# shiftlab-nanodrone/sparse-gslam

Hardware: AMD Instinct MI355X
Metric: edge-Jacobians/sec per GN iter on SE(2) graph; final chi2 vs g2o (higher is better)
Workload: dtype f64

## Files before the change

### sparse_gslam_amd/csrc/sgo_amg.h

```cpp
#pragma once
#include <hip/hip_runtime.h>

#include <string>
#include <vector>

#include "sgo_internal.h"

namespace sgo {

struct AmgConfig {
  double theta = 0.02;
  double theta_coarse = 0.02;
  double theta_scale = 1.0;
  double omega = 0.8;
  int max_levels = 10;
  int nu_coarse = 1;
  bool nu_from_env = false;
  int kdepth = 1 << 20;
  int fcg2_depth = 1;
  bool smooth = true;
  double omega_p = 0.66;
  double theta_filter = 1e-3;
  bool filtered_smoothing = true;
  bool fold = true;
  int fold0_rows = 60000;
  bool lists_on_device = true;
  int coarsest_nodes = 400;
  const struct AmgKeptAgg* keep_agg = nullptr;
};
struct AmgKeptAgg {
  std::vector<std::vector<int>> agg, visit_c;
  std::vector<int> nc;
};

struct AmgProf {
  void* user = nullptr;
  void (*begin)(void* user, int kid, double bytes) = nullptr;
  void (*end)(void* user) = nullptr;
};

struct AmgHalo {
  HaloDev* dev = nullptr;
  int G = 1, bmax = 0;
  const int* bnd_host = nullptr;
  bool (*reserve)(void* user, size_t packet_doubles) = nullptr;
  void* user = nullptr;
  const std::vector<double>* w0 = nullptr;
};

struct ChunkArena;
struct DevArena;
struct Amg;

struct HostLevel {
  int n = 0, nslot = 0;
  std::vector<int> rowptr, row, col;
  std::vector<int> visit;
};

enum class AmgPatterns { host, device, device_aggregation };
Amg* amg_create(hipStream_t s, const BsrDev& A0, const Sym0Dev& S0, const Tile0Dev& T0, const HostLevel& H0, const double* d_poses,
                const int* d_free_id, const AmgConfig& cfg, const AmgProf& prof, std::string* err, ChunkArena* scratch, DevArena* arena,
                DevArena* tmp_arena, AmgPatterns patterns, struct AmgHostL0* pre0 = nullptr, const AmgHalo* halo = nullptr);
struct AmgHostL0;
AmgHostL0* amg_host_l0_new();
void amg_host_l0_run(AmgHostL0* p, const HostLevel& H0, const std::vector<double>& w, const AmgConfig& cfg, ChunkArena* scratch, bool agg_only = false);
bool amg_host_l0_agg_only(const AmgHostL0* p);
void amg_host_l0_free(AmgHostL0* p);
bool amg_host_l0_ready(const AmgHostL0* p);
AmgConfig amg_effective_config(const AmgConfig& cfg_in, int n, int nslot);
void amg_destroy(Amg* m);
int amg_update(Amg* m, hipStream_t s, std::string* err);
enum class AmgXs0 {
  compute = 0,
  ready = 1,
  ready_with_halo = 2
};
int amg_apply(Amg* m, hipStream_t s, const double* r, double* z, const double* dotvec, double* partials,
              const PcgScalars* S, const double* dotvec2 = nullptr, AmgXs0 xs0 = AmgXs0::compute);
struct Comm;
void amg_set_shard(Amg* m, Comm* comm, int u0, int u1, int row0, int row1, const HaloDev* slices = nullptr);
bool amg_comm_failed(const Amg* m);
int amg_debug_coarse_rhs(Amg* m, hipStream_t s, const double* r, double* out_dev, int cap3);
long long amg_debug_array(Amg* m, hipStream_t s, int level, int what, void* out, long long cap_bytes);
double* amg_xs0(Amg* m);
double amg_omega(const Amg* m);
bool amg_coarsest_not_spd(Amg* m, hipStream_t s);
int amg_num_levels(const Amg* m);
bool amg_has_filtered(const Amg* m);
long long amg_level0_bytes(const Amg* m);
void amg_describe(const Amg* m, std::string* out);
void amg_kept_aggregates(const Amg* m, AmgKeptAgg* out);

}
```

### sparse_gslam_amd/csrc/sgo_amg.hip

```cpp
#include <algorithm>
#include <chrono>
#include <cmath>
#include <cstdio>
#include <cstdlib>
#include <cstring>
#include <numeric>
#include <vector>

#include "sgo_amg.h"
#include "sgo_amg_host.h"
#include "sgo_sort.h"
#include "sgo_comm.h"
#include "sgo_device.h"

namespace sgo {

namespace {

__global__ __launch_bounds__(kBlock) void k_block_norms(BsrDev A, double* __restrict__ w) {
  for (int k = blockIdx.x * kBlock + threadIdx.x; k < A.nslot; k += gridDim.x * kBlock) {
    double b[9];
    load_block(A, (size_t)k, b);
    double s = 0.0;
#pragma unroll
// ... 318 lines not shown
    }
    seg_scan<9>(key, acc);
    if (segment_end(key, lane)) {
#pragma unroll
      for (int c = 0; c < 9; ++c) {
        if (OUT_BSR) out[blk_at(c, (size_t)key, nout)] = acc[c];
        else out[9 * (size_t)key + c] = acc[c];
      }
      if (OUT_BSR && mirror) {
        const int mk = mirror[key];
        if (mk >= 0) {
#pragma unroll
          for (int r = 0; r < 3; ++r)
#pragma unroll
            for (int c = 0; c < 3; ++c) out[blk_at(3 * c + r, (size_t)mk, nout)] = acc[3 * r + c];
        }
      }
    }
  }
}

__device__ __forceinline__ void restrict_groups(const PDev& P, const double* __restrict__ r, double* __restrict__ rc,
                                                const PcgScalars* S, int row0, int row1, int nb_main, int block) {
  const int lane = threadIdx.x & 63;
  const size_t np = (size_t)P.t_n;
  if (block >= nb_main) {
    if (S && S->stop) return;
    __shared__ double sm[kWavesPerBlock][3];
    const int lc = block - nb_main;
    const int gb = P.t_long[2 * lc], ge = P.t_long[2 * lc + 1];
    double acc[3] = {0.0, 0.0, 0.0};
    for (int t = gb + (int)threadIdx.x; t < ge; t += kBlock) {
      const size_t i = (size_t)P.t_row[t];
      if (row1 > 0 && ((int)i < row0 || (int)i >= row1)) continue;
      const double ri[3] = {r[3 * i], r[3 * i + 1], r[3 * i + 2]};
      double b[9];
      load9_pairs(P.t_blk, P.t_blk8, (size_t)t, np, b, P.stream_nt != 0);
      block_tmul_acc(b, ri, acc);
    }
#pragma unroll
    for (int q = 0; q < 3; ++q) {
      const double v = wave_sum(acc[q]);
      if (lane == 0) sm[threadIdx.x >> 6][q] = v;
    }
    __syncthreads();
    if (threadIdx.x < 3) {
      double v = sm[0][threadIdx.x];
      for (int w = 1; w < kWavesPerBlock; ++w) v += sm[w][threadIdx.x];
      rc[3 * (size_t)P.t_col[gb] + threadIdx.x] = v;
    }
    return;
  }
  GroupCursor gc = group_cursor(P.t_grp, P.t_ngrp, nb_main, block);
  if (S && S->stop) return;
  for (bool first = true; gc.g < gc.gend; gc.g += gc.gstride, first = false) {
    int gb, ge;
    group_bounds(gc, P.t_grp, first, gb, ge);
    if (P.t_nlong > 0 && ge - gb > kLongColumn) continue;
    double acc[3] = {0.0, 0.0, 0.0};
    int key = -1 - lane;
    for (int t = gb + lane; t < ge; t += 64) {
      key = P.t_col[t];
      const size_t i = (size_t)P.t_row[t];
      if (row1 > 0 && ((int)i < row0 || (int)i >= row1)) continue;
      const double ri[3] = {r[3 * i], r[3 * i + 1], r[3 * i + 2]};
      double b[9];
      load9_pairs(P.t_blk, P.t_blk8, (size_t)t, np, b, P.stream_nt != 0);
      block_tmul_acc(b, ri, acc);
    }
    seg_scan<3>(key, acc);
    if (segment_end(key, lane)) {
      rc[3 * (size_t)key] = acc[0];
      rc[3 * (size_t)key + 1] = acc[1];
      rc[3 * (size_t)key + 2] = acc[2];
    }
  }
}
__global__ __launch_bounds__(kBlock) void k_restrict_p(PDev P, const double* __restrict__ r, double* __restrict__ rc,
                                                       const PcgScalars* S, int row0, int row1, int nb_main) {
  restrict_groups(P, r, rc, S, row0, row1, nb_main, (int)blockIdx.x);
}
__global__ __launch_bounds__(kBlock, 4) void k_jacobi0_restrict(Sym0Dev A, Spmv0Args a, int nb_spmv, PDev P, double* __restrict__ rc,
                                                                 int nb_main) {
  if ((int)blockIdx.x < nb_spmv) spmv0_groups<S0_JACOBI>(A, a, nb_spmv);
  else restrict_groups(P, a.b, rc, a.S, 0, 0, nb_main, (int)blockIdx.x - nb_spmv);
}
void launch_restrict_p(hipStream_t s, const PDev& P, const double* r, double* rc, const PcgScalars* S, int row0, int row1) {
  const int nb = grid_for(P.t_ngrp, kWavesPerBlock);
  SGO_LAUNCH(k_restrict_p, dim3(nb + P.t_nlong), dim3(kBlock), 0, s, P, r, rc, S, row0, row1, nb);
}

__global__ __launch_bounds__(kBlock) void k_prolong_p(int n, PDev P, const double* __restrict__ u1, SpmvRatio r1,
                                                      const double* __restrict__ u2, SpmvRatio r2,
                                                      double* __restrict__ x, const PcgScalars* S,
                                                      const double* __restrict__ xadd, int row0, int row1) {
  GroupCursor gc = group_cursor(P.r_grp, P.r_ngrp, gridDim.x, blockIdx.x);
  if (S && S->stop) return;
  double c1, c2;
  cycle_coefficients(r1, r2, u2 != nullptr, c1, c2);
  const int lane = threadIdx.x & 63;
  const size_t np = (size_t)P.r_n;
  for (bool first = true; gc.g < gc.gend; gc.g += gc.gstride, first = false) {
    int gb, ge;
    group_bounds(gc, P.r_grp, first, gb, ge);
    double acc[3] = {0.0, 0.0, 0.0};
    int key = -1 - lane;
    for (int e = gb + lane; e < ge; e += 64) {
      key = P.row[e];
      if (row1 > 0 && (key < row0 || key >= row1)) {
        key = -1 - lane;
        continue;
      }
      double w[3], b[9];
      coarse_operand(u1, u2, c1, c2, 3 * (size_t)P.col[e], w);
      load9_pairs(P.r_blk, P.r_blk8, (size_t)e, np, b, P.stream_nt != 0);
      block_mul_acc(b, w, acc);
    }
    seg_scan<3>(key, acc);
    if (segment_end(key, lane)) {
      const size_t o = 3 * (size_t)key;
      if (xadd) {
        acc[0] += xadd[o]; acc[1] += xadd[o + 1]; acc[2] += xadd[o + 2];
      }
      x[o] += acc[0]; x[o + 1] += acc[1]; x[o + 2] += acc[2];
    }
  }
}

__device__ __forceinline__ int find_sorted(const int* __restrict__ v, int lo, int hi, int key) {
  while (lo < hi) {
    const int mid = (lo + hi) >> 1;
    const int x = v[mid];
    if (x == key) return mid;
    if (x < key) lo = mid + 1;
    else hi = mid;
  }
  return -1;
}

struct FoldDev {
  int f_lo = 0, f_hi = 0;
  const int* row = nullptr;
  const int* col = nullptr;
  int* ap2p = nullptr;
  int* st_pos = nullptr;
};
struct UpDev {
  int n = 0, ngrp = 0;
  const int* row = nullptr;
  const int* idx = nullptr;
  const int* col = nullptr;
  const int* grp = nullptr;
};

__global__ __launch_bounds__(kBlock) void k_fold_match(FoldDev F, const int* __restrict__ p_rowptr, const int* __restrict__ p_col,
                                                       unsigned long long* __restrict__ keys) {
  for (int f = F.f_lo + blockIdx.x * kBlock + threadIdx.x; f < F.f_hi; f += gridDim.x * kBlock) {
    const int i = F.row[f], c = F.col[f];
    F.ap2p[f] = find_sorted(p_col, p_rowptr[i], p_rowptr[i + 1], c);
    keys[f - F.f_lo] = ((unsigned long long)(unsigned)c << 32) | (unsigned)(f - F.f_lo);
  }
}
__global__ __launch_bounds__(kBlock) void k_fold_unpack(FoldDev F, const unsigned long long* __restrict__ sorted, int* __restrict__ t_row,
                                                        int* __restrict__ t_col) {
  const int nf = F.f_hi - F.f_lo;
  for (int t = blockIdx.x * kBlock + threadIdx.x; t < nf; t += gridDim.x * kBlock) {
    const unsigned long long k = sorted[t];
    const int f = F.f_lo + (int)(unsigned)(k & 0xffffffffull);
// ... 880 lines not shown
               (const double*)P.blk, (const double*)L.A.dinv, m->cfg.omega, L.PS);
  }
  if (P.local_lists) hipMemsetAsync(C.A.blk, 0, sizeof(double) * 9 * (size_t)C.A.nslot, s);
  {
    Scope sc(m->prof, level0 ? K_SA_RAP0 : K_SA_RAP, 156.0 * P.rap.n + 72.0 * C.A.nslot);
    SGO_LAUNCH((k_block_products<false, true, true>), dim3(grid_for(P.rap.ngrp, kWavesPerBlock)), dim3(kBlock), 0, s,
               P.rap, BsrDev(), (const double*)P.blk, (const double*)P.apblk, C.A.blk, (size_t)C.A.nslot, (const int*)P.rap_mirror,
               (const int*)P.row, row0, P.local_lists ? 0 : row1, 1);
  }
  if (own) sh.reduce(s, C.A.blk, 9 * (size_t)C.A.nslot);
}

struct CoarseSol {
  const double *u1 = nullptr, *u2 = nullptr;
  SpmvRatio c1, c2;
};
struct RhsSub { const double* sub; SpmvRatio c; double* out; };
struct DotReq { const double *vec = nullptr, *vec2 = nullptr; double* parts = nullptr; };

struct CycleForm { int nu; enum { unfolded, folded, folded_in_two_sweeps } kind; };
CycleForm cycle_form(const Amg* m, int l, bool rhs_sub, bool dots) {
  const AmgLevel& L = m->lv[l];
  CycleForm f{(l > 0 && L.tR && L.smoothed) ? std::max(1, m->cfg.nu_coarse) : 1, CycleForm::unfolded};
  if (!L.fold || rhs_sub) return f;
  if (l == 0) {
    if (m->shard.mode == Shard0::single) f.kind = CycleForm::folded;
  } else if (!dots) {
    if (f.nu == 1) f.kind = CycleForm::folded;
    if (f.nu == 2) f.kind = CycleForm::folded_in_two_sweeps;
  }
  return f;
}

bool fold_level(const Amg* m, int l, int nf) {
  return m->cfg.fold && nf > 0 && (l > 0 || (m->shard.mode != Shard0::owner && m->lv[0].A.n <= m->cfg.fold0_rows));
}

CoarseSol coarse_solve(Amg* m, hipStream_t s, int l, const PcgScalars* S);

void restrict_level(Amg* m, hipStream_t s, int l, const double* res, const PcgScalars* S, bool folded = false) {
  AmgLevel& L = m->lv[l];
  AmgLevel& C = m->lv[l + 1];
  const int row0 = l == 0 ? m->shard.row0 : 0, row1 = l == 0 ? m->shard.row1 : 0;
  if (l == 0 && m->shard.mode == Shard0::owner && L.smoothed && L.P.local_lists)
    hipMemsetAsync(C.bk, 0, sizeof(double) * 3 * (size_t)C.A.n, s);
  if (L.smoothed) {
    const PDev& P = folded ? L.PS : L.P;
    Scope sc(m->prof, l == 0 ? K_RESTRICT_P0 : K_RESTRICT_P, 44.0 * P.t_n + 24.0 * L.A.n + 24.0 * L.nc);
    launch_restrict_p(s, P, res, C.bk, S, row0, row1);
  } else {
    Scope sc(m->prof, l == 0 ? K_RESTRICT0 : K_RESTRICT, 40.0 * L.A.n + 24.0 * L.nc);
    SGO_LAUNCH(k_restrict, dim3(grid_for(L.mem_ngrp, kWavesPerBlock)), dim3(kBlock), 0, s, L.mem_ngrp, L.mem_grp, L.mem, L.agg, L.d, res, C.bk, S, row0, row1);
  }
}
int jacobi_sweep(Amg* m, hipStream_t s, AmgLevel& L, const double* x, const double* b, double* out, const PcgScalars* S,
                 const DotReq& dots = DotReq(), const CoarseSol* cs = nullptr) {
  SpmvArgs a{};
  a.x = x; a.b = b; a.y = out; a.omega = m->cfg.omega; a.S = S;
  if (dots.vec) { a.dotA = dots.vec; a.dotA2 = dots.vec2; a.partials = dots.parts; }
  if (cs) {
    a.agg = L.agg; a.d = L.d; a.u1 = cs->u1; a.u2 = cs->u2; a.c1 = cs->c1; a.c2 = cs->c2;
    Scope sc(m->prof, K_SPMV_JACOBI_P, 80.0 * L.A.nslot + 140.0 * L.A.n + 48.0 * L.nc);
    return launch_spmv_ex(s, L.A, SPMV_JACOBI_P, a);
  }
  Scope sc(m->prof, K_SPMV_JACOBI, 80.0 * L.A.nslot + 120.0 * L.A.n);
  return launch_spmv_ex(s, L.A, SPMV_JACOBI, a);
}

int pass0(Amg* m, hipStream_t s, int mode, const Spmv0Args& a, int ranks = 1) {
  const bool tile = m->T0.ntile > 0, f32 = tile && m->S0.fblk != nullptr;
  const int kid = mode == S0_RESID ? (tile ? (f32 ? K_SPMV0T_RESID_F32 : K_SPMV0T_RESID) : K_SPMV0_RESID)
                                   : (tile ? (f32 ? K_SPMV0T_JACOBI_F32 : K_SPMV0T_JACOBI) : K_SPMV0_JACOBI);
  Scope sc(m->prof, kid, bytes_spmv0(m->S0, mode, f32) / ranks);
  return launch_spmv0_any(s, m->S0, m->T0, mode, a);
}
void first_sweep0(Amg* m, hipStream_t s, const double* rhs, AmgXs0 xs0) {
  if (xs0 != AmgXs0::compute) return;
  const Shard0& sh = m->shard;
  const bool own = sh.mode == Shard0::owner;
  const size_t r0 = own ? sh.row0 : 0;
  Scope sc(m->prof, K_DOT, 96.0 * m->lv[0].A.n);
  launch_precond_bj(s, own ? sh.row1 - sh.row0 : m->lv[0].A.n, m->S0.dinv + 6 * r0, rhs + 3 * r0, m->lv[0].xs + 3 * r0, m->cfg.omega);
}
void presmooth0(Amg* m, hipStream_t s, const double* rhs, const PcgScalars* S, AmgXs0 xs0) {
  AmgLevel& L = m->lv[0];
  Shard0& sh = m->shard;
  first_sweep0(m, s, rhs, xs0);
  if (sh.mode == Shard0::owner && xs0 != AmgXs0::ready_with_halo) sh.exchange(s, L.xs, 3, sh.part->bnd, sh.part->bmax);
  if (sh.mode == Shard0::allreduce && !sh.part) hipMemsetAsync(L.rs, 0, sizeof(double) * 3 * (size_t)L.A.n, s);
  Spmv0Args a{};
  a.x = L.xs; a.b = rhs; a.y = L.rs; a.S = S; a.u0 = sh.u0; a.u1 = sh.u1;
  if (sh.mode == Shard0::single || a.u1 > a.u0) pass0(m, s, S0_RESID, a, sh.G);
}
void prolong0(Amg* m, hipStream_t s, const CoarseSol& cs, const PcgScalars* S) {
  AmgLevel& L = m->lv[0];
  const Shard0& sh = m->shard;
  const bool own = sh.mode == Shard0::owner;
  const int row0 = own ? sh.row0 : 0, row1 = own ? sh.row1 : 0;
  if (L.smoothed) {
    Scope sc(m->prof, K_PROLONG_P0, 44.0 * L.P.r_n + 52.0 * L.A.n);
    SGO_LAUNCH(k_prolong_p, dim3(grid_for(L.P.r_ngrp, kWavesPerBlock)), dim3(kBlock), 0, s, L.A.n, L.P, cs.u1, cs.c1, cs.u2, cs.c2,
               L.xs, S, (const double*)nullptr, row0, row1);
  } else {
    Scope sc(m->prof, K_PROLONG0, 68.0 * L.A.n);
    SGO_LAUNCH(k_prolong_add, dim3(grid_for(own ? row1 - row0 : L.A.n, kBlock)), dim3(kBlock), 0, s, L.A.n, L.agg, L.d, cs.u1, cs.c1,
                       cs.u2, cs.c2, L.xs, S, (const double*)nullptr, row0, row1);
  }
  if (own && sh.part->nhalo > 0) {
    const HaloDev& H = *sh.part;
    SGO_LAUNCH(k_prolong_rows, dim3(grid_for(H.nhalo, kBlock)), dim3(kBlock), 0, s, H.nhalo, H.halo_rows, L.smoothed ? L.P : PDev(),
               (const int*)L.agg, (const double*)L.d, cs.u1, cs.c1, cs.u2, cs.c2, L.xs, S);
  }
}
int postsmooth0(Amg* m, hipStream_t s, const double* rhs, double* out, const DotReq& dots, const PcgScalars* S) {
  AmgLevel& L = m->lv[0];
  Shard0& sh = m->shard;
  Spmv0Args b{};
  b.x = L.xs; b.b = rhs; b.y = out; b.omega = m->cfg.omega; b.S = S; b.u0 = sh.u0; b.u1 = sh.u1;
  if (sh.mode != Shard0::allreduce) {
    if (dots.vec) { b.dotA = dots.vec; b.dotA2 = dots.vec2; b.partials = dots.parts; }
    return pass0(m, s, S0_JACOBI, b, sh.G);
  }
  if (!sh.part) hipMemsetAsync(out, 0, sizeof(double) * 3 * (size_t)L.A.n, s);
  if (b.u1 > b.u0) pass0(m, s, S0_JACOBI, b);
  if (sh.part) sh.gather(s, out);
  else sh.reduce(s, out, 3 * (size_t)L.A.n);
  if (!dots.vec) return 0;
  const int grid = grid_for(3LL * L.A.n, kBlock);
  Scope sc(m->prof, K_DOT, 72.0 * L.A.n);
  SGO_LAUNCH(k_dots2, dim3(grid), dim3(kBlock), 0, s, 3 * L.A.n, (const double*)out, dots.vec, dots.vec2, dots.parts, S);
  return grid;
}
int cycle0_fold(Amg* m, hipStream_t s, const double* rhs, double* out, const DotReq& dots, const PcgScalars* S, AmgXs0 xs0) {
  AmgLevel& L = m->lv[0];
  AmgLevel& C = m->lv[1];
  first_sweep0(m, s, rhs, xs0);
  Spmv0Args b{};
  b.x = L.xs; b.b = rhs; b.y = L.rs; b.omega = m->cfg.omega; b.S = S;
  if (m->T0.ntile == 0) {
    const int nb_spmv = grid_for(m->S0.ngrp, kWavesPerBlock), nb_main = grid_for(L.PS.t_ngrp, kWavesPerBlock);
    Scope sc(m->prof, K_JACOBI0_RESTRICT, bytes_spmv0(m->S0, S0_JACOBI) + 44.0 * L.PS.t_n + 24.0 * L.A.n + 24.0 * L.nc);
    SGO_LAUNCH(k_jacobi0_restrict, dim3(nb_spmv + nb_main + L.PS.t_nlong), dim3(kBlock), 0, s, m->S0, b, nb_spmv, L.PS, C.bk, nb_main);
  } else {
    pass0(m, s, S0_JACOBI, b);
    restrict_level(m, s, 0, rhs, S, true);
  }
  const CoarseSol cs = coarse_solve(m, s, 0, S);
  const int grid = std::min(grid_for(L.PS.r_ngrp, kFoldThreads / 64), 512);
  Scope sc(m->prof, K_PROLONG_FOLD0, 44.0 * L.PS.r_n + 72.0 * L.A.n);
  SGO_LAUNCH(k_prolong_fold, dim3(grid), dim3(kFoldThreads), 0, s, L.PS, cs.u1, cs.c1, cs.u2, cs.c2, (const double*)L.rs, out, S, dots.vec,
             dots.vec2, dots.vec ? dots.parts : nullptr);
  return grid;
}
int cycle0(Amg* m, hipStream_t s, const double* rhs, double* out, const DotReq& dots, const PcgScalars* S, AmgXs0 xs0) {
  if (cycle_form(m, 0, false, dots.vec).kind == CycleForm::folded) return cycle0_fold(m, s, rhs, out, dots, S, xs0);
  presmooth0(m, s, rhs, S, xs0);
  restrict_level(m, s, 0, m->lv[0].rs, S);
  m->shard.reduce(s, m->lv[1].bk, 3 * (size_t)m->lv[1].A.n);
  const CoarseSol cs = coarse_solve(m, s, 0, S);
  prolong0(m, s, cs, S);
  return postsmooth0(m, s, rhs, out, dots, S);
}

constexpr int kUnfuseSlots = 400000;
void pre_resid(Amg* m, hipStream_t s, AmgLevel& L, const double* rhs, const PcgScalars* S) {
  SpmvArgs a{};
  a.b = rhs; a.y = L.rs; a.omega = m->cfg.omega; a.S = S;
  if (L.A.nslot >= kUnfuseSlots) {
    {
      Scope sc(m->prof, K_DOT, 96.0 * L.A.n);
      launch_precond_bj(s, L.A.n, L.A.dinv, rhs, L.xs, m->cfg.omega);
    }
    a.x = L.xs;
    Scope sc(m->prof, K_SPMV_RESID, 80.0 * L.A.nslot + 72.0 * L.A.n);
    launch_spmv_ex(s, L.A, SPMV_RESID, a);
    return;
  }
  a.y2 = L.xs;
  Scope sc(m->prof, K_SPMV_PRE_RESID, 80.0 * L.A.nslot + 120.0 * L.A.n);
  launch_spmv_ex(s, L.A, SPMV_PRE_RESID, a);
}
const double* presmooth(Amg* m, hipStream_t s, AmgLevel& L, const double* rhs, const RhsSub* sub, int nu, const PcgScalars* S) {
  if (sub) {
    SpmvArgs a{};
    a.b = rhs; a.y = L.rs; a.y2 = L.xs; a.omega = m->cfg.omega; a.S = S; a.bsub = sub->sub; a.c1 = sub->c; a.b_out = sub->out;
    Scope sc(m->prof, K_SPMV_PRE_RESID_S, 80.0 * L.A.nslot + 168.0 * L.A.n);
    launch_spmv_ex(s, L.A, SPMV_PRE_RESID_S, a);
  } else {
    pre_resid(m, s, L, rhs, S);
  }
  double* res = L.rs;
  for (int sw = 1; sw < nu; ++sw) {
    SpmvArgs a{};
    a.b = res; a.y = (res == L.rs) ? L.tR : L.rs; a.y2 = L.xs; a.omega = m->cfg.omega; a.S = S;
    Scope sc(m->prof, K_SPMV_PRE_RESID_ACC, 80.0 * L.A.nslot + 144.0 * L.A.n);
    launch_spmv_ex(s, L.A, SPMV_PRE_RESID_ACC, a);
    res = a.y;
  }
  return res;
}
int prolong_postsmooth(Amg* m, hipStream_t s, AmgLevel& L, const double* rhs, double* out, const CoarseSol& cs, int nu,
                       const DotReq& dots, const PcgScalars* S) {
  if (L.smoothed) {
    {
      Scope sc(m->prof, K_PROLONG_P, 80.0 * L.P.np + 52.0 * L.A.n);
      SGO_LAUNCH(k_prolong_p, dim3(grid_for(L.P.r_ngrp, kWavesPerBlock)), dim3(kBlock), 0, s, L.A.n, L.P, cs.u1, cs.c1, cs.u2, cs.c2,
                 L.xs, S, (const double*)nullptr, 0, 0);
    }
    const double* x = L.xs;
    for (int sw = 1; sw < nu; ++sw) {
      double* dst = (x == L.rs) ? L.tR : L.rs;
      jacobi_sweep(m, s, L, x, rhs, dst, S);
      x = dst;
    }
    return jacobi_sweep(m, s, L, x, rhs, out, S, dots);
  }
  if (L.A.nslot < kUnfuseSlots) return jacobi_sweep(m, s, L, L.xs, rhs, out, S, dots, &cs);
  {
    Scope sc(m->prof, K_PROLONG, 52.0 * L.A.n + 48.0 * L.nc);
    SGO_LAUNCH(k_prolong_add, dim3(grid_for(L.A.n, kBlock)), dim3(kBlock), 0, s, L.A.n, L.agg, L.d, cs.u1, cs.c1, cs.u2, cs.c2, L.xs, S,
               (const double*)nullptr, 0, 0);
  }
  return jacobi_sweep(m, s, L, L.xs, rhs, out, S, dots);
}
int cycle_coarse_fold(Amg* m, hipStream_t s, int l, const double* rhs, double* out, const PcgScalars* S, const double* xadd = nullptr) {
  AmgLevel& L = m->lv[l];
  restrict_level(m, s, l, rhs, S, true);
  const CoarseSol cs = coarse_solve(m, s, l, S);
  Scope sc(m->prof, K_UP_FOLD, 80.0 * L.A.nslot + 44.0 * L.PS.r_n + 100.0 * L.A.n);
  const int grid = grid_for(L.U.ngrp, kWavesPerBlock);
  SGO_LAUNCH(k_up_fold, dim3(grid), dim3(kBlock), 0, s, L.A, L.U, L.PS, rhs, m->cfg.omega, cs.u1, cs.c1, cs.u2, cs.c2, out, S, xadd);
  return grid;
}
int cycle_coarse(Amg* m, hipStream_t s, int l, const double* rhs, double* out, const PcgScalars* S, const RhsSub* sub = nullptr,
                 const DotReq& dots = DotReq()) {
  AmgLevel& L = m->lv[l];
  const CycleForm f = cycle_form(m, l, sub != nullptr, dots.vec != nullptr);
  if (f.kind == CycleForm::folded) return cycle_coarse_fold(m, s, l, rhs, out, S);
  if (f.kind == CycleForm::folded_in_two_sweeps) {
// ... 58 lines not shown
    for (const AmgLevel& L : m->lv)
      if (L.smoothed && L.P.dF) return true;
  return false;
}
long long amg_level0_bytes(const Amg* m) { return m ? m->level0_bytes : 0; }
bool amg_coarsest_not_spd(Amg* m, hipStream_t s) {
  int f = 0;
  if (!m || !m->d_fail) return false;
  if (hipMemcpyAsync(&f, m->d_fail, sizeof(int), hipMemcpyDeviceToHost, s) != hipSuccess) return false;
  if (hipStreamSynchronize(s) != hipSuccess) return false;
  return f != 0;
}
void amg_describe(const Amg* m, std::string* out) { *out = m ? m->desc : ""; }
void amg_kept_aggregates(const Amg* m, AmgKeptAgg* out) {
  if (m && out) *out = m->kept;
}

void amg_destroy(Amg* m) {
  if (!m) return;
  delete m;
}


int amg_update(Amg* m, hipStream_t s, std::string* err) {
  const int last = (int)m->lv.size() - 1;
  {
    AmgLevel& L0 = m->lv[0];
    Scope sc(m->prof, K_POSITIONS0, 40.0 * L0.A.n);
    SGO_LAUNCH(k_positions0, dim3(grid_for(L0.A.n, kBlock)), dim3(kBlock), 0, s, L0.A.n, m->d_free_id, m->d_poses,
                       L0.pos);
  }
  for (int l = 0; l < last; ++l) {
    AmgLevel& L = m->lv[l];
    AmgLevel& C = m->lv[l + 1];
    {
      Scope sc(m->prof, K_CENTRES, 36.0 * L.A.n);
      SGO_LAUNCH(k_centres, dim3(grid_for(L.nc, kWavesPerBlock)), dim3(kBlock), 0, s, L.nc, L.mem_ptr, L.mem, L.pos, C.pos, L.d);
    }
    launch_coarse_operator(m, s, L, C, l == 0);
    {
      Scope sc(m->prof, K_LEVEL_DINV, 120.0 * C.A.n);
      SGO_LAUNCH(k_level_dinv, dim3(grid_for(C.A.n, kBlock)), dim3(kBlock), 0, s, C.A);
    }
  }
  {
    Scope sc(m->prof, K_DENSE_INVERT, 8.0 * m->Np * m->Np);
    const int nb = m->Np / kGjB;
    hipMemsetAsync(m->inv0, 0, sizeof(double) * (size_t)m->Np * m->Np, s);
    hipMemsetAsync(m->d_fail, 0, sizeof(int), s);
    if (last > 0)
      SGO_LAUNCH(k_dense_fill_unique, dim3(grid_for(m->lv[last].A.nslot, kBlock)), dim3(kBlock), 0, s, m->lv[last].A, m->Np, m->inv0);
    else
      SGO_LAUNCH(k_dense_fill, dim3(grid_for(m->lv[last].A.n, kBlock)), dim3(kBlock), 0, s, m->lv[last].A, m->Np, m->inv0);
    SGO_LAUNCH(k_gj_pivot, dim3(1), dim3(kGjB * kGjB), 0, s, m->inv0, m->Np, 0, m->gjP[0], m->d_fail);
    for (int kb = 0; kb < nb; ++kb) {
      const double* src = (kb & 1) ? m->inv1 : m->inv0;
      double* dst = (kb & 1) ? m->inv0 : m->inv1;
      SGO_LAUNCH(k_gj_step, dim3(nb, nb), dim3(kBlock), 0, s, src, dst, m->Np, kb, (const double*)m->gjP[kb & 1],
                 m->gjP[(kb + 1) & 1], m->d_fail);
    }
  }
  const hipError_t le = hipGetLastError();
  if (le != hipSuccess) {
    if (err) *err = std::string("amg_update: a kernel launch failed: ") + hipGetErrorString(le);
    return SGO_EHIP;
  }
  return SGO_OK;
}

void amg_set_shard(Amg* m, Comm* comm, int u0, int u1, int row0, int row1, const HaloDev* slices) {
  m->shard.mode = Shard0::allreduce;
  m->shard.u0 = u0; m->shard.u1 = u1; m->shard.row0 = row0; m->shard.row1 = row1;
  m->shard.comm = comm;
  m->shard.part = slices;
}
bool amg_comm_failed(const Amg* m) { return m && m->shard.failed; }
int amg_debug_coarse_rhs(Amg* m, hipStream_t s, const double* r, double* out_dev, int cap3) {
  if (!m || m->lv.size() < 2) return 0;
  const int n3c = 3 * m->lv[1].A.n;
  if (cap3 < n3c) return -1;
  if (m->lv[0].fold) {
    restrict_level(m, s, 0, r, nullptr, true);
  } else {
    presmooth0(m, s, r, nullptr, AmgXs0::compute);
    restrict_level(m, s, 0, m->lv[0].rs, nullptr);
  }
  hipMemcpyAsync(out_dev, m->lv[1].bk, sizeof(double) * n3c, hipMemcpyDeviceToDevice, s);
  return n3c;
}
namespace {
__global__ __launch_bounds__(kBlock) void k_debug_blocks(BsrDev A, const float* __restrict__ fblk, const float* __restrict__ fblk8,
                                                         double* __restrict__ out) {
  for (int k = blockIdx.x * kBlock + threadIdx.x; k < A.nslot; k += gridDim.x * kBlock) {
    double b[9];
    load_block(A, (size_t)k, b);
    if (fblk && A.ref && A.ref[k] >= 0) {
      const int r = A.ref[k];
      const size_t u = (size_t)(r >> 1), nu = (size_t)A.nus;
      double v[9];
      for (int c = 0; c < 8; ++c) v[c] = (double)fblk[4 * ((size_t)(c >> 2) * nu + u) + (c & 3)];
      v[8] = (double)fblk8[u];
      for (int p = 0; p < 3; ++p)
        for (int q = 0; q < 3; ++q) b[3 * p + q] = (r & 1) ? v[3 * q + p] : v[3 * p + q];
    }
    for (int c = 0; c < 9; ++c) out[9 * (size_t)k + c] = b[c];
  }
}
}

long long amg_debug_array(Amg* m, hipStream_t s, int level, int what, void* out, long long cap_bytes) {
  if (!m || level < 0 || level >= (int)m->lv.size()) return 0;
  if (m->shard.mode != Shard0::single) return SGO_EINVAL;
  const int last = (int)m->lv.size() - 1;
  AmgLevel& L = m->lv[level];
  const PDev& P = L.P;
  const PDev& PS = L.PS;
  const bool transfer = level < last, sm = transfer && L.smoothed, fo = sm && L.fold;
  const size_t n = (size_t)L.A.n, ns = (size_t)L.A.nslot, nc = transfer ? (size_t)L.nc : 0;
  const size_t nsc = transfer ? (size_t)m->lv[level + 1].A.nslot : 0;
  const void* src = nullptr;
  size_t bytes = 0;
  auto arr = [&](bool have, const void* p, size_t count, size_t elem) {
    if (have && p) {
      src = p;
      bytes = count * elem;
    }
  };
  const size_t I = sizeof(int), F = sizeof(float), Dd = sizeof(double);
  const bool f32 = level == 0 && m->T0.ntile > 0 && m->S0.fblk != nullptr;
  switch (what) {
    case SGO_AMG_INFO: {
      const CycleForm cf = cycle_form(m, level, false, false);
      const double v[SGO_AMG_INFO_COUNT] = {(double)n, (double)ns, (double)nc, sm ? 1.0 : 0.0, (sm && P.dF) ? 1.0 : 0.0, fo ? 1.0 : 0.0,
                                            transfer ? (double)cf.kind : 0.0, transfer ? (double)cf.nu : 0.0, m->cfg.omega, m->cfg.omega_p,
                                            sm ? (double)P.np : 0.0, sm ? (double)P.nap : 0.0, sm ? (double)P.val.n : 0.0,
                                            sm ? (double)P.ap.n : 0.0, sm ? (double)P.rap.n : 0.0, (double)(last + 1), f32 ? 1.0 : 0.0,
                                            (double)m->N, (double)m->Np, sm ? (double)P.t_nlong : 0.0, fo ? (double)PS.t_nlong : 0.0,
                                            (double)m->kdepth, m->cfg.theta_filter, (double)nsc};
      if (cap_bytes >= (long long)sizeof v) std::memcpy(out, v, sizeof v);
      return (long long)sizeof v;
    }
    case SGO_AMG_A_ROWPTR: arr(true, L.A.rowptr, n + 1, I); break;
    case SGO_AMG_A_COL: arr(true, L.A.col, ns, I); break;
    case SGO_AMG_A_BLK:
    case SGO_AMG_A_BLK_F32: {
      if (what == SGO_AMG_A_BLK_F32 && !f32) return 0;
      const long long need = (long long)(9 * ns * Dd);
      if (cap_bytes < need) return need;
      double* tmp = nullptr;
      if (hipMalloc(&tmp, (size_t)need) != hipSuccess) return SGO_ENOMEM;
      SGO_LAUNCH(k_debug_blocks, dim3(grid_for((long long)ns, kBlock)), dim3(kBlock), 0, s, L.A,
                 what == SGO_AMG_A_BLK_F32 ? (const float*)m->S0.fblk : (const float*)nullptr, (const float*)m->S0.fblk8, tmp);
      hipError_t e = hipMemcpyAsync(out, tmp, (size_t)need, hipMemcpyDeviceToHost, s);
      if (e == hipSuccess) e = hipStreamSynchronize(s);
      hipFree(tmp);
      return e == hipSuccess ? need : (long long)SGO_EHIP;
    }
    case SGO_AMG_A_DINV: arr(true, L.A.dinv, 6 * n, Dd); break;
    case SGO_AMG_POS: arr(true, L.pos, 2 * n, Dd); break;
    case SGO_AMG_D: arr(transfer, L.d, 2 * n, Dd); break;
    case SGO_AMG_AGG: arr(transfer, L.agg, n, I); break;
    case SGO_AMG_MEM_PTR: arr(transfer, L.mem_ptr, nc + 1, I); break;
    case SGO_AMG_MEM: arr(transfer, L.mem, n, I); break;
    case SGO_AMG_P_ROWPTR: arr(sm, P.rowptr, n + 1, I); break;
    case SGO_AMG_P_ROW: arr(sm, P.row, (size_t)P.np, I); break;
    case SGO_AMG_P_COL: arr(sm, P.col, (size_t)P.np, I); break;
    case SGO_AMG_P_BLK: arr(sm, P.blk, 9 * (size_t)P.np, Dd); break;
    case SGO_AMG_P_RBLK: arr(sm, P.r_blk, 9 * (size_t)P.r_n, F); break;
    case SGO_AMG_P_TBLK: arr(sm, P.t_blk, 9 * (size_t)P.t_n, F); break;
    case SGO_AMG_P_TPOS: arr(sm, P.t_pos, (size_t)P.np, I); break;
    case SGO_AMG_P_TROW: arr(sm, P.t_row, (size_t)P.np, I); break;
    case SGO_AMG_P_TCOL: arr(sm, P.t_col, (size_t)P.np, I); break;
    case SGO_AMG_STRONG: arr(sm && P.dF, P.strong, ns, 1); break;
    case SGO_AMG_DF: arr(sm, P.dF, 9 * n, Dd); break;
    case SGO_AMG_DINVF: arr(sm, P.dinvF, 9 * n, Dd); break;
    case SGO_AMG_AP_A: arr(sm, P.ap.a, (size_t)P.ap.n, I); break;
    case SGO_AMG_AP_B: arr(sm, P.ap.b, (size_t)P.ap.n, I); break;
    case SGO_AMG_AP_TGT: arr(sm, P.ap.tgt, (size_t)P.ap.n, I); break;
    case SGO_AMG_AP_BLK: arr(sm, P.apblk, 9 * (size_t)P.nap, Dd); break;
    case SGO_AMG_PS_ROW: arr(fo, PS.row, (size_t)PS.np, I); break;
    case SGO_AMG_PS_COL: arr(fo, PS.col, (size_t)PS.np, I); break;
    case SGO_AMG_PS_RBLK: arr(fo, PS.r_blk, 9 * (size_t)PS.r_n, F); break;
    case SGO_AMG_PS_TBLK: arr(fo, PS.t_blk, 9 * (size_t)PS.t_n, F); break;
    case SGO_AMG_PS_TROW: arr(fo, PS.t_row, (size_t)PS.np, I); break;
    case SGO_AMG_PS_TCOL: arr(fo, PS.t_col, (size_t)PS.np, I); break;
    case SGO_AMG_PS_STPOS: arr(fo, L.F.st_pos, (size_t)PS.np, I); break;
    case SGO_AMG_INV: arr(level == last, m->inv, (size_t)m->Np * m->Np, Dd); break;
    default: return SGO_EINVAL;
  }
  if (!src || bytes == 0) return 0;
  if (cap_bytes < (long long)bytes) return (long long)bytes;
  if (hipMemcpyAsync(out, src, bytes, hipMemcpyDeviceToHost, s) != hipSuccess || hipStreamSynchronize(s) != hipSuccess) return SGO_EHIP;
  return (long long)bytes;
}
double* amg_xs0(Amg* m) { return (m && m->lv.size() > 1) ? m->lv[0].xs : nullptr; }
double amg_omega(const Amg* m) { return m ? m->cfg.omega : 0.0; }

int amg_apply(Amg* m, hipStream_t s, const double* r, double* z, const double* dotvec, double* partials,
              const PcgScalars* S, const double* dotvec2, AmgXs0 xs0) {
  if (m->lv.size() == 1) {
    {
      Scope sc(m->prof, K_DENSE_APPLY, 8.0 * m->N * m->N);
      SGO_LAUNCH(k_dense_apply, dim3(grid_for(m->N, kWavesPerBlock)), dim3(kBlock), 0, s, m->N, m->Np, m->inv, r, z, S);
    }
    if (!dotvec) return 0;
    const int grid = grid_for(m->N, kBlock);
    Scope sc(m->prof, K_DOT, 24.0 * m->N);
    SGO_LAUNCH(k_dots2, dim3(grid), dim3(kBlock), 0, s, m->N, (const double*)z, dotvec, dotvec2, partials, S);
    return grid;
  }
  return cycle0(m, s, r, z, DotReq{dotvec, dotvec2, partials}, S, xs0);
}

void dev_scan_exclusive(hipStream_t s, int* v, int n, int* sums) {
  if (n <= kScanSmall) {
    SGO_LAUNCH(k_scan_small, dim3(1), dim3(1024), 0, s, v, n);
    return;
  }
  const int nb = (n + kScanChunk - 1) / kScanChunk;
  SGO_LAUNCH(k_scan_sums, dim3(std::max(nb, 1)), dim3(kBlock), 0, s, (const int*)v, n, sums);
  SGO_LAUNCH(k_scan_top, dim3(1), dim3(kBlock), 0, s, sums, nb);
  SGO_LAUNCH(k_scan_apply, dim3(std::max(nb, 1)), dim3(kBlock), 0, s, v, n, (const int*)sums, nb);
}
AmgConfig amg_effective_config(const AmgConfig& cfg_in, int n, int nslot) {
  AmgConfig cfg = cfg_in;
  cfg.nu_coarse = nslot >= 600000 ? 2 : 1;
  if (const char* e = std::getenv("SGO_AMG_SMOOTH")) cfg.smooth = std::atoi(e) != 0;
  if (const char* e = std::getenv("SGO_AMG_LISTS")) cfg.lists_on_device = std::string(e) != "host";
  if (const char* e = std::getenv("SGO_AMG_THETA_FILTER")) cfg.theta_filter = std::atof(e);
  if (const char* e = std::getenv("SGO_AMG_FILTER")) cfg.filtered_smoothing = cfg.filtered_smoothing && std::atoi(e) != 0;
  if (const char* e = std::getenv("SGO_AMG_OMEGA")) cfg.omega = std::atof(e);
  if (const char* e = std::getenv("SGO_AMG_OMEGA_P")) cfg.omega_p = std::atof(e);
  if (const char* e = std::getenv("SGO_AMG_THETA")) cfg.theta = cfg.theta_coarse = std::atof(e);
  if (const char* e = std::getenv("SGO_AMG_FOLD")) cfg.fold = std::atoi(e) != 0;
  if (const char* e = std::getenv("SGO_AMG_FOLD0_ROWS")) cfg.fold0_rows = std::atoi(e);
  cfg.fold = cfg.fold && cfg.smooth && cfg.lists_on_device;
  if (const char* e = std::getenv("SGO_AMG_NU")) {
    cfg.nu_coarse = std::max(1, std::atoi(e));
    cfg.nu_from_env = true;
  }
  if (cfg.smooth) cfg.kdepth = 0;
  if (const char* e = std::getenv("SGO_AMG_KDEPTH")) cfg.kdepth = std::atoi(e);
  if (const char* e = std::getenv("SGO_AMG_FCG2_DEPTH")) cfg.fcg2_depth = std::atoi(e);
  cfg.coarsest_nodes = std::min(1000, std::max(cfg.coarsest_nodes, n / 1500));
  return cfg;
}

struct AmgHostL0 {
  HostCoarse hc;
  bool ready = false;
  bool agg_only = false;
  double theta_used = 0.0;
};

#include "sgo_amg_dev.inc"

AmgHostL0* amg_host_l0_new() { return new AmgHostL0(); }
void amg_host_l0_free(AmgHostL0* p) { delete p; }
bool amg_host_l0_ready(const AmgHostL0* p) { return p && p->ready; }
bool amg_host_l0_agg_only(const AmgHostL0* p) { return p && p->ready && p->agg_only; }
void amg_host_l0_run(AmgHostL0* p, const HostLevel& H0, const std::vector<double>& w, const AmgConfig& cfg_in, ChunkArena* scratch, bool agg_only) {
  try {
    const AmgConfig cfg = amg_effective_config(cfg_in, H0.n, H0.nslot);
    if (H0.n <= cfg.coarsest_nodes || 1 >= cfg.max_levels) return;
    if (agg_only) {
      p->hc.nc = host_aggregate(H0, w, cfg, 0, scratch, p->hc.agg, p->hc.visit_c, &p->theta_used);
      p->agg_only = true;
      p->ready = true;
      return;
    }
    host_coarsen(H0, w, cfg, 0, scratch, p->hc);
    p->ready = p->hc.err.empty();
  } catch (...) {
    p->ready = false;
  }
}

namespace {

enum GroupId { G_MEM, G_VAL, G_R, G_T, G_C, G_F, G_GAL, G_ST, G_PSR, G_U, G_APL, G_RAPL, G_COUNT };
struct GroupBatch {
  struct Job {
    const int* ptr = nullptr;
    int nseg = 0, total = 0;
    bool on = false;
    const int** grp = nullptr;
    int* ngrp = nullptr;
  };
  Job job[G_COUNT];
  template <class IntPtr>
  void add(GroupId id, const int* ptr, int nseg, int total, IntPtr* grp, int* ngrp) {
    job[id] = Job{ptr, nseg, total, true, (const int**)grp, ngrp};
  }
  bool run(DevSetup& D) {
// ... 690 lines not shown
```

### sparse_gslam_amd/csrc/sgo_ctx.h

```cpp
#pragma once
#include <chrono>
#include <cstdio>
#include <cstring>
#include <memory>
#include <string>
#include <thread>
#include <vector>

#include "sgo_amg.h"
#include "sgo_comm.h"
#include "sgo_direct.h"
#include "sgo_mfront.h"
#include "sgo_internal.h"
#include "sgo_overlay.h"
#include "sgo_policy.h"

using namespace sgo;

struct HostArena {
  std::unique_ptr<char[]> mem;
  size_t cap = 0, used = 0;
  void reserve(size_t bytes) {
    used = 0;
    if (bytes <= cap) return;
// ... 1 lines not shown
    cap = bytes + bytes / 4;
    mem.reset(new char[cap + 64]);
  }
  void* take(size_t bytes) {
    char* base = (char*)(((uintptr_t)mem.get() + 63) & ~(uintptr_t)63);
    void* q = base + used;
    used += (bytes + 63) & ~(size_t)63;
    return used <= cap ? q : nullptr;
  }
};

struct HaloHost {
  int G = 1, me = 0, bmax = 0;
  std::vector<int> rank_row;
  std::vector<int> bnd;
};

struct sgo_ctx {
  int device = 0;
  HostArena stage;
  ChunkArena amg_scratch;
  hipStream_t stream = nullptr;
  sgo_opts opts{};
  std::string err;
  Comm comm;
  int shard_u0 = 0, shard_u1 = 0, shard_units = 0;
  int shard_row0 = 0, shard_row1 = 0;
  std::vector<int> unit_row0;
  bool owner = false;
  bool gather_slices = false;
  bool replicated = false;
  HaloDev halo;
  HaloHost halo_host;
  bool halo_failed = false;
  std::vector<double> order_xy;
  HierarchyState hier;
  bool amg_dchg_pending = false;
  int probe_dev_k = -1;
  double probe_dev_max = -1.0;
  double* d_dref = nullptr;
  double* d_dref_agg = nullptr;
  int agg_grid = 0;
  double* h_dchg = nullptr;
  int dchg_grid = 0;
  double* h_dchg_dev = nullptr;
  double last_dchg[3] = {0, 0, 0};
  std::string lag_note;
  int* d_comm_flag = nullptr;
  bool comm_graph_failed = false;
  long long level0_bytes = 0;
  double *halo_send = nullptr, *halo_recv = nullptr;
  size_t halo_cap = 0;
  int halo_ranks = 0;

  bool has_graph = false;
  int V = 0, E = 0, n = 0;
  std::vector<int> free_id;
  std::vector<int> fixed_active;
  std::vector<int> row_of_asc;
  HostLevel H0;
  double setup_seconds = 0.0;

  DevArena graph_arena;
  DevArena amg_arena;
  DevArena amg_arena_prev;
  DevArena amg_tmp_arena;
  Amg* amg_prev = nullptr;
  std::string amg_prev_desc;
  struct CallKnobs {
    int comm_graph = -1;
    int stall_window = -1;
    int first_solve_cap = 600;
    bool fail_trial_build = false;
    bool fail_device_setup = false;
    bool keep_agg = false;
    int setup_mode = 2;
    bool dev_aggregation = false;
    bool lag_on = true;
    double lag_tau = 0.006;
    double lag_slope = 0.0;
    int lag_force_from = -1;
    int rebuild_cost = 150;
    bool force_rebuild = false;
  } knobs;
  struct CallState {
    bool in_optimize = false;
    int pcg_softcap = 0;
    double bb_ref = 0.0;
    bool warm_valid = false;
    bool floor_seen = false;
    bool lag_on = false;
    bool skip_update = false;
    bool lag_expect = false;
    bool force_keep = false;
    int lag_cap = 0;
  } call;
  AmgKeptAgg kept_agg;
  double* d_poses = nullptr;
  int* d_free_id = nullptr;
  EdgeListDev el;
  Sym0Dev S0;
  Tile0Dev T0;
  BsrDev A;
  EdgeSlotsDev es;
  int *d_rowptr = nullptr, *d_eidx = nullptr, *d_hrowptr = nullptr;
  double *d_dgb = nullptr, *d_b = nullptr, *d_x = nullptr, *d_r = nullptr, *d_z = nullptr, *d_p = nullptr,
         *d_q = nullptr, *d_s1 = nullptr, *d_s2 = nullptr, *d_e2 = nullptr;
  double* d_partials = nullptr;
  double* d_hist = nullptr;
  PcgScalars* d_S = nullptr;
  double* d_lanczos = nullptr;
  int pcg_exec_key = 0;
  PcgScalars* h_S = nullptr;
  double* h_hist = nullptr;
  bool linearized = false;

  Amg* amg = nullptr;
  bool amg_pending = false;
  bool rows_pending = false;
  std::vector<uint8_t> lz_fixed;
  std::vector<int32_t> lz_ei, lz_ej;
  Direct* direct = nullptr;
  std::string direct_why;
  Mfront* mf = nullptr;
  std::string mf_why;
  int mf_order_hint = -1;
  DirectResult* d_dres = nullptr;
  DirectResult* h_dres = nullptr;
  double* d_zparts = nullptr;
  struct PcgCounts {
    int start_bb = 0, start_rz = 0;
    int n_pq = 0, n_rz = 0, n_rr = 0, n_zq = 0;
    int n_xq = 0, n_bx = 0;
  } pcg_counts;
  struct PcgStartArgs {
    double tol = 0.0, tol_cap = 0.0, bb_ref = 0.0;
    int maxit = 0;
  } pcg_start;
  std::string solver_desc;
  std::string solver_text;

  hipGraphExec_t pcg_exec = nullptr;
  int pcg_exec_chunk = 0;
  int pcg_pred = 0;
  bool pcg_stalled = false;
  int pcg_stall_window = 0;
  double tol_scale = 1.0;
  double* d_xprev = nullptr;
  double tol_cap = 0.0;
  AmgHostL0* l0_pre = nullptr;
  std::thread l0_thread;
  std::vector<double> l0_w;
  PcgScalars* h_S2 = nullptr;
  double* h_pose_stage = nullptr;
  size_t pose_stage_cap = 0;
  PcgScalars* h_Sz = nullptr;
  PcgScalars* d_Sz = nullptr;
  hipEvent_t ev_S[2] = {nullptr, nullptr};

  Overlay ov;
  int its_base = 0;
  int its_last = 0;
  std::string update_note;

  struct EdgeActivity {
    bool ready = false;
    std::vector<int32_t> vi, vj;
    std::vector<uint8_t> dead;
    std::vector<int32_t> live_deg;
    int n_inactive = 0;
    int* d_ids = nullptr;
    double* d_rows = nullptr;
    unsigned char* d_flag = nullptr;
    unsigned char* d_mark = nullptr;
    double* d_parts = nullptr;
    size_t ids_cap = 0, rows_cap = 0, flag_cap = 0, mark_cap = 0, parts_cap = 0;
  } edges;
  struct RobustKinds {
    std::vector<uint8_t> kind;
    int n_other = 0;
    unsigned char* d_kind = nullptr;
    size_t kind_cap = 0;
  } robust;

  struct Hypotheses {
    char* d_ws = nullptr;
    size_t ws_cap = 0;
  } hyp;

  struct Marginals {
    double* d_cov = nullptr;
    int* d_idx = nullptr;
    size_t cov_cap = 0, idx_cap = 0;
  } marg;

// ... 233 lines not shown
```

### sparse_gslam_amd/csrc/sgo_device.h

```cpp
#pragma once
#include "sgo_internal.h"

namespace sgo {
namespace {

constexpr double kPi = 3.14159265358979323846;

__device__ __forceinline__ double norm_theta(double t) {
  if (t >= -kPi && t < kPi) return t;
  double m = floor(t / (2 * kPi));
  t = t - m * 2 * kPi;
  if (t >= kPi) t -= 2 * kPi;
  if (t < -kPi) t += 2 * kPi;
  return t;
}


struct EdgeOperands {
  double xi, yi, ti, xj, yj, tj;
  double zx, zy, zt;
};
template <class Src>
__device__ __forceinline__ void edge_operands(const Src& s, size_t ns, int k, const double* __restrict__ poses, EdgeOperands& p) {
  const int vi = s.vi[k], vj = s.vj[k];
// ... 180 lines not shown
  edge_error(p, sz, cz, e);
  EdgeWeight W;
  edge_weight<KINDS>(s, ns, k, e, W);
  EdgeJac J;
  edge_jacobians(p, sz, cz, J);
  edge_side(W, J, dir, S);
}

__device__ __forceinline__ double readlane_d(double v, int l) {
  const int lo = __builtin_amdgcn_readlane(__double2loint(v), l), hi = __builtin_amdgcn_readlane(__double2hiint(v), l);
  return __hiloint2double(hi, lo);
}

__device__ __forceinline__ double wave_sum(double v);

template <int N>
__device__ __forceinline__ void block_sum_store(double (&v)[N], double* out, int stride) {
  __shared__ double sm[N][kWavesPerBlock];
  const int lane = threadIdx.x & 63, w = threadIdx.x >> 6;
#pragma unroll
  for (int i = 0; i < N; ++i) {
    double s = wave_sum(v[i]);
    if (lane == 0) sm[i][w] = s;
  }
  __syncthreads();
  if (threadIdx.x == 0) {
#pragma unroll
    for (int i = 0; i < N; ++i) {
      double s = sm[i][0];
#pragma unroll
      for (int k = 1; k < kWavesPerBlock; ++k) s += sm[i][k];
      out[(size_t)i * stride + blockIdx.x] = s;
    }
  }
}

__device__ __forceinline__ double block_reduce_parts(const double* parts, int nparts) {
  __shared__ double sm2[kWavesPerBlock];
  __shared__ double res;
  double s = 0.0;
  for (int i = threadIdx.x; i < nparts; i += kBlock) s += parts[i];
  s = wave_sum(s);
  __syncthreads();
  if ((threadIdx.x & 63) == 0) sm2[threadIdx.x >> 6] = s;
  __syncthreads();
  if (threadIdx.x == 0) {
    double t = sm2[0];
#pragma unroll
    for (int k = 1; k < kWavesPerBlock; ++k) t += sm2[k];
    res = t;
  }
  __syncthreads();
  return res;
}

template <int N>
__device__ __forceinline__ void block_reduce_parts_n(const double* const (&parts)[N], const int (&cnt)[N],
                                                     double (&out)[N]) {
  __shared__ double smn[N][kWavesPerBlock];
  double s[N];
#pragma unroll
  for (int c = 0; c < N; ++c) {
    s[c] = 0.0;
    if (parts[c])
      for (int i = threadIdx.x; i < cnt[c]; i += kBlock) s[c] += parts[c][i];
  }
#pragma unroll
  for (int c = 0; c < N; ++c) s[c] = wave_sum(s[c]);
  __syncthreads();
  if ((threadIdx.x & 63) == 0) {
#pragma unroll
    for (int c = 0; c < N; ++c) smn[c][threadIdx.x >> 6] = s[c];
  }
  __syncthreads();
#pragma unroll
  for (int c = 0; c < N; ++c) {
    double t = smn[c][0];
#pragma unroll
    for (int k = 1; k < kWavesPerBlock; ++k) t += smn[c][k];
    out[c] = t;
  }
}

template <int CTRL, int ROW_MASK>
__device__ __forceinline__ int dpp_int(int old, int v) {
  if (ROW_MASK == 0xF) return __builtin_amdgcn_update_dpp(0, v, CTRL, 0xF, 0xF, true);
  return __builtin_amdgcn_update_dpp(old, v, CTRL, ROW_MASK, 0xF, false);
}
__device__ __forceinline__ int next_lane_key(int key) { return __builtin_amdgcn_update_dpp(0, key, 0x130, 0xF, 0xF, true); }
template <int CTRL, int ROW_MASK>
__device__ __forceinline__ double dpp_double(double v) {
  const int lo = dpp_int<CTRL, ROW_MASK>(0, __double2loint(v)), hi = dpp_int<CTRL, ROW_MASK>(0, __double2hiint(v));
  return __hiloint2double(hi, lo);
}
__device__ __forceinline__ double wave_sum(double v) {
  v += dpp_double<0x111, 0xF>(v);
  v += dpp_double<0x112, 0xF>(v);
  v += dpp_double<0x114, 0xF>(v);
  v += dpp_double<0x118, 0xF>(v);
  v += dpp_double<0x142, 0xA>(v);
  v += dpp_double<0x143, 0xC>(v);
  return __hiloint2double(__builtin_amdgcn_readlane(__double2hiint(v), 63), __builtin_amdgcn_readlane(__double2loint(v), 63));
}

template <int N, int CTRL, int ROW_MASK>
__device__ __forceinline__ void seg_scan_step(int row, double (&v)[N]) {
  constexpr int kNoKey = (int)0x80000000;
  const double f = dpp_int<CTRL, ROW_MASK>(kNoKey, row) == row ? 1.0 : 0.0;
#pragma unroll
  for (int i = 0; i < N; ++i) {
    const double u = dpp_double<CTRL, ROW_MASK>(v[i]);
    v[i] = fma(f, u, v[i]);
  }
}
template <int N>
__device__ __forceinline__ void seg_scan(int row, double (&v)[N]) {
  seg_scan_step<N, 0x111, 0xF>(row, v);
  seg_scan_step<N, 0x112, 0xF>(row, v);
  seg_scan_step<N, 0x114, 0xF>(row, v);
  seg_scan_step<N, 0x118, 0xF>(row, v);
  seg_scan_step<N, 0x142, 0xA>(row, v);
  seg_scan_step<N, 0x143, 0xC>(row, v);
}
__device__ __forceinline__ bool segment_end(int key, int lane) {
  const int kn = next_lane_key(key);
  return key >= 0 && (lane == 63 || kn != key);
}

__device__ __forceinline__ void load_block(const BsrDev& A, size_t k, double (&b)[9]) {
  double v0, v1, v2, v3, v4, v5, v6, v7, v8;
  if (A.ref == nullptr) {
    const size_t ns = (size_t)A.nslot;
    v0 = A.blk[blk_at(0, k, ns)]; v1 = A.blk[blk_at(1, k, ns)]; v2 = A.blk[blk_at(2, k, ns)];
    v3 = A.blk[blk_at(3, k, ns)]; v4 = A.blk[blk_at(4, k, ns)]; v5 = A.blk[blk_at(5, k, ns)];
    v6 = A.blk[blk_at(6, k, ns)]; v7 = A.blk[blk_at(7, k, ns)]; v8 = A.blk[blk_at(8, k, ns)];
  } else {
    const int r = A.ref[k];
    if (r < 0) {
      const double* d = A.dblk + 6 * (size_t)(~r);
      v0 = d[0]; v1 = d[1]; v2 = d[2];
      v3 = v1; v4 = d[3]; v5 = d[4];
      v6 = v2; v7 = v5; v8 = d[5];
    } else {
      const size_t u = (size_t)(r >> 1), nu = (size_t)A.nus;
      const double2* __restrict__ bp = reinterpret_cast<const double2*>(A.ublk);
      const double2 p0 = bp[u], p1 = bp[nu + u], p2 = bp[2 * nu + u], p3 = bp[3 * nu + u];
      const bool tr = r & 1;
      v0 = p0.x; v4 = p2.x; v8 = A.ublk8[u];
      v1 = tr ? p1.y : p0.y; v3 = tr ? p0.y : p1.y;
      v2 = tr ? p3.x : p1.x; v6 = tr ? p1.x : p3.x;
      v5 = tr ? p3.y : p2.y; v7 = tr ? p2.y : p3.y;
    }
  }
  b[0] = v0; b[1] = v1; b[2] = v2; b[3] = v3; b[4] = v4; b[5] = v5; b[6] = v6; b[7] = v7; b[8] = v8;
}

template <int WAVES = kWavesPerBlock, class NB, class B>
__device__ __forceinline__ void group_walk_b(int ngrp, NB nblocks, B block, int* first, int* last, int* stride) {
  const int xcd = block & 7, slot = block >> 3, per_xcd = nblocks >> 3;
  const int lo = (int)(((long long)ngrp * xcd) >> 3), hi = (int)(((long long)ngrp * (xcd + 1)) >> 3);
  *first = lo + slot * WAVES + (threadIdx.x >> 6);
  *last = hi;
  *stride = per_xcd * WAVES;
}
__device__ __forceinline__ void group_walk(int ngrp, int* first, int* last, int* stride) {
  group_walk_b(ngrp, gridDim.x, blockIdx.x, first, last, stride);
// ... 30 lines not shown
  const double* const parts[4] = {r1.num ? r1.den : nullptr, r1.num, (use2 && r2.num) ? r2.den : nullptr,
                                  use2 ? r2.num : nullptr};
  const int cnt[4] = {r1.n_den, r1.n_num, r2.n_den, r2.n_num};
  double v[4];
  block_reduce_parts_n<4>(parts, cnt, v);
  if (r1.num) c1 = cycle_ratio(v[0], v[1]);
  if (use2) c2 = cycle_ratio(v[2], v[3]);
}

__device__ __forceinline__ void coarse_operand(const double* __restrict__ u1, const double* __restrict__ u2, double c1, double c2,
                                               size_t a, double (&w)[3]) {
  w[0] = c1 * u1[a]; w[1] = c1 * u1[a + 1]; w[2] = c1 * u1[a + 2];
  if (u2) {
    w[0] += c2 * u2[a]; w[1] += c2 * u2[a + 1]; w[2] += c2 * u2[a + 2];
  }
}

__device__ __forceinline__ void block_mul_acc(const double (&b)[9], const double (&x)[3], double* acc) {
  acc[0] += b[0] * x[0] + b[1] * x[1] + b[2] * x[2];
  acc[1] += b[3] * x[0] + b[4] * x[1] + b[5] * x[2];
  acc[2] += b[6] * x[0] + b[7] * x[1] + b[8] * x[2];
}
__device__ __forceinline__ void block_mul_acc(double2 p0, double2 p1, double2 p2, double2 p3, double b8, const double (&x)[3], double* acc) {
  acc[0] += p0.x * x[0] + p0.y * x[1] + p1.x * x[2];
  acc[1] += p1.y * x[0] + p2.x * x[1] + p2.y * x[2];
  acc[2] += p3.x * x[0] + p3.y * x[1] + b8 * x[2];
}
__device__ __forceinline__ void block_tmul_acc(const double (&b)[9], const double (&r)[3], double* acc) {
  acc[0] += b[0] * r[0] + b[3] * r[1] + b[6] * r[2];
  acc[1] += b[1] * r[0] + b[4] * r[1] + b[7] * r[2];
  acc[2] += b[2] * r[0] + b[5] * r[1] + b[8] * r[2];
}

__device__ __forceinline__ void rigid_add(double dx, double dy, const double (&w)[3], double* x) {
  x[0] += w[0] - dy * w[2]; x[1] += w[1] + dx * w[2]; x[2] += w[2];
}
__device__ __forceinline__ void rigid_t_acc(double dx, double dy, const double (&r)[3], double* acc) {
  acc[0] += r[0]; acc[1] += r[1]; acc[2] += -dy * r[0] + dx * r[1] + r[2];
}
__device__ __forceinline__ void block_rigid_col(const double (&b)[9], double dx, double dy, double (&m)[3]) {
  m[0] = -dy * b[0] + dx * b[1] + b[2];
  m[1] = -dy * b[3] + dx * b[4] + b[5];
  m[2] = -dy * b[6] + dx * b[7] + b[8];
}
__device__ __forceinline__ void block_rigid_acc(const double (&b)[9], double dx, double dy, double* acc) {
  acc[0] += b[0]; acc[1] += b[1]; acc[2] += -dy * b[0] + dx * b[1] + b[2];
  acc[3] += b[3]; acc[4] += b[4]; acc[5] += -dy * b[3] + dx * b[4] + b[5];
  acc[6] += b[6]; acc[7] += b[7]; acc[8] += -dy * b[6] + dx * b[7] + b[8];
}
__device__ __forceinline__ void rigid_t_block_acc(const double (&b)[9], const double (&m)[3], double dx, double dy, double* acc) {
  acc[0] += b[0]; acc[1] += b[1]; acc[2] += m[0];
  acc[3] += b[3]; acc[4] += b[4]; acc[5] += m[1];
  acc[6] += -dy * b[0] + dx * b[3] + b[6]; acc[7] += -dy * b[1] + dx * b[4] + b[7];
  acc[8] += -dy * m[0] + dx * m[1] + m[2];
}

__device__ __forceinline__ void dinv_apply(const double* __restrict__ di, double omega, const double (&v)[3], double (&o)[3]) {
  o[0] = omega * (di[0] * v[0] + di[1] * v[1] + di[2] * v[2]);
  o[1] = omega * (di[1] * v[0] + di[3] * v[1] + di[4] * v[2]);
  o[2] = omega * (di[2] * v[0] + di[4] * v[1] + di[5] * v[2]);
}
__device__ __forceinline__ void dinv_from_block(const double (&d)[6], double* __restrict__ di) {
  const double d00 = d[0], d01 = d[1], d02 = d[2], d11 = d[3], d12 = d[4], d22 = d[5];
  const double c00 = d11 * d22 - d12 * d12, c01 = d02 * d12 - d01 * d22, c02 = d01 * d12 - d02 * d11;
  const double c11 = d00 * d22 - d02 * d02, c12 = d01 * d02 - d00 * d12, c22 = d00 * d11 - d01 * d01;
  const double det = d00 * c00 + d01 * c01 + d02 * c02;
  const double id = (det != 0.0 && isfinite(det)) ? 1.0 / det : 0.0;
  di[0] = c00 * id; di[1] = c01 * id; di[2] = c02 * id; di[3] = c11 * id; di[4] = c12 * id; di[5] = c22 * id;
}

template <int MODE>
__device__ __forceinline__ void spmv0_groups(const Sym0Dev& A, const Spmv0Args& a, int nblocks) {
  const int lane = threadIdx.x & 63;
  const size_t nu = (size_t)A.nus;
  const double2* __restrict__ bp = reinterpret_cast<const double2*>(A.ublk);
  double dotacc[2] = {0.0, 0.0};
  const int ulo = a.u1 > 0 ? a.u0 : 0, uhi = a.u1 > 0 ? a.u1 : A.ngrp;
  GroupCursor gc = group_cursor(A.grp, uhi - ulo, nblocks, blockIdx.x, ulo);
  int f_r0 = 0, f_ob = 0, f_tb = 0;
  if (gc.g < gc.gend) {
    f_r0 = A.grow[gc.g]; f_ob = A.gown[gc.g]; f_tb = A.gtr[gc.g];
  }
  if (a.S && a.S->stop) return;
  for (bool first = true; gc.g < gc.gend; gc.g += gc.gstride, first = false) {
    int gb, ge;
    group_bounds(gc, A.grp, first, gb, ge);
    const int r0 = first ? f_r0 : A.grow[gc.g];
    int ob = first ? f_ob : A.gown[gc.g], tb = first ? f_tb : A.gtr[gc.g];
    double acc[3] = {0.0, 0.0, 0.0};
    int row = -1 - lane;
    for (int kb = gb; kb < ge; kb += 64) {
      const int k = kb + lane;
      const bool active = k < ge;
      const int m = active ? (int)A.meta[k] : (kSlotNoBlock << 6);
      const int cj = active ? A.col[k] : 0;
      const int type = m >> 6;
      const unsigned long long omask = __ballot(type == kSlotOwned), tmask = __ballot(type == kSlotTransposed);
      const int orank = (int)__builtin_amdgcn_mbcnt_hi((unsigned)(omask >> 32), __builtin_amdgcn_mbcnt_lo((unsigned)omask, 0u));
      const int trank = (int)__builtin_amdgcn_mbcnt_hi((unsigned)(tmask >> 32), __builtin_amdgcn_mbcnt_lo((unsigned)tmask, 0u));
      int idx = ob + orank;
      const bool tr = type == kSlotTransposed;
      if (tr) idx = A.tref[tb + trank];
      ob += __popcll(omask);
      tb += __popcll(tmask);
      if (active) row = r0 + (m & 63);
      if (type != kSlotNoBlock) {
        const size_t c = 3 * (size_t)cj;
        const double x0 = a.x[c], x1 = a.x[c + 1], x2 = a.x[c + 2];
        const double2 p0 = bp[idx], p1 = bp[nu + idx], p2 = bp[2 * nu + idx], p3 = bp[3 * nu + idx];
        const double b8 = A.ublk8[idx];
        const double m01 = tr ? p1.y : p0.y, m02 = tr ? p3.x : p1.x;
        const double m10 = tr ? p0.y : p1.y, m12 = tr ? p3.y : p2.y;
        const double m20 = tr ? p1.x : p3.x, m21 = tr ? p2.y : p3.y;
        acc[0] += p0.x * x0 + m01 * x1 + m02 * x2;
        acc[1] += m10 * x0 + p2.x * x1 + m12 * x2;
        acc[2] += m20 * x0 + m21 * x1 + b8 * x2;
      }
    }
    double dd0 = 0, dd1 = 0, dd2 = 0, dd3 = 0, dd4 = 0, dd5 = 0, s0 = 0, s1 = 0, s2 = 0, rb0 = 0, rb1 = 0, rb2 = 0;
    double di[6] = {0, 0, 0, 0, 0, 0};
    if (row >= 0) {
      const size_t o = 3 * (size_t)row;
      const double* dd = A.dblk + 6 * (size_t)row;
      dd0 = dd[0]; dd1 = dd[1]; dd2 = dd[2]; dd3 = dd[3]; dd4 = dd[4]; dd5 = dd[5];
      s0 = a.x[o]; s1 = a.x[o + 1]; s2 = a.x[o + 2];
      if (MODE != S0_AX) {
        rb0 = a.b[o]; rb1 = a.b[o + 1]; rb2 = a.b[o + 2];
      }
      if (MODE == S0_JACOBI) {
#pragma unroll
        for (int q = 0; q < 6; ++q) di[q] = A.dinv[6 * (size_t)row + q];
      }
    }
    seg_scan<3>(row, acc);
    if (segment_end(row, lane)) {
      const size_t o = 3 * (size_t)row;
      double o0 = acc[0] + dd0 * s0 + dd1 * s1 + dd2 * s2;
      double o1 = acc[1] + dd1 * s0 + dd3 * s1 + dd4 * s2;
      double o2 = acc[2] + dd2 * s0 + dd4 * s1 + dd5 * s2;
      if (MODE != S0_AX) {
        const double t[3] = {rb0 - o0, rb1 - o1, rb2 - o2};
        if (MODE == S0_JACOBI) {
          double sw[3];
          dinv_apply(di, a.omega, t, sw);
          o0 = s0 + sw[0]; o1 = s1 + sw[1]; o2 = s2 + sw[2];
        } else {
          o0 = t[0]; o1 = t[1]; o2 = t[2];
        }
      }
      a.y[o] = o0; a.y[o + 1] = o1; a.y[o + 2] = o2;
      if (a.dotA) dotacc[0] += a.dotA[o] * o0 + a.dotA[o + 1] * o1 + a.dotA[o + 2] * o2;
      if (a.dotA2) dotacc[1] += a.dotA2[o] * o0 + a.dotA2[o + 1] * o1 + a.dotA2[o + 2] * o2;
    }
  }
  if (a.partials) block_sum_store<2>(dotacc, a.partials, kMaxPartials);
}

}
}
```

### sparse_gslam_amd/csrc/sgo_internal.h

```cpp
#pragma once
#include <hip/hip_runtime.h>
#include <hip/hip_ext.h>

#include <algorithm>
#include <atomic>
#include <cstdint>
#include <cstdlib>
#include <string>
#include <vector>

#include "sgo.h"
#include "sgo_hostpool.h"

namespace sgo {

struct BsrDev {
  int n = 0;
  int nslot = 0;
  int ngrp = 0;
  int* row = nullptr;
  int* col = nullptr;
  int* grp = nullptr;
  int* rowptr = nullptr;
  double* blk = nullptr;
// ... 18 lines not shown
  int ncs = 0;
  int ngrp = 0;
  int* col = nullptr;
  unsigned char* meta = nullptr;
  int* tref = nullptr;
  int* grp = nullptr;
  int* grow = nullptr;
  int* gown = nullptr;
  int* gtr = nullptr;
  int nus = 0;
  double* ublk = nullptr;
  double* ublk8 = nullptr;
  float* fblk = nullptr;
  float* fblk8 = nullptr;
  double* dblk = nullptr;
  double* dinv = nullptr;
};

struct TileDesc {
  int row0, row1;
  int g0, g1;
  int h0, h1;
  int e0;
  int nstaged;
};
struct Tile0Dev {
  int ntile = 0;
  int lds_bytes = 0;
  TileDesc* tile = nullptr;
  unsigned int* cv = nullptr;
  unsigned char* off1 = nullptr;
  int* grp1 = nullptr;
  int* grow1 = nullptr;
  int* trowptr = nullptr;
  int* hcol = nullptr;
  int* hfirst = nullptr;
  int hstride = 0;
};

enum : int {
  kRobustDcs = 0, kRobustHuber = 2, kRobustPseudoHuber = 3, kRobustCauchy = 4, kRobustGemanMcClure = 5, kRobustWelsch = 6,
  kRobustFair = 7, kRobustTukey = 8, kRobustSaturated = 9
};

enum : int { kSlotDir = 1, kSlotNoEdge = 2, kSlotFixedCol = 4 };
struct EdgeSlotsDev {
  int stride = 0;
  int* vi = nullptr;
  int* vj = nullptr;
  unsigned char* flags = nullptr;
  double* zinv = nullptr;
  double* info = nullptr;
  double* phi = nullptr;
  unsigned char* kind = nullptr;
  int kinds = 0;
};

struct EdgeListDev {
  int E = 0;
  int cnt = 0;
  int* vi = nullptr;
  int* vj = nullptr;
  double* zinv = nullptr;
  double* info = nullptr;
  double* phi = nullptr;
  unsigned char* kind = nullptr;
  int kinds = 0;
};

struct PcgScalars {
  double rz;
  double pq;
  double rr;
  double bb;
  double alpha;
  double beta;
  double tol2;
  double rz_prev;
  int iter;
  int maxit;
  int stop;
  int iter_prev;
  int probe_k;
  int pad_;
  double probe_rel;
  double probe_max;
};

enum : int {
  SPMV_AX = 0, SPMV_RESID = 1, SPMV_JACOBI = 2, SPMV_PRE_RESID = 3,
  SPMV_JACOBI_P = 4, SPMV_PRE_RESID_S = 5, SPMV_AX_C = 6,
  SPMV_PRE_RESID_ACC = 7
};
struct SpmvRatio {
  const double* num = nullptr;
  int n_num = 0;
  const double* den = nullptr;
  int n_den = 0;
};
struct SpmvArgs {
  const double* x = nullptr;
  double* y = nullptr;
  const double* b = nullptr;
  double* y2 = nullptr;
  double omega = 0.0;
  const double* dotA = nullptr;
  const double* dotA2 = nullptr;
  const double* dotB = nullptr;
  const double* dotC = nullptr;
  double* partials = nullptr;
  const PcgScalars* S = nullptr;
  SpmvRatio c1, c2;
  const int* agg = nullptr;
  const double* d = nullptr;
  const double* u1 = nullptr;
  const double* u2 = nullptr;
  const double* bsub = nullptr;
  double* b_out = nullptr;
  const double* x2 = nullptr;
  double* x_out = nullptr;
};

enum : int { S0_AX = 0, S0_RESID = 1, S0_JACOBI = 2 };
struct Spmv0Args {
  const double* x = nullptr;
  double* y = nullptr;
  const double* b = nullptr;
  double omega = 0.0;
  const double* dotA = nullptr;
  const double* dotA2 = nullptr;
  double* partials = nullptr;
  const PcgScalars* S = nullptr;
  long long* dbg_stamps = nullptr;
  bool force_f64 = false;
  int u0 = 0, u1 = 0;
};

struct Comm;
constexpr int kHaloScalars = 4;
struct HaloDev {
  Comm* comm = nullptr;
  int G = 1, me = 0;
  int row0 = 0, row1 = 0;
  int u0 = 0, u1 = 0;
  int g0 = 0, g1 = 0;
  int bmax = 0;
  const int* bnd = nullptr;
  int maxrows = 0;
  const int* rank_row = nullptr;
  int nhalo = 0;
  const int* halo_rows = nullptr;
  int pemax = 0;
  const int* pent = nullptr;
  double* send = nullptr;
  double* recv = nullptr;
  size_t cap = 0;
  double* gparts = nullptr;
  bool* failed = nullptr;
};
struct HaloScalars {
  const double* parts[kHaloScalars] = {nullptr, nullptr, nullptr, nullptr};
  int n[kHaloScalars] = {0, 0, 0, 0};
};

enum KernelId : int {
  K_CHI2 = 0,
  K_REDUCE2,
  K_LINEARIZE,
  K_FINALIZE,
  K_INIT_SCALARS,
  K_SPMV_AX,
  K_SPMV_RESID,
  K_SPMV_JACOBI,
  K_SPMV_PRE_RESID,
  K_SPMV_JACOBI_P,
  K_SPMV_PRE_RESID_S,
  K_SPMV_AX_C,
  K_ALPHA,
  K_UPDATE_XR,
  K_BETA,
  K_UPDATE_P,
  K_DOT,
  K_POSE_UPDATE,
  K_POSITIONS0,
  K_CENTRES,
  K_GALERKIN,
  K_LEVEL_DINV,
  K_RESTRICT,
  K_PROLONG,
  K_DENSE_INVERT,
  K_DENSE_APPLY,
  K_SA_P,
  K_SA_AP,
  K_SA_RAP,
  K_RESTRICT_P,
  K_PROLONG_P,
  K_SPMV_PRE_RESID_ACC,
  K_SPMV0_AX,
  K_SPMV0_RESID,
  K_SPMV0_JACOBI,
  K_SPMV0T_AX,
  K_SPMV0T_RESID,
  K_SPMV0T_JACOBI,
  K_DIRECT,
  K_SPMV0T_RESID_F32,
  K_SPMV0T_JACOBI_F32,
  K_RESTRICT_P0,
  K_PROLONG_P0,
  K_SA_P0,
  K_SA_AP0,
  K_SA_RAP0,
  K_GALERKIN0,
  K_RESTRICT0,
  K_PROLONG0,
  K_PTILDE,
// ... 125 lines not shown
  }
  struct Mark {
    std::vector<size_t> used;
  };
  Mark mark() const {
    Mark m;
    for (const Chunk& c : chunks) m.used.push_back(c.used);
    return m;
  }
  void rewind_to(const Mark& m) {
    for (size_t i = 0; i < chunks.size(); ++i) chunks[i].used = i < m.used.size() ? m.used[i] : 0;
  }
  void release() {
    for (Chunk& c : chunks) hipFree(c.base);
    chunks.clear();
  }
};

struct LaunchEvents {
  hipEvent_t start = nullptr;
  hipEvent_t stop = nullptr;
};
extern thread_local LaunchEvents tl_launch_ev;
#define SGO_LAUNCH(kernel, grid, block, shmem, stream, ...)                                              \
  do {                                                                                                   \
    const ::sgo::LaunchEvents ev_ = ::sgo::tl_launch_ev;                                                 \
    ::sgo::tl_launch_ev = ::sgo::LaunchEvents();                                                         \
    if (ev_.start) hipExtLaunchKernelGGL(kernel, grid, block, shmem, stream, ev_.start, ev_.stop, 0, __VA_ARGS__); \
    else hipLaunchKernelGGL(kernel, grid, block, shmem, stream, __VA_ARGS__);                            \
  } while (0)

void launch_chi2(hipStream_t s, const EdgeListDev& el, int e0, int e1, const double* poses, double* e2_out,
                 double* partials , int* grid_out, const EdgeListDev* el2 = nullptr);
void launch_reduce2(hipStream_t s, const double* partials, int nparts, double* out2);
void launch_edge_prepare(hipStream_t s, int E, const double* meas, const double* info, double* zinv, double* info_soa, size_t stride, size_t at);
void launch_slot_expand(hipStream_t s, int k0, int k1, const int* eidx, const EdgeListDev& el, const EdgeSlotsDev& es);
void launch_edge_gate(hipStream_t s, const EdgeListDev& el, const EdgeListDev* el2, int n, const int* ids, const double* poses,
                      double chi2_max, unsigned char* flag, double* partials, int* count);
void launch_edge_dead_flags(hipStream_t s, const EdgeListDev& el, const EdgeListDev* el2, unsigned char* dead);
void launch_edge_info_scatter(hipStream_t s, int n, const int* ids, const double* rows, const EdgeListDev& el, const EdgeListDev* el2,
                              unsigned char* mark);
void launch_slot_info_refresh(hipStream_t s, int ncs, const int* eidx, const unsigned char* mark, const EdgeListDev& el,
                              const EdgeSlotsDev& es);
void launch_edge_kernel_scatter(hipStream_t s, int n, const int* ids, const double* delta, const unsigned char* kind, const EdgeListDev& el,
                                const EdgeListDev* el2, unsigned char* mark);
void launch_slot_kernel_refresh(hipStream_t s, int ncs, const int* eidx, const unsigned char* mark, const EdgeListDev& el,
                                const EdgeSlotsDev& es);
void launch_edge_robust(hipStream_t s, const EdgeListDev& el, const EdgeListDev* el2, const double* poses, double* rho0, double* w);
void launch_rhs_inject(hipStream_t s, int n, double* dgb, double* save, const double* src, int unit_row, int unit_k);
void launch_rhs_restore(hipStream_t s, int n, double* dgb, const double* save);
void launch_cov_gather(hipStream_t s, int q0, int q1, const int* order, const int* pair_row, int col_row, int k, int n, const double* x,
                       double* cov);
void launch_early_strength(hipStream_t s, const EdgeListDev& el, const double* poses, int n, const int* rowptr, const int* eidx,
                           const unsigned char* flags, const int* hrowptr, double* w);
void launch_linearize(hipStream_t s, const Sym0Dev& A, int g0, int g1, const EdgeSlotsDev& es, const double* poses,
                      double* dgb );
int launch_diag_change(hipStream_t s, int row0, int row1, const double* dblk, double* dref, bool store_ref, double* partials);
void launch_finalize(hipStream_t s, const Sym0Dev& A, int row0, int row1, const double* dgb, double* b, double* x, double* r, double* z,
                     double* p, double* xs, double omega, double* partials, int* grid_out);
void launch_init_scalars(hipStream_t s, PcgScalars* S, const double* rz_parts, int n_rz, const double* bb_parts,
                         int n_bb, double tol, int maxit, double bb_ref, double tol_cap);
void launch_set_probe(hipStream_t s, PcgScalars* S, int probe_k, double probe_max);
void launch_force_stop(hipStream_t s, PcgScalars* S, PcgScalars* mirror);
void launch_restart_scalars(hipStream_t s, PcgScalars* S, const double* rz_parts, int n_rz, int maxit, int keep_stop);
void launch_warm_start(hipStream_t s, int n3, const double* xp, const double* q, const double* b, double* x, double* r,
                       const double* xq_parts, int n_xq, const double* bx_parts, int n_bx);
int launch_spmv0(hipStream_t s, const Sym0Dev& A, int mode, const Spmv0Args& a);
int launch_spmv0t(hipStream_t s, const Sym0Dev& A, const Tile0Dev& T, int mode, const Spmv0Args& a);
inline int launch_spmv0_any(hipStream_t s, const Sym0Dev& A, const Tile0Dev& T, int mode, const Spmv0Args& a) {
  return T.ntile > 0 ? launch_spmv0t(s, A, T, mode, a) : launch_spmv0(s, A, mode, a);
}
inline double bytes_spmv0(const Sym0Dev& A, int mode, bool f32 = false) {
  return (f32 ? 40.0 : 76.0) * A.npairs + (96.0 + (mode != S0_AX ? 24.0 : 0.0) + (mode == S0_JACOBI ? 48.0 : 0.0)) * A.n;
}
constexpr int kTileLdsMax = 157 * 1024;
int launch_spmv_ex(hipStream_t s, const BsrDev& A, int mode, const SpmvArgs& a);
void launch_update_xr(hipStream_t s, int n, PcgScalars* S, const double* pq_parts, int n_pq, const double* dinv,
                      const double* p, const double* q, double* x, double* r, double* z, double* xs, double omega,
                      double* partials, int* grid_out);
constexpr int kLanczosMax = 2048;
struct RecDev {
  PcgScalars* mirror = nullptr;
  double* lanczos = nullptr;
};
void launch_update_p(hipStream_t s, int n, PcgScalars* S, const double* rz_parts, int n_rz, const double* rr_parts,
                     int n_rr, const double* zq_parts, const double* z, double* p, const RecDev& rec = RecDev());
void launch_pose_update(hipStream_t s, int n, const int* free_id, const double* x, double* poses);
void launch_closure_cov(hipStream_t s, int n, const sgo_match_window* win, const float* scores, double* cov,
                        double* info);
void launch_dot(hipStream_t s, int n3, const double* a, const double* b, double* partials, const PcgScalars* S,
                int* grid_out);
void launch_precond_bj(hipStream_t s, int n, const double* dinv, const double* r, double* z, double scale);
void launch_update_xr_rows(hipStream_t s, int nrows, const int* rows, const PcgScalars* S, const double* dinv, const double* p,
                           const double* q, double* r, double* xs, double omega);
void launch_update_p_rows(hipStream_t s, int nrows, const int* rows, const PcgScalars* S, const double* z, double* p);
bool halo_exchange(const HaloDev& H, hipStream_t s, double* data, int width, const int* idx, int idx_max, const HaloScalars& sc,
                   std::string* err);
bool halo_gather_slices(const HaloDev& H, hipStream_t s, double* vec, int width, std::string* err);

}
```

### sparse_gslam_amd/csrc/sgo_kernels.hip

```cpp
#include <algorithm>
#include <cstdlib>

#include "sgo_comm.h"
#include "sgo_device.h"
#include "sgo_internal.h"

namespace sgo {

thread_local LaunchEvents tl_launch_ev;

const char* const kKernelNames[K_COUNT] = {
    "k_chi2",        "k_reduce2",  "k_linearize",   "k_finalize",   "k_init_scalars", "k_spmv<0>",  "k_spmv<1>",
    "k_spmv<2>", "k_spmv<3>", "k_spmv<4>", "k_spmv<5>", "k_spmv<6>",      "k_alpha",       "k_update_xr",  "k_beta",         "k_update_p", "k_dot",
    "k_pose_update", "k_positions0", "k_centres",   "k_galerkin",   "k_level_dinv",   "k_restrict", "k_prolong_add",
    "k_gj_step (dense inverse, all block steps)", "k_dense_apply", "k_p_values", "k_block_products<1, 0, 0>",
    "k_block_products<0, 1, 1>", "k_restrict_p", "k_prolong_p", "k_spmv<7>",
    "k_spmv0<0>", "k_spmv0<1>", "k_spmv0<2>", "k_spmv0t<0, 1024, false>", "k_spmv0t<1, 1024, false>", "k_spmv0t<2, 1024, false>",
    "k_direct", "k_spmv0t<1, 1024, true>", "k_spmv0t<2, 1024, true>", "k_restrict_p @level0", "k_prolong_p @level0", "k_p_values @level0", "k_block_products<1, 0, 0> @level0",
    "k_block_products<0, 1, 1> @level0", "k_galerkin @level0", "k_restrict @level0", "k_prolong_add @level0",
    "k_ptilde_values", "k_ptilde_values @level0", "k_up_fold", "k_prolong_fold @level0", "k_jacobi0_restrict @level0",
    "k_mf_edges + k_mf_factor + k_mf_solve + k_mf_update (multifrontal optimize)", "k_rhs_inject", "k_rhs_restore", "k_cov_gather",
    "k_mf_edges + k_mf_merge + k_mf_panels (multifrontal factor phase)", "k_si_gather", "k_si_panels", "k_si_result",
    "k_fs_rhs", "k_fs_forward", "k_fs_backward", "k_fs_gate"};

// ... 186 lines not shown
    }
  }
}

__global__ __launch_bounds__(kBlock) void k_finalize(Sym0Dev A, int row0, int row1, const double* __restrict__ dgb,
                                                     double* __restrict__ b, double* __restrict__ x,
                                                     double* __restrict__ r, double* __restrict__ z,
                                                     double* __restrict__ p, double* __restrict__ xs, double omega,
                                                     double* __restrict__ partials) {
  double acc[2] = {0.0, 0.0};
  for (int i = row0 + blockIdx.x * kBlock + threadIdx.x; i < row1; i += gridDim.x * kBlock) {
    const double* d = dgb + 9 * (size_t)i;
    const double dg[6] = {d[0], d[1], d[2], d[3], d[4], d[5]};
    const double b0 = d[6], b1 = d[7], b2 = d[8];
    double di[6];
    dinv_from_block(dg, di);
#pragma unroll
    for (int q = 0; q < 6; ++q) {
      A.dblk[6 * (size_t)i + q] = dg[q];
      A.dinv[6 * (size_t)i + q] = di[q];
    }
    const double z0 = di[0] * b0 + di[1] * b1 + di[2] * b2;
    const double z1 = di[1] * b0 + di[3] * b1 + di[4] * b2;
    const double z2 = di[2] * b0 + di[4] * b1 + di[5] * b2;
    const size_t o = 3 * (size_t)i;
    b[o] = b0; b[o + 1] = b1; b[o + 2] = b2;
    if (x) {
      x[o] = 0.0; x[o + 1] = 0.0; x[o + 2] = 0.0;
      r[o] = b0; r[o + 1] = b1; r[o + 2] = b2;
      z[o] = z0; z[o + 1] = z1; z[o + 2] = z2;
      p[o] = z0; p[o + 1] = z1; p[o + 2] = z2;
    }
    if (xs) {
      xs[o] = omega * z0; xs[o + 1] = omega * z1; xs[o + 2] = omega * z2;
    }
    acc[0] += b0 * z0 + b1 * z1 + b2 * z2;
    acc[1] += b0 * b0 + b1 * b1 + b2 * b2;
  }
  block_sum_store<2>(acc, partials, kMaxPartials);
}

__global__ __launch_bounds__(kBlock) void k_diag_change(int row0, int row1, const double* __restrict__ dblk, double* __restrict__ dref,
                                                        int store_ref, double* __restrict__ partials) {
  double acc[3] = {0.0, 0.0, 0.0};
  for (int i = row0 + blockIdx.x * kBlock + threadIdx.x; i < row1; i += gridDim.x * kBlock) {
    const double* d = dblk + 6 * (size_t)i;
    double* e = dref + 6 * (size_t)i;
    double dn = 0.0, nn = 0.0;
#pragma unroll
    for (int k = 0; k < 6; ++k) {
      const double w = (k == 0 || k == 3 || k == 5) ? 1.0 : 2.0, v = d[k], u = v - e[k];
      dn += w * u * u;
      nn += w * v * v;
      if (store_ref) e[k] = v;
    }
    dn = sqrt(dn);
    nn = sqrt(nn);
    acc[0] += dn;
    acc[1] += nn;
    acc[2] += (dn > 0.25 * nn) ? 1.0 : 0.0;
  }
  block_sum_store<3>(acc, partials, kMaxPartials);
}
__global__ void k_force_stop(PcgScalars* S, PcgScalars* mirror) {
  if (S->stop == 0) S->stop = 2;
  if (mirror) *mirror = *S;
}
__global__ void k_set_probe(PcgScalars* S, int probe_k, double probe_max) {
  S->probe_k = probe_k;
  S->probe_rel = 0.0;
  S->probe_max = probe_max;
}
__global__ __launch_bounds__(kBlock) void k_restart_scalars(PcgScalars* S, const double* __restrict__ rz_parts, int n_rz, int maxit,
                                                            int keep_stop) {
  const double rz = block_reduce_parts(rz_parts, n_rz);
  if (threadIdx.x == 0) {
    S->rz = rz;
    S->rz_prev = rz;
    S->pq = 0.0;
    S->alpha = 0.0;
    S->beta = 0.0;
    S->iter_prev = S->iter;
    S->maxit = maxit;
    if (!(keep_stop && S->stop)) S->stop = (isfinite(rz) && rz >= 0.0) ? (rz == 0.0 ? 1 : 0) : 3;
  }
}

__global__ __launch_bounds__(kBlock) void k_warm_start(int n3, const double* __restrict__ xp, const double* __restrict__ q,
                                                       const double* __restrict__ b, double* __restrict__ x, double* __restrict__ r,
                                                       const double* __restrict__ xq_parts, int n_xq,
                                                       const double* __restrict__ bx_parts, int n_bx) {
  const double xq = block_reduce_parts(xq_parts, n_xq);
  const double bx = block_reduce_parts(bx_parts, n_bx);
  double gamma = bx / xq;
  if (!(xq > 0.0) || !isfinite(gamma) || !(gamma > 0.0) || gamma > 4.0) gamma = 0.0;
  for (int i = blockIdx.x * kBlock + threadIdx.x; i < n3; i += gridDim.x * kBlock) {
    x[i] = gamma * xp[i];
    r[i] = b[i] - gamma * q[i];
  }
}

__global__ __launch_bounds__(kBlock) void k_init_scalars(PcgScalars* S, const double* __restrict__ rz_parts, int n_rz,
                                                         const double* __restrict__ bb_parts, int n_bb, double tol,
                                                         int maxit, double bb_ref, double tol_cap) {
  const double* const parts[2] = {rz_parts, bb_parts};
  const int cnt[2] = {n_rz, n_bb};
  double v[2];
  block_reduce_parts_n<2>(parts, cnt, v);
  const double rz = v[0], bb = v[1];
  if (threadIdx.x == 0) {
    S->rz = rz;
    S->bb = bb;
    S->rr = bb;
    S->pq = 0.0;
    S->alpha = 0.0;
    S->beta = 0.0;
    double t2 = tol * tol;
    if (bb_ref > 0.0 && bb > 0.0 && bb < bb_ref) t2 = fmin(tol_cap * tol_cap, t2 * (bb_ref / bb));
    S->tol2 = t2;
    S->rz_prev = rz;
    S->iter = 0;
    S->iter_prev = 0;
    S->maxit = maxit;
    S->stop = (bb == 0.0) ? 1 : (isfinite(bb) && isfinite(rz) ? 0 : 3);
  }
}

__device__ __forceinline__ double ratio_value(const SpmvRatio& r, double den, double num) {
  if (!r.num) return r.den ? 0.0 : 1.0;
  return (den > 0.0 && isfinite(den) && isfinite(num)) ? num / den : 0.0;
}
__device__ __forceinline__ void ratios2(const SpmvRatio& r1, const SpmvRatio& r2, bool use2, double& c1, double& c2) {
  const double* const parts[4] = {r1.num ? r1.den : nullptr, r1.num, (use2 && r2.num) ? r2.den : nullptr,
                                  use2 ? r2.num : nullptr};
  const int cnt[4] = {r1.n_den, r1.n_num, r2.n_den, r2.n_num};
  double v[4];
  block_reduce_parts_n<4>(parts, cnt, v);
  c1 = ratio_value(r1, v[0], v[1]);
  if (use2) c2 = ratio_value(r2, v[2], v[3]);
}

template <int MODE>
__global__ __launch_bounds__(kBlock, ((MODE == SPMV_JACOBI || MODE == SPMV_PRE_RESID) ? 8 : 1))
void k_spmv(BsrDev A, SpmvArgs a) {
  int g, gend, gstride;
  group_walk(A.ngrp, &g, &gend, &gstride);
  int gb0 = 0, ge0 = 0;
  if (g < gend) {
    gb0 = A.grp[g];
    ge0 = A.grp[g + 1];
  }
  if (a.S && a.S->stop) return;
  const int lane = threadIdx.x & 63;
  const size_t ns = (size_t)A.nslot;
  double c1 = 1.0, c2 = 0.0;
  if (MODE == SPMV_JACOBI_P || MODE == SPMV_PRE_RESID_S || MODE == SPMV_AX_C) {
    ratios2(a.c1, a.c2, MODE == SPMV_JACOBI_P && a.u2 != nullptr, c1, c2);
  }
  auto operand = [&](size_t v, double& x0, double& x1, double& x2) {
    if (MODE == SPMV_PRE_RESID || MODE == SPMV_PRE_RESID_S || MODE == SPMV_PRE_RESID_ACC) {
      const double* di = A.dinv + 6 * v;
      double b0 = a.b[3 * v], b1 = a.b[3 * v + 1], b2 = a.b[3 * v + 2];
      if (MODE == SPMV_PRE_RESID_S) {
        b0 -= c1 * a.bsub[3 * v]; b1 -= c1 * a.bsub[3 * v + 1]; b2 -= c1 * a.bsub[3 * v + 2];
      }
      x0 = a.omega * (di[0] * b0 + di[1] * b1 + di[2] * b2);
      x1 = a.omega * (di[1] * b0 + di[3] * b1 + di[4] * b2);
      x2 = a.omega * (di[2] * b0 + di[4] * b1 + di[5] * b2);
    } else {
      x0 = a.x[3 * v]; x1 = a.x[3 * v + 1]; x2 = a.x[3 * v + 2];
      if (MODE == SPMV_JACOBI_P) {
        const size_t ag = 3 * (size_t)a.agg[v];
        double w0 = c1 * a.u1[ag], w1 = c1 * a.u1[ag + 1], w2 = c1 * a.u1[ag + 2];
        if (a.u2) {
          w0 += c2 * a.u2[ag]; w1 += c2 * a.u2[ag + 1]; w2 += c2 * a.u2[ag + 2];
        }
        x0 += w0 - a.d[2 * v + 1] * w2;
        x1 += w1 + a.d[2 * v] * w2;
        x2 += w2;
      } else if (MODE == SPMV_AX_C) {
        x0 -= c1 * a.x2[3 * v]; x1 -= c1 * a.x2[3 * v + 1]; x2 -= c1 * a.x2[3 * v + 2];
      }
    }
  };
  double dotacc[2] = {0.0, 0.0};
  for (bool first = true; g < gend; g += gstride, first = false) {
    const int gb = first ? gb0 : A.grp[g], ge = first ? ge0 : A.grp[g + 1];
    double acc[3] = {0.0, 0.0, 0.0};
    int row = -1 - lane;
    for (int k = gb + lane; k < ge; k += 64) {
      row = A.row[k];
      double x0, x1, x2;
      operand((size_t)A.col[k], x0, x1, x2);
      const double2* __restrict__ bp = reinterpret_cast<const double2*>(A.blk);
      const double2 p0 = bp[k], p1 = bp[ns + k], p2 = bp[2 * ns + k], p3 = bp[3 * ns + k];
      const double b0 = p0.x, b1 = p0.y, b2 = p1.x, b3 = p1.y, b4 = p2.x, b5 = p2.y, b6 = p3.x, b7 = p3.y;
      const double b8 = A.blk[8 * ns + k];
      acc[0] += b0 * x0 + b1 * x1 + b2 * x2;
      acc[1] += b3 * x0 + b4 * x1 + b5 * x2;
      acc[2] += b6 * x0 + b7 * x1 + b8 * x2;
    }
    seg_scan<3>(row, acc);
    if (segment_end(row, lane)) {
      const size_t o = 3 * (size_t)row;
      double o0 = acc[0], o1 = acc[1], o2 = acc[2];
      if (MODE == SPMV_AX_C) {
// ... 28 lines not shown
            v0 += a.y2[o]; v1 += a.y2[o + 1]; v2 += a.y2[o + 2];
          }
          a.y2[o] = v0; a.y2[o + 1] = v1; a.y2[o + 2] = v2;
        }
      }
      a.y[o] = o0; a.y[o + 1] = o1; a.y[o + 2] = o2;
      if (MODE != SPMV_AX_C) {
        if (a.dotA) dotacc[0] += a.dotA[o] * o0 + a.dotA[o + 1] * o1 + a.dotA[o + 2] * o2;
        if (a.dotA2) dotacc[1] += a.dotA2[o] * o0 + a.dotA2[o + 1] * o1 + a.dotA2[o + 2] * o2;
        else if (a.dotB) dotacc[1] += a.dotB[o] * a.dotC[o] + a.dotB[o + 1] * a.dotC[o + 1] + a.dotB[o + 2] * a.dotC[o + 2];
      }
    }
  }
  if (a.partials) block_sum_store<2>(dotacc, a.partials, kMaxPartials);
}

template <int MODE>
__global__ __launch_bounds__(kBlock, 4) void k_spmv0(Sym0Dev A, Spmv0Args a) {
  spmv0_groups<MODE>(A, a, (int)gridDim.x);
}

template <bool F32> struct TileBlk;
template <> struct TileBlk<false> {
  double2 p0, p1, p2, p3;
  double b8;
  __device__ __forceinline__ void load(const Sym0Dev& A, size_t nu, int k) {
    const double2* __restrict__ bp = reinterpret_cast<const double2*>(A.ublk);
    p0 = bp[k]; p1 = bp[nu + k]; p2 = bp[2 * nu + k]; p3 = bp[3 * nu + k];
    b8 = A.ublk8[k];
  }
  __device__ __forceinline__ void get(double (&b)[9]) const {
    b[0] = p0.x; b[1] = p0.y; b[2] = p1.x; b[3] = p1.y; b[4] = p2.x; b[5] = p2.y; b[6] = p3.x; b[7] = p3.y; b[8] = b8;
  }
};
template <> struct TileBlk<true> {
  float4 q0, q1;
  float b8;
  __device__ __forceinline__ void load(const Sym0Dev& A, size_t nu, int k) {
    const float4* __restrict__ fp = reinterpret_cast<const float4*>(A.fblk);
    q0 = fp[k]; q1 = fp[nu + k];
    b8 = A.fblk8[k];
  }
  __device__ __forceinline__ void get(double (&b)[9]) const {
    b[0] = q0.x; b[1] = q0.y; b[2] = q0.z; b[3] = q0.w; b[4] = q1.x; b[5] = q1.y; b[6] = q1.z; b[7] = q1.w; b[8] = b8;
  }
};
template <bool F32>
struct TileGroupLoad {
  int gb, ge, r0;
  bool valid;
  unsigned cw;
  int off;
  TileBlk<F32> blk;
};
template <bool F32>
__device__ __forceinline__ void tile_group_load(const Sym0Dev& A, const Tile0Dev& TL, size_t nu, int g, int lane, TileGroupLoad<F32>& L) {
  L.gb = TL.grp1[g];
  L.ge = TL.grp1[g + 1];
  L.r0 = TL.grow1[g];
  const int k = L.gb + lane;
  L.valid = k < L.ge;
  if (L.valid) {
    L.cw = TL.cv[k];
    L.off = TL.off1[k];
    L.blk.load(A, nu, k);
  }
}
__device__ __forceinline__ void tile_slot(const double* __restrict__ xs, double* __restrict__ vst, int rowl, unsigned cw,
                                          const double (&b)[9], double (&acc)[3]) {
  const double* xc = xs + 3 * (cw & 0xFFFFu);
  const double x[3] = {xc[0], xc[1], xc[2]};
  block_mul_acc(b, x, acc);
  const unsigned vp = cw >> 16;
  if (vp != 0xFFFFu) {
    const double* xr = xs + 3 * rowl;
    const double s0 = xr[0], s1 = xr[1], s2 = xr[2];
    double* v = vst + 3 * vp;
    v[0] = b[0] * s0 + b[3] * s1 + b[6] * s2;
    v[1] = b[1] * s0 + b[4] * s1 + b[7] * s2;
    v[2] = b[2] * s0 + b[5] * s1 + b[8] * s2;
  }
}

template <int MODE, int kTileThreads, bool F32 = false>
__global__ __launch_bounds__(kTileThreads) void k_spmv0t(Sym0Dev A, Tile0Dev TL, Spmv0Args a) {
  const int stop_flag = a.S ? a.S->stop : 0;
  extern __shared__ double lds[];
  __shared__ int next_group_cell;
  int* next_group = &next_group_cell;
  constexpr int NW = kTileThreads / 64;
  const int tid = threadIdx.x, lane = tid & 63, wave = tid >> 6;
  const size_t nu = (size_t)A.nus;
  double dotacc[2] = {0.0, 0.0};
  const int xcd = blockIdx.x & 7, slot = blockIdx.x >> 3, per_xcd = gridDim.x >> 3;
  const int ulo = a.u1 > 0 ? a.u0 : 0, nun = (a.u1 > 0 ? a.u1 : TL.ntile) - ulo;
  const int tlo = ulo + (int)(((long long)nun * xcd) >> 3), thi = ulo + (int)(((long long)nun * (xcd + 1)) >> 3);
  for (int t = tlo + slot; t < thi; t += per_xcd) {
    const int hc_first = tid < TL.hstride ? TL.hfirst[(size_t)t * TL.hstride + tid] : -1;
    const TileDesc T = TL.tile[t];
    if (stop_flag) return;
    const int nr = T.row1 - T.row0, nh = T.h1 - T.h0;
    long long* stamp = a.dbg_stamps ? a.dbg_stamps + 8 * (size_t)t : nullptr;
    if (stamp && tid == 0) stamp[0] = __builtin_amdgcn_s_memtime();
    double* xs = lds;
    double* ys = xs + 3 * (nr + nh);
    double* vst = ys + 3 * nr;
    double xsl[3] = {0.0, 0.0, 0.0};
#pragma unroll
    for (int q = 0; q < 3; ++q) {
      const int i = tid + q * kTileThreads;
      if (i < 3 * nr) xsl[q] = a.x[3 * (size_t)T.row0 + i];
    }
    const int hc0 = tid < TL.hstride ? hc_first : (tid < nh ? TL.hcol[T.h0 + tid] : -1);
    if (tid == 0) *next_group = T.g0 + NW;
    int g = T.g0 + wave;
    bool has = g < T.g1;
    TileGroupLoad<F32> cur;
    cur.valid = false;
    if (has) tile_group_load<F32>(A, TL, nu, g, lane, cur);
    int e0 = 0, e1 = 0;
    double dd0 = 0, dd1 = 0, dd2 = 0, dd3 = 0, dd4 = 0, dd5 = 0;
    if (tid < nr) {
      const int r = T.row0 + tid;
      e0 = TL.trowptr[r] - T.e0;
      e1 = TL.trowptr[r + 1] - T.e0;
      const double* dd = A.dblk + 6 * (size_t)r;
      dd0 = dd[0]; dd1 = dd[1]; dd2 = dd[2]; dd3 = dd[3]; dd4 = dd[4]; dd5 = dd[5];
    }
#pragma unroll
    for (int q = 0; q < 3; ++q) {
      const int i = tid + q * kTileThreads;
      if (i < 3 * nr) {
        xs[i] = xsl[q];
        ys[i] = 0.0;
      }
    }
    for (int i = tid + 3 * kTileThreads; i < 3 * nr; i += kTileThreads) {
      xs[i] = a.x[3 * (size_t)T.row0 + i];
      ys[i] = 0.0;
    }
    if (hc0 >= 0) {
      const size_t c3 = 3 * (size_t)hc0;
      const double h0 = a.x[c3], h1 = a.x[c3 + 1], h2 = a.x[c3 + 2];
      double* d = xs + 3 * (nr + tid);
      d[0] = h0; d[1] = h1; d[2] = h2;
    }
    for (int i = tid + kTileThreads; i < nh; i += kTileThreads) {
      const size_t c3 = 3 * (size_t)TL.hcol[T.h0 + i];
      const double h0 = a.x[c3], h1 = a.x[c3 + 1], h2 = a.x[c3 + 2];
      double* d = xs + 3 * (nr + i);
      d[0] = h0; d[1] = h1; d[2] = h2;
    }
    if (stamp && tid == 0) stamp[1] = __builtin_amdgcn_s_memtime();
    __syncthreads();
    if (stamp && tid == 0) stamp[2] = __builtin_amdgcn_s_memtime();
    while (has) {
      int gn = 0;
      if (lane == 0) gn = atomicAdd(next_group, 1);
      gn = __builtin_amdgcn_readfirstlane(gn);
      const bool hasn = gn < T.g1;
      TileGroupLoad<F32> nxt;
      nxt.valid = false;
      if (hasn) tile_group_load<F32>(A, TL, nu, gn, lane, nxt);
      double acc[3] = {0.0, 0.0, 0.0};
      int row = -1 - lane;
      if (cur.valid) {
        row = cur.r0 + cur.off;
        double b[9];
        cur.blk.get(b);
        tile_slot(xs, vst, row - T.row0, cur.cw, b, acc);
      }
      for (int k = cur.gb + 64 + lane; k < cur.ge; k += 64) {
        const unsigned cw = TL.cv[k];
        row = cur.r0 + TL.off1[k];
        TileBlk<F32> bl;
        bl.load(A, nu, k);
        double b[9];
        bl.get(b);
        tile_slot(xs, vst, row - T.row0, cw, b, acc);
// ... 101 lines not shown
    }
    if (dinv) {
#pragma unroll
      for (int c = 0; c < 6; ++c) pd[c] = dinv[6 * (size_t)i0 + c];
    }
  }
  const int stop0 = S->stop, iter0 = S->iter;
  const double rz = S->rz;
  if (stop0) return;
  const double pq = block_reduce_parts(pq_parts, n_pq);
  const bool bad = !(pq > 0.0) || !isfinite(pq);
  const double alpha = rz / pq;
  if (blockIdx.x == 0 && threadIdx.x == 0) {
    S->pq = pq;
    S->rz_prev = rz;
    S->iter_prev = iter0;
    if (bad) S->stop = 3;
    else S->alpha = alpha;
  }
  if (bad) return;
  double acc[2] = {0.0, 0.0};
  for (int i = i0; i < n; i += gridDim.x * kBlock) {
    const size_t o = 3 * (size_t)i;
    if (i != i0) {
#pragma unroll
      for (int c = 0; c < 3; ++c) {
        pr[c] = r[o + c];
        pq_[c] = q[o + c];
        pp[c] = p[o + c];
        px[c] = x[o + c];
      }
      if (dinv) {
#pragma unroll
        for (int c = 0; c < 6; ++c) pd[c] = dinv[6 * (size_t)i + c];
      }
    }
    const double r0 = pr[0] - alpha * pq_[0], r1 = pr[1] - alpha * pq_[1], r2 = pr[2] - alpha * pq_[2];
    x[o] = px[0] + alpha * pp[0]; x[o + 1] = px[1] + alpha * pp[1]; x[o + 2] = px[2] + alpha * pp[2];
    r[o] = r0; r[o + 1] = r1; r[o + 2] = r2;
    if (dinv) {
      const double z0 = pd[0] * r0 + pd[1] * r1 + pd[2] * r2;
      const double z1 = pd[1] * r0 + pd[3] * r1 + pd[4] * r2;
      const double z2 = pd[2] * r0 + pd[4] * r1 + pd[5] * r2;
      if (xs) {
        xs[o] = omega * z0; xs[o + 1] = omega * z1; xs[o + 2] = omega * z2;
      } else {
        z[o] = z0; z[o + 1] = z1; z[o + 2] = z2;
        acc[0] += r0 * z0 + r1 * z1 + r2 * z2;
      }
    }
    acc[1] += r0 * r0 + r1 * r1 + r2 * r2;
  }
  block_sum_store<2>(acc, partials, kMaxPartials);
}

__global__ __launch_bounds__(kBlock) void k_update_p(int n3, PcgScalars* S, const double* __restrict__ rz_parts, int n_rz,
                                                     const double* __restrict__ rr_parts, int n_rr,
                                                     const double* __restrict__ zq_parts, const double* __restrict__ z,
                                                     double* __restrict__ p, RecDev rec) {
  const int i0 = blockIdx.x * kBlock + threadIdx.x;
  double z0 = 0.0, p0 = 0.0;
  if (i0 < n3) {
    z0 = z[i0];
    p0 = p[i0];
  }
  const int stop0 = S->stop, iter_prev = S->iter_prev, maxit = S->maxit;
  const double alpha = S->alpha, rz_prev = S->rz_prev, tol2 = S->tol2, bb = S->bb;
  if (stop0) {
    if (rec.mirror && blockIdx.x == 0 && threadIdx.x == 0) *rec.mirror = *S;
    return;
  }
  const double* const parts[3] = {rz_parts, rr_parts, zq_parts};
  const int cnt[3] = {n_rz, n_rr, n_rz};
  double v[3];
  block_reduce_parts_n<3>(parts, cnt, v);
  const double rz = v[0], rr = v[1], zq = v[2];
  const double beta = zq_parts ? -alpha * zq / rz_prev : rz / rz_prev;
  int stop = 0;
  if (!isfinite(rz) || !isfinite(rr)) stop = 3;
  else if (rr <= tol2 * bb) stop = 1;
  else if (iter_prev + 1 >= maxit) stop = 2;
  const bool probe = iter_prev + 1 == S->probe_k;
  if (probe && !stop && S->probe_max > 0.0 && rr > S->probe_max * bb) stop = 4;
  if (blockIdx.x == 0 && threadIdx.x == 0) {
    if (probe) S->probe_rel = rr / bb;
    S->beta = beta;
    S->rz = rz;
    S->rr = rr;
    S->iter = iter_prev + 1;
    if (stop) S->stop = stop;
    if (rec.lanczos && iter_prev < kLanczosMax) {
      rec.lanczos[3 * iter_prev] = alpha;
      rec.lanczos[3 * iter_prev + 1] = beta;
      rec.lanczos[3 * iter_prev + 2] = rz_prev;
    }
    if (rec.mirror) {
      PcgScalars m = *S;
      m.beta = beta; m.rz = rz; m.rr = rr; m.iter = iter_prev + 1;
      if (probe) m.probe_rel = rr / bb;
      if (stop) m.stop = stop;
      *rec.mirror = m;
    }
  }
  if (stop) return;
  if (i0 < n3) {
    p[i0] = z0 + beta * p0;
  }
  for (int i = i0 + gridDim.x * kBlock; i < n3; i += gridDim.x * kBlock) {
    p[i] = z[i] + beta * p[i];
  }
}

__global__ __launch_bounds__(kBlock) void k_dot(int n3, const double* __restrict__ a, const double* __restrict__ b,
                                                double* __restrict__ partials, const PcgScalars* S) {
  if (S && S->stop) return;
  double acc[1] = {0.0};
  for (int i = blockIdx.x * kBlock + threadIdx.x; i < n3; i += gridDim.x * kBlock) acc[0] += a[i] * b[i];
  block_sum_store<1>(acc, partials, kMaxPartials);
}

__global__ __launch_bounds__(kBlock) void k_precond_bj(int n, const double* __restrict__ dinv,
                                                       const double* __restrict__ r, double* __restrict__ z, double scale) {
  for (int i = blockIdx.x * kBlock + threadIdx.x; i < n; i += gridDim.x * kBlock) {
    const size_t o = 3 * (size_t)i;
    const double* di = dinv + 6 * (size_t)i;
    const double r0 = r[o], r1 = r[o + 1], r2 = r[o + 2];
    z[o] = scale * (di[0] * r0 + di[1] * r1 + di[2] * r2);
    z[o + 1] = scale * (di[1] * r0 + di[3] * r1 + di[4] * r2);
    z[o + 2] = scale * (di[2] * r0 + di[4] * r1 + di[5] * r2);
  }
}

__global__ __launch_bounds__(kBlock) void k_pose_update(int n, const int* __restrict__ free_id,
                                                        const double* __restrict__ x, double* __restrict__ poses) {
  for (int i = blockIdx.x * kBlock + threadIdx.x; i < n; i += gridDim.x * kBlock) {
    const size_t v = 3 * (size_t)free_id[i], o = 3 * (size_t)i;
    poses[v] += x[o];
    poses[v + 1] += x[o + 1];
    poses[v + 2] = norm_theta(poses[v + 2] + x[o + 2]);
  }
}

__global__ __launch_bounds__(kBlock) void k_update_xr_rows(int nrows, const int* __restrict__ rows, const PcgScalars* S,
                                                           const double* __restrict__ dinv, const double* __restrict__ p,
                                                           const double* __restrict__ q, double* __restrict__ r,
                                                           double* __restrict__ xs, double omega) {
  if (S->stop) return;
  const double alpha = S->alpha;
  for (int t = blockIdx.x * kBlock + threadIdx.x; t < nrows; t += gridDim.x * kBlock) {
    const size_t i = (size_t)rows[t], o = 3 * i;
    const double r0 = r[o] - alpha * q[o], r1 = r[o + 1] - alpha * q[o + 1], r2 = r[o + 2] - alpha * q[o + 2];
    r[o] = r0; r[o + 1] = r1; r[o + 2] = r2;
    if (xs) {
      const double* pd = dinv + 6 * i;
      const double z0 = pd[0] * r0 + pd[1] * r1 + pd[2] * r2;
      const double z1 = pd[1] * r0 + pd[3] * r1 + pd[4] * r2;
      const double z2 = pd[2] * r0 + pd[4] * r1 + pd[5] * r2;
      xs[o] = omega * z0; xs[o + 1] = omega * z1; xs[o + 2] = omega * z2;
    }
  }
}
__global__ __launch_bounds__(kBlock) void k_update_p_rows(int nrows, const int* __restrict__ rows, const PcgScalars* S,
                                                          const double* __restrict__ z, double* __restrict__ p) {
  if (S->stop) return;
  const double beta = S->beta;
  for (int t = blockIdx.x * kBlock + threadIdx.x; t < nrows; t += gridDim.x * kBlock) {
    const size_t o = 3 * (size_t)rows[t];
    p[o] = z[o] + beta * p[o]; p[o + 1] = z[o + 1] + beta * p[o + 1]; p[o + 2] = z[o + 2] + beta * p[o + 2];
  }
}

__global__ __launch_bounds__(kBlock) void k_halo_pack(const double* __restrict__ data, int width, const int* __restrict__ idx,
                                                      int cnt, double* __restrict__ send, HaloScalars sc) {
// ... 94 lines not shown
  return true;
}

void launch_chi2(hipStream_t s, const EdgeListDev& el, int e0, int e1, const double* poses, double* e2_out,
                 double* partials, int* grid_out, const EdgeListDev* el2) {
  const int grid = grid_for(e1 - e0, kBlock);
  if (el.kinds) SGO_LAUNCH(k_chi2<true>, dim3(grid), dim3(kBlock), 0, s, el, e0, e1, el2 ? *el2 : EdgeListDev(), poses, e2_out, partials);
  else SGO_LAUNCH(k_chi2<false>, dim3(grid), dim3(kBlock), 0, s, el, e0, e1, el2 ? *el2 : EdgeListDev(), poses, e2_out, partials);
  *grid_out = grid;
}
void launch_reduce2(hipStream_t s, const double* partials, int nparts, double* out2) {
  SGO_LAUNCH(k_reduce2, dim3(1), dim3(kBlock), 0, s, partials, nparts, out2);
}
void launch_linearize(hipStream_t s, const Sym0Dev& A, int g0, int g1, const EdgeSlotsDev& es, const double* poses,
                      double* dgb) {
  const int grid = grid_for(g1 - g0, kWavesPerBlock);
  if (es.kinds) SGO_LAUNCH(k_linearize<true>, dim3(grid), dim3(kBlock), 0, s, A, g0, g1, es, poses, dgb);
  else SGO_LAUNCH(k_linearize<false>, dim3(grid), dim3(kBlock), 0, s, A, g0, g1, es, poses, dgb);
}
void launch_finalize(hipStream_t s, const Sym0Dev& A, int row0, int row1, const double* dgb, double* b, double* x, double* r, double* z,
                     double* p, double* xs, double omega, double* partials, int* grid_out) {
  const int grid = grid_for(row1 - row0, kBlock);
  SGO_LAUNCH(k_finalize, dim3(grid), dim3(kBlock), 0, s, A, row0, row1, dgb, b, x, r, z, p, xs, omega, partials);
  *grid_out = grid;
}
int launch_diag_change(hipStream_t s, int row0, int row1, const double* dblk, double* dref, bool store_ref, double* partials) {
  const int grid = grid_for(row1 - row0, kBlock);
  SGO_LAUNCH(k_diag_change, dim3(grid), dim3(kBlock), 0, s, row0, row1, dblk, dref, store_ref ? 1 : 0, partials);
  return grid;
}
void launch_force_stop(hipStream_t s, PcgScalars* S, PcgScalars* mirror) { SGO_LAUNCH(k_force_stop, dim3(1), dim3(1), 0, s, S, mirror); }
void launch_set_probe(hipStream_t s, PcgScalars* S, int probe_k, double probe_max) {
  SGO_LAUNCH(k_set_probe, dim3(1), dim3(1), 0, s, S, probe_k, probe_max);
}
void launch_restart_scalars(hipStream_t s, PcgScalars* S, const double* rz_parts, int n_rz, int maxit, int keep_stop) {
  SGO_LAUNCH(k_restart_scalars, dim3(1), dim3(kBlock), 0, s, S, rz_parts, n_rz, maxit, keep_stop);
}
void launch_warm_start(hipStream_t s, int n3, const double* xp, const double* q, const double* b, double* x, double* r,
                       const double* xq_parts, int n_xq, const double* bx_parts, int n_bx) {
  SGO_LAUNCH(k_warm_start, dim3(grid_for(n3, kBlock)), dim3(kBlock), 0, s, n3, xp, q, b, x, r, xq_parts, n_xq, bx_parts, n_bx);
}
void launch_init_scalars(hipStream_t s, PcgScalars* S, const double* rz_parts, int n_rz, const double* bb_parts,
                         int n_bb, double tol, int maxit, double bb_ref, double tol_cap) {
  SGO_LAUNCH(k_init_scalars, dim3(1), dim3(kBlock), 0, s, S, rz_parts, n_rz, bb_parts, n_bb, tol, maxit, bb_ref, tol_cap);
}
void launch_edge_prepare(hipStream_t s, int E, const double* meas, const double* info, double* zinv, double* info_soa, size_t stride, size_t at) {
  SGO_LAUNCH(k_edge_prepare, dim3(grid_for(E, kBlock)), dim3(kBlock), 0, s, E, meas, info, zinv, info_soa, stride, at);
}
void launch_early_strength(hipStream_t s, const EdgeListDev& el, const double* poses, int n, const int* rowptr, const int* eidx,
                           const unsigned char* flags, const int* hrowptr, double* w) {
  if (n > 0 && el.kinds) SGO_LAUNCH(k_row_strength<true>, dim3(grid_for(n, kBlock)), dim3(kBlock), 0, s, n, rowptr, eidx, flags, hrowptr, el, poses, w);
  else if (n > 0) SGO_LAUNCH(k_row_strength<false>, dim3(grid_for(n, kBlock)), dim3(kBlock), 0, s, n, rowptr, eidx, flags, hrowptr, el, poses, w);
}
void launch_slot_expand(hipStream_t s, int k0, int k1, const int* eidx, const EdgeListDev& el, const EdgeSlotsDev& es) {
  SGO_LAUNCH(k_slot_expand, dim3(grid_for(k1 - k0, kBlock)), dim3(kBlock), 0, s, k0, k1, eidx, el, es);
}
int launch_spmv_ex(hipStream_t s, const BsrDev& A, int mode, const SpmvArgs& a) {
  const int grid = grid_for(A.ngrp, kWavesPerBlock);
  switch (mode) {
    case SPMV_AX: SGO_LAUNCH((k_spmv<SPMV_AX>), dim3(grid), dim3(kBlock), 0, s, A, a); break;
    case SPMV_RESID: SGO_LAUNCH((k_spmv<SPMV_RESID>), dim3(grid), dim3(kBlock), 0, s, A, a); break;
    case SPMV_JACOBI:
      SGO_LAUNCH((k_spmv<SPMV_JACOBI>), dim3(grid), dim3(kBlock), 0, s, A, a);
      break;
    case SPMV_JACOBI_P: SGO_LAUNCH((k_spmv<SPMV_JACOBI_P>), dim3(grid), dim3(kBlock), 0, s, A, a); break;
    case SPMV_PRE_RESID_S: SGO_LAUNCH((k_spmv<SPMV_PRE_RESID_S>), dim3(grid), dim3(kBlock), 0, s, A, a); break;
    case SPMV_PRE_RESID_ACC: SGO_LAUNCH((k_spmv<SPMV_PRE_RESID_ACC>), dim3(grid), dim3(kBlock), 0, s, A, a); break;
    case SPMV_AX_C: SGO_LAUNCH((k_spmv<SPMV_AX_C>), dim3(grid), dim3(kBlock), 0, s, A, a); break;
    default:
      SGO_LAUNCH((k_spmv<SPMV_PRE_RESID>), dim3(grid), dim3(kBlock), 0, s, A, a);
      break;
  }
  return grid;
}
int launch_spmv0(hipStream_t s, const Sym0Dev& A, int mode, const Spmv0Args& a) {
  const int grid = grid_for(A.ngrp, kWavesPerBlock);
  switch (mode) {
    case S0_AX: SGO_LAUNCH((k_spmv0<S0_AX>), dim3(grid), dim3(kBlock), 0, s, A, a); break;
    case S0_RESID: SGO_LAUNCH((k_spmv0<S0_RESID>), dim3(grid), dim3(kBlock), 0, s, A, a); break;
    default: SGO_LAUNCH((k_spmv0<S0_JACOBI>), dim3(grid), dim3(kBlock), 0, s, A, a); break;
  }
  return grid;
}
template <int MODE, int NT, bool F32>
void launch_spmv0t_inst(hipStream_t s, const Sym0Dev& A, const Tile0Dev& T, const Spmv0Args& a, int grid) {
  static int lds_allowed = 0;
  if (T.lds_bytes > 65536 && T.lds_bytes > lds_allowed) {
    constexpr int kDynMax = 160 * 1024 - 2048;
    if (hipFuncSetAttribute(reinterpret_cast<const void*>(&k_spmv0t<MODE, NT, F32>), hipFuncAttributeMaxDynamicSharedMemorySize,
                            kDynMax) == hipSuccess)
      lds_allowed = kDynMax;
  }
  SGO_LAUNCH((k_spmv0t<MODE, NT, F32>), dim3(grid), dim3(NT), (size_t)T.lds_bytes, s, A, T, a);
}
int launch_spmv0t(hipStream_t s, const Sym0Dev& A, const Tile0Dev& T, int mode, const Spmv0Args& a) {
  const int per_cu = std::max(1, std::min(2, (160 * 1024) / std::max(T.lds_bytes + 512, 1)));
  long long g = std::min<long long>(T.ntile, 256LL * per_cu);
  if (g < 8) g = 8;
  const int grid = (int)((g + 7) / 8 * 8);
  const bool f32 = A.fblk != nullptr && !a.force_f64;
  switch (mode) {
    case S0_AX: launch_spmv0t_inst<S0_AX, 1024, false>(s, A, T, a, grid); break;
    case S0_RESID:
      if (f32) launch_spmv0t_inst<S0_RESID, 1024, true>(s, A, T, a, grid);
      else launch_spmv0t_inst<S0_RESID, 1024, false>(s, A, T, a, grid);
      break;
    default:
      if (f32) launch_spmv0t_inst<S0_JACOBI, 1024, true>(s, A, T, a, grid);
      else launch_spmv0t_inst<S0_JACOBI, 1024, false>(s, A, T, a, grid);
      break;
  }
  return grid;
}
void launch_update_xr(hipStream_t s, int n, PcgScalars* S, const double* pq_parts, int n_pq, const double* dinv,
                      const double* p, const double* q, double* x, double* r, double* z, double* xs, double omega,
                      double* partials, int* grid_out) {
  const int grid = grid_for(n, kBlock);
  SGO_LAUNCH(k_update_xr, dim3(grid), dim3(kBlock), 0, s, n, S, pq_parts, n_pq, dinv, p, q, x, r, z, xs, omega, partials);
  if (grid_out) *grid_out = grid;
}
void launch_update_p(hipStream_t s, int n, PcgScalars* S, const double* rz_parts, int n_rz, const double* rr_parts,
                     int n_rr, const double* zq_parts, const double* z, double* p, const RecDev& rec) {
  const int grid = grid_for(3LL * n, kBlock);
  SGO_LAUNCH(k_update_p, dim3(grid), dim3(kBlock), 0, s, 3 * n, S, rz_parts, n_rz, rr_parts, n_rr, zq_parts, z, p, rec);
}
__global__ __launch_bounds__(kBlock) void k_closure_cov(int n, const sgo_match_window* __restrict__ win,
                                                        const float* __restrict__ scores, double* __restrict__ cov,
                                                        double* __restrict__ info) {
  const int lane = threadIdx.x & 63;
  for (int q = blockIdx.x * kWavesPerBlock + (threadIdx.x >> 6); q < n; q += gridDim.x * kWavesPerBlock) {
    const sgo_match_window W = win[q];
    const int nw = 2 * W.w_size + 1, nk = 2 * W.scan_window + 1, total = nw * nw * nk;
    const float* sc = scores + W.score_offset;
    double a[10] = {0, 0, 0, 0, 0, 0, 0, 0, 0, 0};
    for (int e = lane; e < total; e += 64) {
      const int kk = e % nk, jj = (e / nk) % nw, ii = e / (nk * nw);
      const int i = W.x_index_offset - W.w_size + ii, j = W.y_index_offset - W.w_size + jj;
      const int k = W.scan_index - W.scan_window + kk;
      const double x = -j * W.resolution, y = -i * W.resolution;
      const double t = (k - W.num_angular_perturbations) * W.angular_step;
      const double w = (double)sc[e];
      a[0] += x * x * w; a[1] += x * y * w; a[2] += x * t * w;
      a[3] += y * y * w; a[4] += y * t * w; a[5] += t * t * w;
      a[6] += x * w; a[7] += y * w; a[8] += t * w;
      a[9] += w;
    }
#pragma unroll
    for (int c = 0; c < 10; ++c) a[c] = wave_sum(a[c]);
    if (lane == 0) {
      const double d = 1.0 / a[9], d2 = d * d;
      const double c00 = d * a[0] - d2 * a[6] * a[6], c01 = d * a[1] - d2 * a[6] * a[7], c02 = d * a[2] - d2 * a[6] * a[8];
      const double c11 = d * a[3] - d2 * a[7] * a[7], c12 = d * a[4] - d2 * a[7] * a[8], c22 = d * a[5] - d2 * a[8] * a[8];
      double* C = cov + 9 * (size_t)q;
      C[0] = c00; C[1] = c01; C[2] = c02;
      C[3] = c01; C[4] = c11; C[5] = c12;
      C[6] = c02; C[7] = c12; C[8] = c22;
      const double k00 = c11 * c22 - c12 * c12, k01 = c02 * c12 - c01 * c22, k02 = c01 * c12 - c02 * c11;
      const double k11 = c00 * c22 - c02 * c02, k12 = c01 * c02 - c00 * c12, k22 = c00 * c11 - c01 * c01;
      const double id = 1.0 / (c00 * k00 + c01 * k01 + c02 * k02);
      double* I = info + 9 * (size_t)q;
      I[0] = k00 * id; I[1] = k01 * id; I[2] = k02 * id;
      I[3] = k01 * id; I[4] = k11 * id; I[5] = k12 * id;
      I[6] = k02 * id; I[7] = k12 * id; I[8] = k22 * id;
    }
  }
}

void launch_closure_cov(hipStream_t s, int n, const sgo_match_window* win, const float* scores, double* cov,
                        double* info) {
  const int grid = grid_for(n, kWavesPerBlock);
  SGO_LAUNCH(k_closure_cov, dim3(grid), dim3(kBlock), 0, s, n, win, scores, cov, info);
}
void launch_pose_update(hipStream_t s, int n, const int* free_id, const double* x, double* poses) {
  const int grid = grid_for(n, kBlock);
  SGO_LAUNCH(k_pose_update, dim3(grid), dim3(kBlock), 0, s, n, free_id, x, poses);
}
void launch_dot(hipStream_t s, int n3, const double* a, const double* b, double* partials, const PcgScalars* S,
                int* grid_out) {
  const int grid = grid_for(n3, kBlock);
  SGO_LAUNCH(k_dot, dim3(grid), dim3(kBlock), 0, s, n3, a, b, partials, S);
  if (grid_out) *grid_out = grid;
}
void launch_precond_bj(hipStream_t s, int n, const double* dinv, const double* r, double* z, double scale) {
  const int grid = grid_for(n, kBlock);
  SGO_LAUNCH(k_precond_bj, dim3(grid), dim3(kBlock), 0, s, n, dinv, r, z, scale);
}

}
```

### sparse_gslam_amd/csrc/sgo_rules.h

```cpp
#pragma once
#include <algorithm>
#include <cmath>
#include <cstddef>
#include <initializer_list>

#if defined(__HIP__)
#define SGO_RULE_HD __attribute__((host)) __attribute__((device))
#else
#define SGO_RULE_HD
#endif

namespace sgo {
namespace rules {

SGO_RULE_HD inline bool gain_stop(double last, double cur, double gain_tol) {
  const double gain = (last - cur) / cur;
  return gain >= 0.0 && gain < gain_tol;
}
SGO_RULE_HD inline bool gain_stop_applies(int it, int max_iters) { return it >= 2 && it < max_iters; }

template <class Dead>
inline int hypothesis_isolated_vertex(const unsigned char* fixed, int E, const int* ei, const int* ej, Dead dead, const unsigned char* off,
                                      int* live_deg) {
  for (int e = 0; e < E; ++e)
    if (off[e] && !dead(e)) {
      --live_deg[ei[e]];
      --live_deg[ej[e]];
    }
  int lowest = -1;
  for (int e = 0; e < E; ++e)
    if (off[e] && !dead(e))
      for (const int v : {ei[e], ej[e]})
        if (!fixed[v] && live_deg[v] <= 0 && (lowest < 0 || v < lowest)) lowest = v;
  for (int e = 0; e < E; ++e)
    if (off[e] && !dead(e)) {
      ++live_deg[ei[e]];
      ++live_deg[ej[e]];
    }
  return lowest;
}

inline int equal_tolerance_count(int iter, double tol0, double tolk) {
  return (tolk > tol0 && tolk < 1.0 && tol0 > 0.0) ? (int)std::lround(iter * std::log(tol0) / std::log(tolk)) : iter;
}

inline int max_rebuilds(int iters) { return std::max(3, (iters + 2) / 3); }

inline int bail_out_cap(int best) { return 4 * best + 40; }

struct Staleness {
  bool doubled, pays;
  bool rebuild() const { return doubled || pays; }
};
constexpr int kRebuildCostIters = 150;
inline Staleness staleness(int eq_iter, int call_best, int iterations_left, int cost_iters = kRebuildCostIters) {
  Staleness s;
  s.doubled = eq_iter > 2 * call_best + 10;
  s.pays = 4 * eq_iter > 5 * call_best && (long long)(eq_iter - call_best) * iterations_left > cost_iters;
  return s;
}

inline double lag_allowed(double tau, double slope) { return std::min(tau, 4.0 / std::max(slope, 1.0)); }
constexpr double kLagRowsMoved = 32.0;
constexpr double kLagSlopeStart = 2700.0;
constexpr double kLagSlopeMax = 40000.0;
inline double lag_slope_after_kept(double slope, bool seen, int excess, double moved) {
  const double obs = std::min(kLagSlopeMax, std::max(0.5, (double)excess) / std::max(moved, 1e-5));
  return seen ? std::max(obs, 0.8 * slope) : obs;
}
inline double lag_slope_after_interrupt(double slope, double moved) {
  return std::min(std::max(slope, 16.0 / std::max(moved, 1e-6)), kLagSlopeMax);
}
inline double lag_slope_after_fresh(double slope) { return slope > kLagSlopeStart ? std::max(kLagSlopeStart, 0.95 * slope) : slope; }
inline bool kept_solve_too_slow(int eq_iter, int fresh_pcg) { return eq_iter > fresh_pcg + 8 + fresh_pcg / 4; }
inline int lag_cap(int fresh_pcg) { return fresh_pcg > 0 ? fresh_pcg + 3 : 0; }
inline int probe_iteration(int fresh_iter) { return std::max(4, fresh_iter / 3); }

inline bool moved_far(double sum_diff, double sum_norm, double rows_quarter, int n) {
  return sum_norm > 0.0 && (sum_diff > 0.05 * sum_norm || rows_quarter > 0.01 * (double)n);
}
inline bool reaggregate(bool far, bool rule_off, int iterations_left_incl, int agg_best, int eq_iter, int rebuilds, int max_rb, bool rebuild_pending) {
  return far && !rule_off && iterations_left_incl >= 5 && agg_best > 0 && 10 * eq_iter > 11 * agg_best && rebuilds < max_rb && !rebuild_pending;
}
inline bool trial_reverts(int trial_best, int trial_old) { return 100 * trial_best > 85 * trial_old; }

constexpr double kFloorEta = 1e-12;
inline double floor_backward_error(int n, const double* r, const double* x, const double* b, const double* dblk6) {
  double sr = 0.0, sx = 0.0, sb = 0.0;
  for (int i = 0; i < n; ++i)
    for (int q = 0; q < 3; ++q) {
      const double h = dblk6[6 * (std::size_t)i + (q == 0 ? 0 : q == 1 ? 3 : 5)];
      if (!(h > 0.0) || !std::isfinite(h)) return 1.0;
      const std::size_t k = 3 * (std::size_t)i + q;
      sr += r[k] * r[k] / h;
      sx += x[k] * x[k] * h;
      sb += b[k] * b[k] / h;
    }
  const double den = std::sqrt(sx) + std::sqrt(sb);
  const double eta = std::sqrt(sr) / den;
  return (den > 0.0 && std::isfinite(eta)) ? eta : 1.0;
}

}
}
```

### sparse_gslam_amd/csrc/sgo_solve.cpp

```cpp
#include <algorithm>
#include <cmath>
#include <cstdio>
#include <cstdlib>
#include <cstring>

#include "sgo_ctx.h"
#include "sgo_rules.h"

namespace sgo {

hipEvent_t get_event(sgo_ctx* c) {
  if (!c->ev_pool.empty()) {
    hipEvent_t e = c->ev_pool.back();
    c->ev_pool.pop_back();
    return e;
  }
  hipEvent_t e;
  hipEventCreate(&e);
  return e;
}
void prof_calibrate(sgo_ctx* c) {
  if (c->prof_null_ms >= 0.0) return;
  std::vector<float> v;
  for (int k = 0; k < 33; ++k) {
// ... 37 lines not shown
  }
  {
    Scope sc(c, K_REDUCE2, 16.0 * grid);
    launch_reduce2(c->stream, c->d_partials, grid, d_out2);
  }
  if (c->comm.nranks > 1 && !c->replicated && !d_e2 && !c->comm.allreduce_f64(d_out2, 2, c->stream, &c->err)) return SGO_ECOMM;
  return SGO_OK;
}

int do_spmv(sgo_ctx* c, const double* x, double* y, bool dot, const PcgScalars* S, int* grid_out);

static bool xch(sgo_ctx* c, double* vec, const HaloScalars& sc) {
  return halo_exchange(c->halo, c->stream, vec, 3, c->halo.bnd, c->halo.bmax, sc, &c->err);
}
static HaloScalars scal(const double* p0, int n0, const double* p1 = nullptr, int n1 = 0, const double* p2 = nullptr, int n2 = 0) {
  HaloScalars sc;
  sc.parts[0] = p0; sc.n[0] = n0;
  sc.parts[1] = p1; sc.n[1] = n1;
  sc.parts[2] = p2; sc.n[2] = n2;
  return sc;
}

static void set_probe(sgo_ctx* c, int k, double max);
static int start_pcg_owner(sgo_ctx* c, int grid) {
  set_probe(c, 0, 0.0);
  const HaloDev& H = c->halo;
  const int G = H.G, nr = H.row1 - H.row0;
  const size_t o3 = 3 * (size_t)H.row0;
  const int maxit = c->call.pcg_softcap > 0 ? std::min(c->call.pcg_softcap, c->opts.pcg_maxit) : c->opts.pcg_maxit;
  const double tol = c->opts.pcg_tol * c->tol_scale;
  double* bb_parts = c->d_partials + kMaxPartials;
  int rc;
  if (c->amg && !c->call.skip_update && (rc = amg_update(c->amg, c->stream, &c->err))) return rc;
  if (c->amg && amg_comm_failed(c->amg)) return SGO_ECOMM;
  if (c->amg && !halo_exchange(H, c->stream, c->S0.dinv, 6, H.bnd, H.bmax, HaloScalars(), &c->err)) return SGO_ECOMM;
  if (!c->amg) {
    if (!xch(c, c->d_p, scal(c->d_partials, grid, bb_parts, grid))) return SGO_ECOMM;
    Scope sc(c, K_INIT_SCALARS, 16.0 * G);
    launch_init_scalars(c->stream, c->d_S, H.gparts, G, H.gparts + G, G, tol, maxit, c->call.bb_ref, c->tol_cap);
    return SGO_OK;
  }
  if (c->call.warm_valid && c->d_xprev) {
    int gq = 0, gd = 0;
    double* bb_keep = c->d_zparts + kMaxPartials;
    HIP_TRY(c, hipMemcpyAsync(bb_keep, bb_parts, sizeof(double) * (size_t)grid, hipMemcpyDeviceToDevice, c->stream));
    if ((rc = do_spmv(c, c->d_xprev, c->d_q, true, nullptr, &gq))) return rc;
    {
      Scope sc(c, K_DOT, 48.0 * nr);
      launch_dot(c->stream, 3 * nr, c->d_b + o3, c->d_xprev + o3, c->d_partials + 2 * kMaxPartials, nullptr, &gd);
    }
    if (!xch(c, nullptr, scal(bb_keep, grid, c->d_partials, gq, c->d_partials + 2 * kMaxPartials, gd))) return SGO_ECOMM;
    {
      Scope sc(c, K_INIT_SCALARS, 16.0 * G);
      launch_init_scalars(c->stream, c->d_S, H.gparts, G, H.gparts, G, tol, maxit, c->call.bb_ref, c->tol_cap);
    }
    {
      Scope sc(c, K_UPDATE_XR, 120.0 * nr);
      launch_warm_start(c->stream, 3 * nr, c->d_xprev + o3, c->d_q + o3, c->d_b + o3, c->d_x + o3, c->d_r + o3, H.gparts + G, G,
                        H.gparts + 2 * G, G);
    }
    const int gz = amg_apply(c->amg, c->stream, c->d_r, c->d_z, c->d_r, c->d_zparts, nullptr, nullptr, AmgXs0::compute);
    if (amg_comm_failed(c->amg)) return SGO_ECOMM;
    HIP_TRY(c, hipMemcpyAsync(c->d_p + o3, c->d_z + o3, sizeof(double) * 3 * (size_t)nr, hipMemcpyDeviceToDevice, c->stream));
    if (!xch(c, c->d_p, scal(c->d_zparts, gz))) return SGO_ECOMM;
    {
      Scope sc(c, K_INIT_SCALARS, 8.0 * G);
      launch_restart_scalars(c->stream, c->d_S, H.gparts, G, maxit, 1);
    }
    if (!xch(c, c->d_r, HaloScalars())) return SGO_ECOMM;
    return SGO_OK;
  }
  const int gz = amg_apply(c->amg, c->stream, c->d_r, c->d_z, c->d_r, c->d_zparts, nullptr, nullptr, AmgXs0::ready);
  if (amg_comm_failed(c->amg)) return SGO_ECOMM;
  HIP_TRY(c, hipMemcpyAsync(c->d_p + o3, c->d_z + o3, sizeof(double) * 3 * (size_t)nr, hipMemcpyDeviceToDevice, c->stream));
  if (!xch(c, c->d_p, scal(c->d_zparts, gz, bb_parts, grid))) return SGO_ECOMM;
  {
    Scope sc(c, K_INIT_SCALARS, 16.0 * G);
    launch_init_scalars(c->stream, c->d_S, H.gparts, G, H.gparts + G, G, tol, maxit, c->call.bb_ref, c->tol_cap);
  }
  if (!xch(c, c->d_r, HaloScalars())) return SGO_ECOMM;
  return SGO_OK;
}

static RecDev rec_dev(const sgo_ctx* c) {
  RecDev r;
  r.mirror = c->d_Sz;
  r.lanczos = c->d_lanczos;
  return r;
}

static void sum_diag_change(const sgo_ctx* c, int half, int grid, double v[3]) {
  const volatile double* h = c->h_dchg + 3 * (size_t)half * kMaxPartials;
  for (int k = 0; k < 3; ++k) {
    v[k] = 0.0;
    for (int i = 0; i < grid; ++i) v[k] += h[(size_t)k * kMaxPartials + i];
  }
}
static void read_diag_change(sgo_ctx* c) {
  sum_diag_change(c, 0, c->dchg_grid, c->last_dchg);
  c->amg_dchg_pending = false;
}
static void set_probe(sgo_ctx* c, int k, double max) {
  if (k == c->probe_dev_k && max == c->probe_dev_max) return;
  launch_set_probe(c->stream, c->d_S, k, max);
  c->probe_dev_k = k;
  c->probe_dev_max = max;
}

int start_pcg(sgo_ctx* c, int grid) {
  if (c->owner) return start_pcg_owner(c, grid);
  const int maxit = c->call.pcg_softcap > 0 ? std::min(c->call.pcg_softcap, c->opts.pcg_maxit) : c->opts.pcg_maxit;
  const double tol = c->opts.pcg_tol * c->tol_scale;
  c->pcg_counts.start_bb = c->pcg_counts.start_rz = grid;
  c->pcg_counts.n_xq = c->pcg_counts.n_bx = 0;
  c->pcg_start.tol = tol;
  c->pcg_start.tol_cap = c->tol_cap;
  c->pcg_start.bb_ref = c->call.bb_ref;
  c->pcg_start.maxit = maxit;
  if (c->amg) {
    int rc = c->call.skip_update ? SGO_OK : amg_update(c->amg, c->stream, &c->err);
    if (rc) return rc;
    const bool warm = c->call.warm_valid && c->d_xprev;
    if (warm) {
      {
        Scope sc(c, K_INIT_SCALARS, 16.0 * grid);
        launch_init_scalars(c->stream, c->d_S, c->d_partials, grid, c->d_partials + kMaxPartials, grid, tol, maxit, c->call.bb_ref, c->tol_cap);
      }
      int gq = 0, gd = 0;
      if ((rc = do_spmv(c, c->d_xprev, c->d_q, true, nullptr, &gq))) return rc;
      {
        Scope sc(c, K_DOT, 48.0 * c->n);
        launch_dot(c->stream, 3 * c->n, c->d_b, c->d_xprev, c->d_partials + 2 * kMaxPartials, nullptr, &gd);
      }
      {
        Scope sc(c, K_UPDATE_XR, 120.0 * c->n);
        launch_warm_start(c->stream, 3 * c->n, c->d_xprev, c->d_q, c->d_b, c->d_x, c->d_r, c->d_partials, gq,
                          c->d_partials + 2 * kMaxPartials, gd);
      }
      c->pcg_counts.n_xq = gq;
      c->pcg_counts.n_bx = gd;
    }
    const AmgXs0 xs_ready = warm ? AmgXs0::compute : AmgXs0::ready;
    const int gz = amg_apply(c->amg, c->stream, c->d_r, c->d_z, c->d_r, c->d_zparts, nullptr, nullptr, xs_ready);
    if (amg_comm_failed(c->amg)) return SGO_ECOMM;
    HIP_TRY(c, hipMemcpyAsync(c->d_p, c->d_z, sizeof(double) * 3 * (size_t)c->n, hipMemcpyDeviceToDevice, c->stream));
    c->pcg_counts.start_rz = gz;
    if (warm) {
      Scope sc(c, K_INIT_SCALARS, 8.0 * gz);
      launch_restart_scalars(c->stream, c->d_S, c->d_zparts, gz, maxit, 1);
    } else {
      Scope sc(c, K_INIT_SCALARS, 8.0 * (gz + grid));
      launch_init_scalars(c->stream, c->d_S, c->d_zparts, gz, c->d_partials + kMaxPartials, grid, tol, maxit, c->call.bb_ref, c->tol_cap);
    }
    set_probe(c, c->call.lag_on ? c->hier.probe_k : 0, c->call.skip_update ? c->hier.probe_max : 0.0);
  } else {
    Scope sc(c, K_INIT_SCALARS, 16.0 * grid);
    launch_init_scalars(c->stream, c->d_S, c->d_partials, grid, c->d_partials + kMaxPartials, grid, tol, maxit, c->call.bb_ref, c->tol_cap);
    set_probe(c, 0, 0.0);
  }
  return SGO_OK;
}

static double lag_allowed(const sgo_ctx* c) { return rules::lag_allowed(c->knobs.lag_tau, c->hier.lag_slope); }
static double moved_rel(const sgo_ctx* c, double none) { return c->last_dchg[1] > 0.0 ? c->last_dchg[0] / c->last_dchg[1] : none; }

static int refresh_and_continue(sgo_ctx* c, int maxit) {
  int rc = amg_update(c->amg, c->stream, &c->err);
  if (rc) return rc;
  HIP_TRY(c, hipMemcpyAsync(c->d_dref, c->S0.dblk, sizeof(double) * 6 * (size_t)c->n, hipMemcpyDeviceToDevice, c->stream));
  c->hier.ref_valid = true;
// ... 78 lines not shown
    if (!c->gather_slices) HIP_TRY(c, hipMemsetAsync(y, 0, sizeof(double) * 3 * (size_t)c->n, c->stream));
    if (a.u1 > a.u0) {
      Scope sc(c, c->T0.ntile > 0 ? K_SPMV0T_AX : K_SPMV0_AX, bytes_spmv0(c->S0, S0_AX) * (a.u1 - a.u0) / std::max(1, c->shard_units));
      launch_spmv0_any(c->stream, c->S0, c->T0, S0_AX, a);
    }
    if (c->gather_slices) {
      if (!halo_gather_slices(c->halo, c->stream, y, 3, &c->err)) return SGO_ECOMM;
    } else if (!c->comm.allreduce_f64(y, 3 * (size_t)c->n, c->stream, &c->err)) {
      return SGO_ECOMM;
    }
    if (dot) {
      int grid = 0;
      Scope sc(c, K_DOT, 48.0 * c->n);
      launch_dot(c->stream, 3 * c->n, x, y, c->d_partials, S, &grid);
      if (grid_out) *grid_out = grid;
    }
    return SGO_OK;
  }
  Scope sc(c, c->T0.ntile > 0 ? K_SPMV0T_AX : K_SPMV0_AX, bytes_spmv0(c->S0, S0_AX));
  if (dot) {
    a.dotA = x;
    a.partials = c->d_partials;
  }
  const int grid = launch_spmv0_any(c->stream, c->S0, c->T0, S0_AX, a);
  if (c->ov.active) launch_ov_ax(c->stream, c->ov.dev, x, y, dot ? c->d_partials : nullptr, S);
  if (grid_out) *grid_out = grid;
  return SGO_OK;
}

static int pcg_iteration_owner(sgo_ctx* c) {
  const HaloDev& H = c->halo;
  const int G = H.G, nr = H.row1 - H.row0;
  const size_t o3 = 3 * (size_t)H.row0;
  int g1 = 0, g2 = 0, rc;
  if ((rc = do_spmv(c, c->d_p, c->d_q, true, c->d_S, &g1))) return rc;
  double* parts2 = c->d_partials + kMaxPartials;
  if (c->amg) {
    if (!xch(c, c->d_q, scal(c->d_partials, g1))) return SGO_ECOMM;
    {
      Scope sc(c, K_UPDATE_XR, (7 * 24.0 + 48.0) * nr);
      launch_update_xr(c->stream, nr, c->d_S, H.gparts, G, c->S0.dinv + 6 * (size_t)H.row0, c->d_p + o3, c->d_q + o3, c->d_x + o3,
                       c->d_r + o3, c->d_z + o3, amg_xs0(c->amg) + o3, amg_omega(c->amg), parts2, &g2);
    }
    launch_update_xr_rows(c->stream, H.nhalo, H.halo_rows, c->d_S, c->S0.dinv, c->d_p, c->d_q, c->d_r, amg_xs0(c->amg), amg_omega(c->amg));
    const int gz = amg_apply(c->amg, c->stream, c->d_r, c->d_z, c->d_r, c->d_zparts, c->d_S, c->d_q, AmgXs0::ready_with_halo);
    if (amg_comm_failed(c->amg)) {
      c->err = "collective failed inside the multigrid cycle";
      return SGO_ECOMM;
    }
    if (!xch(c, c->d_z, scal(c->d_zparts, gz, parts2 + kMaxPartials, g2, c->d_zparts + kMaxPartials, gz))) return SGO_ECOMM;
    {
      Scope sc(c, K_UPDATE_P, 3 * 24.0 * nr);
      launch_update_p(c->stream, nr, c->d_S, H.gparts, G, H.gparts + G, G, H.gparts + 2 * G, c->d_z + o3, c->d_p + o3);
    }
    launch_update_p_rows(c->stream, H.nhalo, H.halo_rows, c->d_S, c->d_z, c->d_p);
    return SGO_OK;
  }
  if (!xch(c, nullptr, scal(c->d_partials, g1))) return SGO_ECOMM;
  {
    Scope sc(c, K_UPDATE_XR, (7 * 24.0 + 48.0) * nr);
    launch_update_xr(c->stream, nr, c->d_S, H.gparts, G, c->S0.dinv + 6 * (size_t)H.row0, c->d_p + o3, c->d_q + o3, c->d_x + o3,
                     c->d_r + o3, c->d_z + o3, nullptr, 0.0, parts2, &g2);
  }
  if (!xch(c, nullptr, scal(parts2, g2, parts2 + kMaxPartials, g2))) return SGO_ECOMM;
  {
    Scope sc(c, K_UPDATE_P, 3 * 24.0 * nr);
    launch_update_p(c->stream, nr, c->d_S, H.gparts, G, H.gparts + G, G, nullptr, c->d_z + o3, c->d_p + o3);
  }
  if (!xch(c, c->d_p, HaloScalars())) return SGO_ECOMM;
  return SGO_OK;
}

int pcg_iteration(sgo_ctx* c) {
  if (c->owner) return pcg_iteration_owner(c);
  int g1 = 0, g2 = 0, rc;
  if ((rc = do_spmv(c, c->d_p, c->d_q, true, c->d_S, &g1))) return rc;
  double* parts2 = c->d_partials + kMaxPartials;
  {
    Scope sc(c, K_UPDATE_XR, (7 * 24.0 + 48.0) * c->n);
    launch_update_xr(c->stream, c->n, c->d_S, c->d_partials, g1, c->S0.dinv, c->d_p, c->d_q, c->d_x, c->d_r, c->d_z,
                     c->amg ? amg_xs0(c->amg) : nullptr, c->amg ? amg_omega(c->amg) : 0.0, parts2, &g2);
  }
  if (c->amg) {
    const int gz = amg_apply(c->amg, c->stream, c->d_r, c->d_z, c->d_r, c->d_zparts, c->d_S, c->d_q, AmgXs0::ready);
    if (amg_comm_failed(c->amg)) {
      c->err = "collective failed inside the multigrid cycle";
      return SGO_ECOMM;
    }
    c->pcg_counts.n_rz = c->pcg_counts.n_zq = gz;
    Scope sc(c, K_UPDATE_P, 3 * 24.0 * c->n);
    launch_update_p(c->stream, c->n, c->d_S, c->d_zparts, gz, parts2 + kMaxPartials, g2, c->d_zparts + kMaxPartials,
                    c->d_z, c->d_p, rec_dev(c));
  } else {
    c->pcg_counts.n_rz = g2;
    c->pcg_counts.n_zq = 0;
    Scope sc(c, K_UPDATE_P, 3 * 24.0 * c->n);
    launch_update_p(c->stream, c->n, c->d_S, parts2, g2, parts2 + kMaxPartials, g2, nullptr, c->d_z, c->d_p, rec_dev(c));
  }
  c->pcg_counts.n_pq = g1;
  c->pcg_counts.n_rr = g2;
  return SGO_OK;
}

int ensure_pcg_graph(sgo_ctx* c, int chunk, bool* captured) {
  const int key = c->ov.active ? 1 : 0;
  if (captured) *captured = false;
  if (c->pcg_exec && c->pcg_exec_chunk == chunk && c->pcg_exec_key == key) return SGO_OK;
  if (captured) *captured = true;
  if (c->pcg_exec) {
    HIP_TRY(c, hipStreamSynchronize(c->stream));
    hipGraphExecDestroy(c->pcg_exec);
    c->pcg_exec = nullptr;
  }
  hipGraph_t graph = nullptr;
  HIP_TRY(c, hipStreamBeginCapture(c->stream, hipStreamCaptureModeThreadLocal));
  int rc = SGO_OK;
  for (int k = 0; k < chunk && rc == SGO_OK; ++k) rc = pcg_iteration(c);
  hipError_t e = hipStreamEndCapture(c->stream, &graph);
  if (rc != SGO_OK) {
    if (graph) hipGraphDestroy(graph);
    return rc;
  }
  if (e != hipSuccess) {
    c->err = std::string("hipStreamEndCapture: ") + hipGetErrorString(e);
    return SGO_EHIP;
  }
  e = hipGraphInstantiate(&c->pcg_exec, graph, nullptr, nullptr, 0);
  hipGraphDestroy(graph);
  if (e != hipSuccess) {
    c->pcg_exec = nullptr;
    c->err = std::string("hipGraphInstantiate: ") + hipGetErrorString(e);
    return SGO_EHIP;
  }
  c->pcg_exec_chunk = chunk;
  c->pcg_exec_key = key;
  return SGO_OK;
}

void read_call_knobs(sgo_ctx* c) {
  sgo_ctx::CallKnobs k;
  if (const char* e = std::getenv("SGO_COMM_GRAPH")) k.comm_graph = std::atoi(e) != 0 ? 1 : 0;
  if (const char* e = std::getenv("SGO_PCG_STALL_WINDOW")) k.stall_window = std::max(0, std::atoi(e));
  if (const char* e = std::getenv("SGO_FIRST_SOLVE_CAP")) k.first_solve_cap = std::max(1, std::atoi(e));
  if (const char* e = std::getenv("SGO_TEST_FAIL_TRIAL_BUILD")) k.fail_trial_build = std::atoi(e) != 0;
  if (const char* e = std::getenv("SGO_TEST_FAIL_DEVICE_SETUP")) k.fail_device_setup = std::atoi(e) != 0;
  if (const char* e = std::getenv("SGO_AMG_KEEP_AGG")) k.keep_agg = std::atoi(e) != 0;
  if (const char* e = std::getenv("SGO_AMG_SETUP")) k.setup_mode = std::string(e) == "host" ? 0 : (std::string(e) == "rebuilds" ? 1 : 2);
  if (const char* e = std::getenv("SGO_AMG_LISTS"))
    if (std::string(e) == "host") k.setup_mode = 0;
  if (const char* e = std::getenv("SGO_AMG_FORCE_REBUILD")) k.force_rebuild = std::atoi(e) != 0;
  if (const char* e = std::getenv("SGO_AMG_AGG")) k.dev_aggregation = std::string(e) == "device";
  if (const char* e = std::getenv("SGO_AMG_REBUILD_COST")) k.rebuild_cost = std::max(1, std::atoi(e));
  if (const char* e = std::getenv("SGO_AMG_LAG")) k.lag_on = std::atoi(e) != 0;
  if (const char* e = std::getenv("SGO_AMG_LAG_TAU")) k.lag_tau = std::atof(e);
  if (const char* e = std::getenv("SGO_AMG_LAG_SLOPE")) k.lag_slope = std::atof(e);
  if (const char* e = std::getenv("SGO_AMG_LAG_FORCE")) k.lag_force_from = std::atoi(e);
  c->knobs = k;
}

int run_pcg(sgo_ctx* c) {
  bool comm_graph = c->comm.handle != nullptr && !c->comm.host_fn && !c->comm_graph_failed && c->comm.nranks <= 1;
  if (c->knobs.comm_graph >= 0)
    comm_graph = c->comm.handle != nullptr && !c->comm.host_fn && !c->comm_graph_failed && c->knobs.comm_graph != 0;
  c->pcg_stalled = false;
  c->pcg_stall_window = multi_rank(c) ? 0 : std::max(3000, 30 * std::max(1, c->pcg_pred));
  if (c->call.floor_seen && c->pcg_stall_window > 0) c->pcg_stall_window = std::max(300, 3 * std::max(1, c->pcg_pred));
  if (c->knobs.stall_window >= 0) c->pcg_stall_window = multi_rank(c) ? 0 : c->knobs.stall_window;
  double stall_rr = -1.0;
  int stall_it = 0;
  auto stalled = [&](const volatile PcgScalars* S) -> bool {
    if (c->pcg_stall_window <= 0 || c->pcg_stalled) return false;
    const double rr = S->rr;
    const int it = S->iter;
    if (stall_rr < 0.0 || rr < stall_rr) {
      stall_rr = rr;
      stall_it = it;
      return false;
    }
    return it - stall_it > c->pcg_stall_window;
  };
  bool graph = c->opts.use_graph && !c->opts.profile && (!multi_rank(c) || comm_graph);
  constexpr int kUnit = 2;
  if (graph) {
    bool attempted = false;
    const int grc = ensure_pcg_graph(c, kUnit, &attempted);
    if (multi_rank(c)) {
      int failed = grc != SGO_OK ? 1 : 0;
      if (attempted && c->comm.nranks > 1) {
        if (!c->d_comm_flag) HIP_TRY(c, hipMalloc((void**)&c->d_comm_flag, sizeof(int)));
        HIP_TRY(c, hipMemcpyAsync(c->d_comm_flag, &failed, sizeof(int), hipMemcpyHostToDevice, c->stream));
        std::string cerr;
        if (!c->comm.allreduce_i32(c->d_comm_flag, 1, c->stream, &cerr)) {
          c->err = "all-reduce of the capture flags: " + cerr;
          return SGO_ECOMM;
        }
        HIP_TRY(c, hipMemcpyAsync(&failed, c->d_comm_flag, sizeof(int), hipMemcpyDeviceToHost, c->stream));
        HIP_TRY(c, hipStreamSynchronize(c->stream));
      }
      if (failed) {
        if (c->pcg_exec) {
          hipGraphExecDestroy(c->pcg_exec);
          c->pcg_exec = nullptr;
        }
        c->comm_graph_failed = true;
        graph = false;
        if (c->opts.verbose)
          std::fprintf(stderr, "[sgo] capturing the collectives failed on %d rank(s)%s%s: plain stream launches on all ranks from here on\n", failed,
                       grc != SGO_OK ? "; here: " : "", grc != SGO_OK ? c->err.c_str() : "");
      }
    } else if (grc != SGO_OK) {
      return grc;
    }
  }
  if (!graph) {
    const int chunk = c->opts.profile ? 1 : std::max(1, c->opts.pcg_chunk);
    for (;;) {
      HIP_TRY(c, hipMemcpyAsync(c->h_S, c->d_S, sizeof(PcgScalars), hipMemcpyDeviceToHost, c->stream));
      HIP_TRY(c, hipStreamSynchronize(c->stream));
      if (c->h_S->stop) break;
      if (stalled(c->h_S)) {
        c->pcg_stalled = true;
        launch_force_stop(c->stream, c->d_S, nullptr);
        continue;
      }
      for (int k = 0; k < chunk; ++k) {
        int rc = pcg_iteration(c);
        if (rc) return rc;
      }
    }
    c->pcg_pred = c->h_S->iter;
    return SGO_OK;
  }
  const int chunk_launches = std::max(1, c->opts.pcg_chunk / 16);
  const int pred = c->pcg_pred;
  const int unchecked = std::max(0, (int)(0.8 * pred) - 4) / kUnit;
  for (int k = 0; k < unchecked; ++k) HIP_TRY(c, hipGraphLaunch(c->pcg_exec, c->stream));
  static const bool mirror_env = !(std::getenv("SGO_MIRROR") && std::atoi(std::getenv("SGO_MIRROR")) == 0);
  const bool mirror = mirror_env && !multi_rank(c) && !c->owner;
  int slot = 0;
// ... 438 lines not shown
static int solve_step(sgo_ctx* c, CallPolicy& pol, int it, int* wasted, bool* interrupted, bool* floor_accept) {
  int rc;
  if ((rc = run_pcg(c))) return rc;
  const PcgScalars& S = *c->h_S;
  if (c->call.skip_update && c->amg && (S.stop == 4 || (S.stop == 2 && S.iter < c->opts.pcg_maxit && c->call.pcg_softcap > 0))) {
    const int at = S.iter;
    c->call.pcg_softcap = pol.continue_cap(c->hier, at);
    const int maxit = c->call.pcg_softcap > 0 ? std::min(c->call.pcg_softcap, c->opts.pcg_maxit) : c->opts.pcg_maxit;
    c->pcg_pred = std::max(2, pol.fresh_pcg);
    if ((rc = refresh_and_continue(c, maxit)) || (rc = run_pcg(c))) return rc;
    *interrupted = true;
    pol.kept_interrupted(c->hier, moved_rel(c, 0.0));
    if (c->opts.verbose)
      std::fprintf(stderr, "[sgo] iteration %d: solve behind kept coarse operators interrupted after %d PCG iterations, operators refreshed\n", it, at);
  }
  if ((rc = check_floor(c, pol, it, floor_accept))) return rc;
  if (!*floor_accept && c->call.pcg_softcap > 0 && S.stop == 2 && S.iter < c->opts.pcg_maxit && c->amg) {
    *wasted = S.iter;
    pol.abandon(c->hier, amg_has_filtered(c->amg));
    const std::string what = "solve abandoned after " + std::to_string(*wasted) + " PCG iterations, hierarchy rebuilt";
    if ((rc = rebuild_and_solve(c, pol, it, c->knobs.keep_agg && c->hier.best != 0, what, floor_accept))) return rc;
  }
  if (!*floor_accept && S.stop == 3 && c->amg && amg_has_filtered(c->amg) && pol.can_rebuild()) {
    *wasted += S.iter;
    c->hier.no_filter = true;
    return rebuild_and_solve(c, pol, it, false, "PCG breakdown behind a filtered hierarchy, rebuilt with tentative transfers and solved again", floor_accept);
  }
  return SGO_OK;
}

static int record_solve(sgo_ctx* c, CallPolicy& pol, int it, bool interrupted, bool floor_accept) {
  const PcgScalars& S = *c->h_S;
  double v[3];
  if (c->agg_grid > 0) sum_diag_change(c, 1, c->agg_grid, v);
  const SolveRecord r{it, S.iter, c->opts.pcg_tol * c->tol_scale, std::sqrt(S.tol2), c->call.skip_update, interrupted, floor_accept,
                      moved_rel(c, 0.0), S.probe_k, S.probe_rel, c->amg_prev != nullptr, c->agg_grid > 0 ? v : nullptr, c->n};
  c->agg_grid = 0;
  if (pol.record(c->hier, r, c->opts.verbose ? stderr : nullptr) != CallPolicy::kRevertTrial) return SGO_OK;
  if (const int rc = revert_amg(c)) return rc;
  if (c->opts.verbose)
    std::fprintf(stderr, "[sgo] iteration %d: the re-aggregated hierarchy is no better (%d against %d): the old one is back\n", it, pol.trial_best, pol.trial_old);
  return SGO_OK;
}

static std::string failure_message(sgo_ctx* c, const PcgScalars& S, int it) {
  if (S.stop == 3)
    return "PCG breakdown in GN iteration " + std::to_string(it) + " (Hessian not positive definite" +
           (c->amg && amg_coarsest_not_spd(c->amg, c->stream) ? "; its coarsest Galerkin operator has a non-positive pivot" : "") + ")";
  return (c->pcg_stalled ? "PCG stagnated (no new minimum of the residual in the last " + std::to_string(c->pcg_stall_window) + " of " +
                               std::to_string(S.iter) + " iterations; pcg_maxit = "
                         : "PCG did not reach pcg_tol within pcg_maxit = ") + std::to_string(c->opts.pcg_maxit) +
         (c->pcg_stalled ? ")" : " iterations") + " in GN iteration " + std::to_string(it) + " (relative residual " +
         std::to_string(S.bb > 0 ? std::sqrt(S.rr / S.bb) : 0.0) + "); the step was not applied";
}

int optimize_gn(sgo_ctx* c, int32_t iters, sgo_stats* out, UntilGain* until) {
  int rc = check_graph(c);
  if (rc) return rc;
  if (iters < 0 || iters > SGO_MAX_ITERS) {
    c->err = "sgo_optimize_gn: iters must be in [0, SGO_MAX_ITERS]";
    return SGO_EINVAL;
  }
  if (out) {
    std::memset(out, 0, sizeof(*out));
    out->iters_requested = iters;
    out->seconds_setup = c->setup_seconds;
  }
  if (c->n == 0) return SGO_ENOTHING;
  const double t0 = wall_s();
  read_call_knobs(c);
  if (until) until->stop_reason = SGO_STOP_MAX_ITERS;
  if (c->direct || c->mf) return optimize_factored(c, iters, out, t0, until);
  if ((rc = ensure_amg(c))) return rc;
  while (c->iter_events.size() < 3 * (size_t)iters + 1) {
    hipEvent_t e = nullptr;
    HIP_TRY(c, hipEventCreate(&e));
    c->iter_events.push_back(e);
  }
  std::vector<hipEvent_t>& ev = c->iter_events;
  struct CallScope { sgo_ctx* c; ~CallScope() { c->call = sgo_ctx::CallState(); } } call_scope{c};
  c->call = sgo_ctx::CallState();
  c->call.in_optimize = true;
  c->call.lag_on = c->knobs.lag_on && !multi_rank(c);
  c->hier.begin_call(c->n, c->knobs.lag_slope);
  c->lag_note.clear();
  c->tol_cap = c->opts.pcg_tol_cap > 0.0 ? std::max(c->opts.pcg_tol_cap, c->opts.pcg_tol * c->tol_scale) : 0.0;
  CallPolicy pol(iters, c->knobs.rebuild_cost, c->knobs.force_rebuild && c->amg != nullptr);
  int done = 0;
  bool failed = false, stopped = false;
  for (int it = 0; it < iters; ++it) {
    hipEventRecord(ev[3 * it], c->stream);
    c->call.pcg_softcap = pol.solve_cap(c->hier, c->amg != nullptr, c->knobs.first_solve_cap);
    c->call.lag_cap = pol.lag_cap();
    c->call.force_keep = c->knobs.lag_force_from >= 0 && it > c->knobs.lag_force_from;
    if ((rc = linearize_step(c, pol, it, iters, until, &stopped))) return rc;
    if (stopped) break;
    hipEventRecord(ev[3 * it + 1], c->stream);
    int wasted = 0;
    bool interrupted = false, floor_accept = false;
    if ((rc = solve_step(c, pol, it, &wasted, &interrupted, &floor_accept))) return rc;
    if (c->amg_dchg_pending) read_diag_change(c);
    if (c->call.lag_on)
      c->call.lag_expect = c->hier.ref_valid && moved_rel(c, 1.0) <= 2.0 * lag_allowed(c) && c->last_dchg[2] <= 4.0 * rules::kLagRowsMoved;
    const PcgScalars S = *c->h_S;
    if (it == 0 && c->tol_cap > 0.0 && S.stop == 1) c->call.bb_ref = S.bb;
    if (c->amg && S.stop != 3 && (rc = record_solve(c, pol, it, interrupted, floor_accept))) return rc;
    if (it == 0 && S.stop == 1) {
      c->its_last = S.iter;
      if (!c->ov.active && c->its_base == 0) c->its_base = S.iter;
    }
    if (out) {
      out->pcg_iters[it] = S.iter + wasted;
      out->pcg_converged[it] = S.stop == 1 ? 1 : (floor_accept ? 2 : 0);
      out->pcg_relres[it] = S.bb > 0 ? std::sqrt(S.rr / S.bb) : 0.0;
    }
    if (S.stop != 1 && !floor_accept) {
      c->err = failure_message(c, S, it);
      failed = true;
      hipEventRecord(ev[3 * it + 2], c->stream);
      break;
    }
    if (c->owner && !halo_gather_slices(c->halo, c->stream, c->d_x, 3, &c->err)) return SGO_ECOMM;
    if (c->ov.active) launch_ov_finish(c->stream, c->ov.dev, c->d_x, c->d_poses);
    {
      Scope sc(c, K_POSE_UPDATE, 72.0 * c->n);
      launch_pose_update(c->stream, c->n, c->d_free_id, c->d_x, c->d_poses);
    }
    if (c->opts.pcg_warm_start && c->amg && c->d_xprev) {
      HIP_TRY(c, hipMemcpyAsync(c->d_xprev, c->d_x, sizeof(double) * 3 * (size_t)c->n, hipMemcpyDeviceToDevice, c->stream));
      c->call.warm_valid = !pol.rebuild_next;
    }
    hipEventRecord(ev[3 * it + 2], c->stream);
    c->linearized = false;
    ++done;
    if (c->opts.verbose)
      std::fprintf(stderr, "[sgo] iteration= %d\t pcg= %d\t relres= %.3e\t |b|= %.3e\t diag moved %.3e (%.0f rows > 1/4; kept up to %.1e)%s\n", it, S.iter,
                   S.bb > 0 ? std::sqrt(S.rr / S.bb) : 0.0, std::sqrt(S.bb), moved_rel(c, 0.0), c->last_dchg[2], lag_allowed(c),
                   c->call.skip_update ? " coarse operators kept" : "");
  }
  c->lag_note = pol.note(done);
  if (until) until->stop_reason = failed ? SGO_STOP_FAILED : (stopped ? SGO_STOP_GAIN : SGO_STOP_MAX_ITERS);
  if ((rc = do_chi2(c, c->d_hist + 2 * done, nullptr))) return rc;
  HIP_TRY(c, hipMemcpyAsync(c->h_hist, c->d_hist, sizeof(double) * 2 * (size_t)(done + 1), hipMemcpyDeviceToHost, c->stream));
  HIP_TRY(c, hipStreamSynchronize(c->stream));
  if (c->amg_prev && pol.trial == CallPolicy::kNoTrial) {
    amg_destroy(c->amg_prev);
    c->amg_prev = nullptr;
    c->amg_arena_prev.rewind();
  }
  prof_flush(c);
  if (out) {
    copy_history(c, done, out);
    const int timed = std::min(iters, done + (stopped ? 0 : 1));
    for (int k = 0; k < timed; ++k) {
      float a = 0.f, b = 0.f;
      hipEventElapsedTime(&a, ev[3 * k], ev[3 * k + 1]);
      hipEventElapsedTime(&b, ev[3 * k + 1], ev[3 * k + 2]);
      out->seconds_linearize[k] = a * 1e-3;
      out->seconds_solve[k] = b * 1e-3;
      out->seconds[k] = (a + b) * 1e-3;
    }
    out->seconds_total = wall_s() - t0;
  }
  return failed ? 0 : done;
}

double debug_spmv0_us(sgo_ctx* c, int mode, int variant, int reps) {
  if (check_graph(c) != SGO_OK || reps < 1 || c->n == 0 || ensure_rows(c) != SGO_OK || c->owner || c->ov.active) return -1.0;
  hipEvent_t a, b;
  if (hipEventCreate(&a) != hipSuccess || hipEventCreate(&b) != hipSuccess) return -1.0;
  Spmv0Args args{};
  args.x = c->d_p;
  args.y = c->d_s2;
  args.b = c->d_b;
  args.omega = 0.8;
  args.force_f64 = (variant & 64) != 0;
  const bool tiled = c->T0.ntile > 0 && !(variant & 16);
  long long* d_st = nullptr;
  if ((variant & 32) && tiled) {
    hipMalloc((void**)&d_st, sizeof(long long) * 8 * (size_t)c->T0.ntile);
    hipMemset(d_st, 0, sizeof(long long) * 8 * (size_t)c->T0.ntile);
    args.dbg_stamps = d_st;
  }
  if (tiled) launch_spmv0t(c->stream, c->S0, c->T0, mode, args);
  else launch_spmv0(c->stream, c->S0, mode, args);
  if (variant & 128) {
    hipGraph_t g = nullptr;
    hipGraphExec_t ex = nullptr;
    hipStreamBeginCapture(c->stream, hipStreamCaptureModeThreadLocal);
    for (int k = 0; k < 16; ++k) {
      if (tiled) launch_spmv0t(c->stream, c->S0, c->T0, mode, args);
      else launch_spmv0(c->stream, c->S0, mode, args);
    }
    hipStreamEndCapture(c->stream, &g);
    if (!g || hipGraphInstantiate(&ex, g, nullptr, nullptr, 0) != hipSuccess) return -1.0;
    hipGraphLaunch(ex, c->stream);
    hipEventRecord(a, c->stream);
    for (int k = 0; k < (reps + 15) / 16; ++k) hipGraphLaunch(ex, c->stream);
    hipEventRecord(b, c->stream);
    hipStreamSynchronize(c->stream);
    hipGraphExecDestroy(ex);
    hipGraphDestroy(g);
    reps = (reps + 15) / 16 * 16;
  } else {
  hipEventRecord(a, c->stream);
  for (int k = 0; k < reps; ++k) {
    if (tiled) launch_spmv0t(c->stream, c->S0, c->T0, mode, args);
    else launch_spmv0(c->stream, c->S0, mode, args);
  }
  hipEventRecord(b, c->stream);
  }
  hipStreamSynchronize(c->stream);
  float ms = 0.f;
  hipEventElapsedTime(&ms, a, b);
  hipEventDestroy(a);
  hipEventDestroy(b);
  if (d_st) {
    std::vector<long long> st(8 * (size_t)c->T0.ntile);
    hipMemcpy(st.data(), d_st, sizeof(long long) * st.size(), hipMemcpyDeviceToHost);
    hipFree(d_st);
    double ph[6] = {0, 0, 0, 0, 0, 0};
    for (int t = 0; t < c->T0.ntile; ++t)
      for (int q = 0; q < 6; ++q) ph[q] += (double)(st[8 * t + q + 1] - st[8 * t + q]);
// ... 19 lines not shown
```

Baseline: 263.2 million.

## Skip multigrid cycle when PCG residual already meets tolerance

```diff
diff --git a/sparse_gslam_amd/csrc/sgo_amg.h b/sparse_gslam_amd/csrc/sgo_amg.h
--- a/sparse_gslam_amd/csrc/sgo_amg.h
+++ b/sparse_gslam_amd/csrc/sgo_amg.h
@@ -77,7 +77,7 @@
   ready_with_halo = 2
 };
 int amg_apply(Amg* m, hipStream_t s, const double* r, double* z, const double* dotvec, double* partials,
-              const PcgScalars* S, const double* dotvec2 = nullptr, AmgXs0 xs0 = AmgXs0::compute);
+              const PcgScalars* S, const double* dotvec2 = nullptr, AmgXs0 xs0 = AmgXs0::compute, const ConvTest& conv = ConvTest());
 struct Comm;
 void amg_set_shard(Amg* m, Comm* comm, int u0, int u1, int row0, int row1, const HaloDev* slices = nullptr);
 bool amg_comm_failed(const Amg* m);
diff --git a/sparse_gslam_amd/csrc/sgo_amg.hip b/sparse_gslam_amd/csrc/sgo_amg.hip
--- a/sparse_gslam_amd/csrc/sgo_amg.hip
+++ b/sparse_gslam_amd/csrc/sgo_amg.hip
@@ -424,8 +424,12 @@
 }
 __global__ __launch_bounds__(kBlock, 4) void k_jacobi0_restrict(Sym0Dev A, Spmv0Args a, int nb_spmv, PDev P, double* __restrict__ rc,
                                                                  int nb_main) {
-  if ((int)blockIdx.x < nb_spmv) spmv0_groups<S0_JACOBI>(A, a, nb_spmv);
-  else restrict_groups(P, a.b, rc, a.S, 0, 0, nb_main, (int)blockIdx.x - nb_spmv);
+  if ((int)blockIdx.x < nb_spmv) {
+    spmv0_groups<S0_JACOBI>(A, a, nb_spmv);
+  } else {
+    if (a.conv.S && !a.conv.S->stop && (a.conv.always || a.conv.S->armed) && cycle_converged<kBlock>(a.conv, false)) return;
+    restrict_groups(P, a.b, rc, a.S, 0, 0, nb_main, (int)blockIdx.x - nb_spmv);
+  }
 }
 void launch_restrict_p(hipStream_t s, const PDev& P, const double* r, double* rc, const PcgScalars* S, int row0, int row1) {
   const int nb = grid_for(P.t_ngrp, kWavesPerBlock);
@@ -1472,7 +1476,7 @@
   Scope sc(m->prof, K_DOT, 96.0 * m->lv[0].A.n);
   launch_precond_bj(s, own ? sh.row1 - sh.row0 : m->lv[0].A.n, m->S0.dinv + 6 * r0, rhs + 3 * r0, m->lv[0].xs + 3 * r0, m->cfg.omega);
 }
-void presmooth0(Amg* m, hipStream_t s, const double* rhs, const PcgScalars* S, AmgXs0 xs0) {
+void presmooth0(Amg* m, hipStream_t s, const double* rhs, const PcgScalars* S, AmgXs0 xs0, const ConvTest& conv) {
   AmgLevel& L = m->lv[0];
   Shard0& sh = m->shard;
   first_sweep0(m, s, rhs, xs0);
@@ -1480,6 +1484,7 @@
   if (sh.mode == Shard0::allreduce && !sh.part) hipMemsetAsync(L.rs, 0, sizeof(double) * 3 * (size_t)L.A.n, s);
   Spmv0Args a{};
   a.x = L.xs; a.b = rhs; a.y = L.rs; a.S = S; a.u0 = sh.u0; a.u1 = sh.u1;
+  a.conv = conv;
   if (sh.mode == Shard0::single || a.u1 > a.u0) pass0(m, s, S0_RESID, a, sh.G);
 }
 void prolong0(Amg* m, hipStream_t s, const CoarseSol& cs, const PcgScalars* S) {
@@ -1521,12 +1526,14 @@
   SGO_LAUNCH(k_dots2, dim3(grid), dim3(kBlock), 0, s, 3 * L.A.n, (const double*)out, dots.vec, dots.vec2, dots.parts, S);
   return grid;
 }
-int cycle0_fold(Amg* m, hipStream_t s, const double* rhs, double* out, const DotReq& dots, const PcgScalars* S, AmgXs0 xs0) {
+int cycle0_fold(Amg* m, hipStream_t s, const double* rhs, double* out, const DotReq& dots, const PcgScalars* S, AmgXs0 xs0,
+                const ConvTest& conv) {
   AmgLevel& L = m->lv[0];
   AmgLevel& C = m->lv[1];
   first_sweep0(m, s, rhs, xs0);
   Spmv0Args b{};
   b.x = L.xs; b.b = rhs; b.y = L.rs; b.omega = m->cfg.omega; b.S = S;
+  b.conv = conv;
   if (m->T0.ntile == 0) {
     const int nb_spmv = grid_for(m->S0.ngrp, kWavesPerBlock), nb_main = grid_for(L.PS.t_ngrp, kWavesPerBlock);
     Scope sc(m->prof, K_JACOBI0_RESTRICT, bytes_spmv0(m->S0, S0_JACOBI) + 44.0 * L.PS.t_n + 24.0 * L.A.n + 24.0 * L.nc);
@@ -1542,9 +1549,9 @@
              dots.vec2, dots.vec ? dots.parts : nullptr);
   return grid;
 }
-int cycle0(Amg* m, hipStream_t s, const double* rhs, double* out, const DotReq& dots, const PcgScalars* S, AmgXs0 xs0) {
-  if (cycle_form(m, 0, false, dots.vec).kind == CycleForm::folded) return cycle0_fold(m, s, rhs, out, dots, S, xs0);
-  presmooth0(m, s, rhs, S, xs0);
+int cycle0(Amg* m, hipStream_t s, const double* rhs, double* out, const DotReq& dots, const PcgScalars* S, AmgXs0 xs0, const ConvTest& conv) {
+  if (cycle_form(m, 0, false, dots.vec).kind == CycleForm::folded) return cycle0_fold(m, s, rhs, out, dots, S, xs0, conv);
+  presmooth0(m, s, rhs, S, xs0, conv);
   restrict_level(m, s, 0, m->lv[0].rs, S);
   m->shard.reduce(s, m->lv[1].bk, 3 * (size_t)m->lv[1].A.n);
   const CoarseSol cs = coarse_solve(m, s, 0, S);
@@ -1769,7 +1776,7 @@
   if (m->lv[0].fold) {
     restrict_level(m, s, 0, r, nullptr, true);
   } else {
-    presmooth0(m, s, r, nullptr, AmgXs0::compute);
+    presmooth0(m, s, r, nullptr, AmgXs0::compute, ConvTest());
     restrict_level(m, s, 0, m->lv[0].rs, nullptr);
   }
   hipMemcpyAsync(out_dev, m->lv[1].bk, sizeof(double) * n3c, hipMemcpyDeviceToDevice, s);
@@ -1884,7 +1891,7 @@
 double amg_omega(const Amg* m) { return m ? m->cfg.omega : 0.0; }
 
 int amg_apply(Amg* m, hipStream_t s, const double* r, double* z, const double* dotvec, double* partials,
-              const PcgScalars* S, const double* dotvec2, AmgXs0 xs0) {
+              const PcgScalars* S, const double* dotvec2, AmgXs0 xs0, const ConvTest& conv) {
   if (m->lv.size() == 1) {
     {
       Scope sc(m->prof, K_DENSE_APPLY, 8.0 * m->N * m->N);
@@ -1896,7 +1903,7 @@
     SGO_LAUNCH(k_dots2, dim3(grid), dim3(kBlock), 0, s, m->N, (const double*)z, dotvec, dotvec2, partials, S);
     return grid;
   }
-  return cycle0(m, s, r, z, DotReq{dotvec, dotvec2, partials}, S, xs0);
+  return cycle0(m, s, r, z, DotReq{dotvec, dotvec2, partials}, S, xs0, conv);
 }
 
 void dev_scan_exclusive(hipStream_t s, int* v, int n, int* sums) {
diff --git a/sparse_gslam_amd/csrc/sgo_ctx.h b/sparse_gslam_amd/csrc/sgo_ctx.h
--- a/sparse_gslam_amd/csrc/sgo_ctx.h
+++ b/sparse_gslam_amd/csrc/sgo_ctx.h
@@ -107,6 +107,9 @@
     int lag_force_from = -1;
     int rebuild_cost = 150;
     bool force_rebuild = false;
+    bool skip_converged_cycle = true;
+    bool skip_arm_always = false;
+    double skip_near = 0.0;
   } knobs;
   struct CallState {
     bool in_optimize = false;
@@ -119,6 +122,9 @@
     bool lag_expect = false;
     bool force_keep = false;
     int lag_cap = 0;
+    bool skip_converged_cycle = false;
+    int cycles_skipped = 0, solves_run = 0;
+    int armed_iters = 0;
   } call;
   AmgKeptAgg kept_agg;
   double* d_poses = nullptr;
@@ -136,6 +142,7 @@
   PcgScalars* d_S = nullptr;
   double* d_lanczos = nullptr;
   int pcg_exec_key = 0;
+  double pcg_exec_near = 0.0;
   PcgScalars* h_S = nullptr;
   double* h_hist = nullptr;
   bool linearized = false;
diff --git a/sparse_gslam_amd/csrc/sgo_device.h b/sparse_gslam_amd/csrc/sgo_device.h
--- a/sparse_gslam_amd/csrc/sgo_device.h
+++ b/sparse_gslam_amd/csrc/sgo_device.h
@@ -286,6 +286,45 @@
   }
 }
 
+template <int kThreads>
+__device__ __forceinline__ double block_reduce_parts_wide(const double* parts, int nparts) {
+  if (kThreads == kBlock) return block_reduce_parts(parts, nparts);
+  __shared__ double smw[kWavesPerBlock];
+  __shared__ double resw;
+  if (threadIdx.x < kBlock) {
+    double s = 0.0;
+    for (int i = threadIdx.x; i < nparts; i += kBlock) s += parts[i];
+    s = wave_sum(s);
+    if ((threadIdx.x & 63) == 0) smw[threadIdx.x >> 6] = s;
+  }
+  __syncthreads();
+  if (threadIdx.x == 0) {
+    double t = smw[0];
+#pragma unroll
+    for (int k = 1; k < kWavesPerBlock; ++k) t += smw[k];
+    resw = t;
+  }
+  __syncthreads();
+  return resw;
+}
+
+template <int kThreads>
+__device__ __forceinline__ bool cycle_converged(const ConvTest& t, bool recorder) {
+  PcgScalars* S = t.S;
+  const double tol2 = S->tol2, bb = S->bb;
+  const int iter_prev = S->iter_prev, probe_k = S->probe_k;
+  const double rr = block_reduce_parts_wide<kThreads>(t.rr_parts, t.n_rr);
+  if (!isfinite(rr) || !(rr <= tol2 * bb)) return false;
+  if (recorder && threadIdx.x == 0) {
+    if (iter_prev + 1 == probe_k) S->probe_rel = rr / bb;
+    S->rr = rr;
+    S->iter = iter_prev + 1;
+    S->armed = -1 - S->armed;
+    S->stop = 1;
+  }
+  return true;
+}
+
 template <int CTRL, int ROW_MASK>
 __device__ __forceinline__ int dpp_int(int old, int v) {
   if (ROW_MASK == 0xF) return __builtin_amdgcn_update_dpp(0, v, CTRL, 0xF, 0xF, true);
@@ -482,6 +521,7 @@
     f_r0 = A.grow[gc.g]; f_ob = A.gown[gc.g]; f_tb = A.gtr[gc.g];
   }
   if (a.S && a.S->stop) return;
+  if (MODE != S0_AX && a.conv.S && (a.conv.always || a.conv.S->armed) && cycle_converged<kBlock>(a.conv, blockIdx.x == 0)) return;
   for (bool first = true; gc.g < gc.gend; gc.g += gc.gstride, first = false) {
     int gb, ge;
     group_bounds(gc, A.grp, first, gb, ge);
diff --git a/sparse_gslam_amd/csrc/sgo_internal.h b/sparse_gslam_amd/csrc/sgo_internal.h
--- a/sparse_gslam_amd/csrc/sgo_internal.h
+++ b/sparse_gslam_amd/csrc/sgo_internal.h
@@ -124,7 +124,7 @@
   int stop;
   int iter_prev;
   int probe_k;
-  int pad_;
+  int armed;
   double probe_rel;
   double probe_max;
 };
@@ -163,6 +163,12 @@
   double* x_out = nullptr;
 };
 
+struct ConvTest {
+  PcgScalars* S = nullptr;
+  const double* rr_parts = nullptr;
+  int n_rr = 0;
+  int always = 0;
+};
 enum : int { S0_AX = 0, S0_RESID = 1, S0_JACOBI = 2 };
 struct Spmv0Args {
   const double* x = nullptr;
@@ -173,6 +179,7 @@
   const double* dotA2 = nullptr;
   double* partials = nullptr;
   const PcgScalars* S = nullptr;
+  ConvTest conv;
   long long* dbg_stamps = nullptr;
   bool force_f64 = false;
   int u0 = 0, u1 = 0;
@@ -464,6 +471,7 @@
 struct RecDev {
   PcgScalars* mirror = nullptr;
   double* lanczos = nullptr;
+  double arm_near = 0.0;
 };
 void launch_update_p(hipStream_t s, int n, PcgScalars* S, const double* rz_parts, int n_rz, const double* rr_parts,
                      int n_rr, const double* zq_parts, const double* z, double* p, const RecDev& rec = RecDev());
diff --git a/sparse_gslam_amd/csrc/sgo_kernels.hip b/sparse_gslam_amd/csrc/sgo_kernels.hip
--- a/sparse_gslam_amd/csrc/sgo_kernels.hip
+++ b/sparse_gslam_amd/csrc/sgo_kernels.hip
@@ -292,6 +292,7 @@
     S->beta = 0.0;
     S->iter_prev = S->iter;
     S->maxit = maxit;
+    S->armed = 0;
     if (!(keep_stop && S->stop)) S->stop = (isfinite(rz) && rz >= 0.0) ? (rz == 0.0 ? 1 : 0) : 3;
   }
 }
@@ -332,6 +333,7 @@
     S->iter = 0;
     S->iter_prev = 0;
     S->maxit = maxit;
+    S->armed = 0;
     S->stop = (bb == 0.0) ? 1 : (isfinite(bb) && isfinite(rz) ? 0 : 3);
   }
 }
@@ -526,7 +528,7 @@
   }
 }
 
-template <int MODE, int kTileThreads, bool F32 = false>
+template <int MODE, int kTileThreads, bool F32 = false, bool CONV = false>
 __global__ __launch_bounds__(kTileThreads) void k_spmv0t(Sym0Dev A, Tile0Dev TL, Spmv0Args a) {
   const int stop_flag = a.S ? a.S->stop : 0;
   extern __shared__ double lds[];
@@ -539,6 +541,10 @@
   const int xcd = blockIdx.x & 7, slot = blockIdx.x >> 3, per_xcd = gridDim.x >> 3;
   const int ulo = a.u1 > 0 ? a.u0 : 0, nun = (a.u1 > 0 ? a.u1 : TL.ntile) - ulo;
   const int tlo = ulo + (int)(((long long)nun * xcd) >> 3), thi = ulo + (int)(((long long)nun * (xcd + 1)) >> 3);
+  if (CONV) {
+    if (stop_flag) return;
+    if ((a.conv.always | a.conv.S->armed) && cycle_converged<kTileThreads>(a.conv, blockIdx.x == 0)) return;
+  }
   for (int t = tlo + slot; t < thi; t += per_xcd) {
     const int hc_first = tid < TL.hstride ? TL.hfirst[(size_t)t * TL.hstride + tid] : -1;
     const TileDesc T = TL.tile[t];
@@ -806,6 +812,7 @@
   else if (iter_prev + 1 >= maxit) stop = 2;
   const bool probe = iter_prev + 1 == S->probe_k;
   if (probe && !stop && S->probe_max > 0.0 && rr > S->probe_max * bb) stop = 4;
+  const bool near = rr <= rec.arm_near * (tol2 * bb);
   if (blockIdx.x == 0 && threadIdx.x == 0) {
     if (probe) S->probe_rel = rr / bb;
     S->beta = beta;
@@ -813,6 +820,7 @@
     S->rr = rr;
     S->iter = iter_prev + 1;
     if (stop) S->stop = stop;
+    else if (rec.arm_near > 0.0) S->armed = near ? S->armed + 1 : 0;
     if (rec.lanczos && iter_prev < kLanczosMax) {
       rec.lanczos[3 * iter_prev] = alpha;
       rec.lanczos[3 * iter_prev + 1] = beta;
@@ -1073,16 +1081,21 @@
   }
   return grid;
 }
-template <int MODE, int NT, bool F32>
+template <int MODE, int NT, bool F32, bool CONV = false>
 void launch_spmv0t_inst(hipStream_t s, const Sym0Dev& A, const Tile0Dev& T, const Spmv0Args& a, int grid) {
   static int lds_allowed = 0;
   if (T.lds_bytes > 65536 && T.lds_bytes > lds_allowed) {
     constexpr int kDynMax = 160 * 1024 - 2048;
-    if (hipFuncSetAttribute(reinterpret_cast<const void*>(&k_spmv0t<MODE, NT, F32>), hipFuncAttributeMaxDynamicSharedMemorySize,
+    if (hipFuncSetAttribute(reinterpret_cast<const void*>(&k_spmv0t<MODE, NT, F32, CONV>), hipFuncAttributeMaxDynamicSharedMemorySize,
                             kDynMax) == hipSuccess)
       lds_allowed = kDynMax;
   }
-  SGO_LAUNCH((k_spmv0t<MODE, NT, F32>), dim3(grid), dim3(NT), (size_t)T.lds_bytes, s, A, T, a);
+  SGO_LAUNCH((k_spmv0t<MODE, NT, F32, CONV>), dim3(grid), dim3(NT), (size_t)T.lds_bytes, s, A, T, a);
+}
+template <int MODE, int NT, bool F32>
+void launch_spmv0t_pass(hipStream_t s, const Sym0Dev& A, const Tile0Dev& T, const Spmv0Args& a, int grid) {
+  if (a.conv.S) launch_spmv0t_inst<MODE, NT, F32, true>(s, A, T, a, grid);
+  else launch_spmv0t_inst<MODE, NT, F32, false>(s, A, T, a, grid);
 }
 int launch_spmv0t(hipStream_t s, const Sym0Dev& A, const Tile0Dev& T, int mode, const Spmv0Args& a) {
   const int per_cu = std::max(1, std::min(2, (160 * 1024) / std::max(T.lds_bytes + 512, 1)));
@@ -1093,12 +1106,12 @@
   switch (mode) {
     case S0_AX: launch_spmv0t_inst<S0_AX, 1024, false>(s, A, T, a, grid); break;
     case S0_RESID:
-      if (f32) launch_spmv0t_inst<S0_RESID, 1024, true>(s, A, T, a, grid);
-      else launch_spmv0t_inst<S0_RESID, 1024, false>(s, A, T, a, grid);
+      if (f32) launch_spmv0t_pass<S0_RESID, 1024, true>(s, A, T, a, grid);
+      else launch_spmv0t_pass<S0_RESID, 1024, false>(s, A, T, a, grid);
       break;
     default:
-      if (f32) launch_spmv0t_inst<S0_JACOBI, 1024, true>(s, A, T, a, grid);
-      else launch_spmv0t_inst<S0_JACOBI, 1024, false>(s, A, T, a, grid);
+      if (f32) launch_spmv0t_pass<S0_JACOBI, 1024, true>(s, A, T, a, grid);
+      else launch_spmv0t_pass<S0_JACOBI, 1024, false>(s, A, T, a, grid);
       break;
   }
   return grid;
diff --git a/sparse_gslam_amd/csrc/sgo_rules.h b/sparse_gslam_amd/csrc/sgo_rules.h
--- a/sparse_gslam_amd/csrc/sgo_rules.h
+++ b/sparse_gslam_amd/csrc/sgo_rules.h
@@ -61,6 +61,7 @@
 }
 
 inline double lag_allowed(double tau, double slope) { return std::min(tau, 4.0 / std::max(slope, 1.0)); }
+constexpr double kSkipNear = 1e1;
 constexpr double kLagRowsMoved = 32.0;
 constexpr double kLagSlopeStart = 2700.0;
 constexpr double kLagSlopeMax = 40000.0;
diff --git a/sparse_gslam_amd/csrc/sgo_solve.cpp b/sparse_gslam_amd/csrc/sgo_solve.cpp
--- a/sparse_gslam_amd/csrc/sgo_solve.cpp
+++ b/sparse_gslam_amd/csrc/sgo_solve.cpp
@@ -143,10 +143,14 @@
   return SGO_OK;
 }
 
+static bool skips_converged_cycle(const sgo_ctx* c) {
+  return c->call.skip_converged_cycle && c->amg && amg_xs0(c->amg) && !c->owner && !multi_rank(c) && !c->d_lanczos;
+}
 static RecDev rec_dev(const sgo_ctx* c) {
   RecDev r;
   r.mirror = c->d_Sz;
   r.lanczos = c->d_lanczos;
+  if (skips_converged_cycle(c)) r.arm_near = c->knobs.skip_near > 0.0 ? c->knobs.skip_near : rules::kSkipNear;
   return r;
 }
 
@@ -391,7 +395,14 @@
                      c->amg ? amg_xs0(c->amg) : nullptr, c->amg ? amg_omega(c->amg) : 0.0, parts2, &g2);
   }
   if (c->amg) {
-    const int gz = amg_apply(c->amg, c->stream, c->d_r, c->d_z, c->d_r, c->d_zparts, c->d_S, c->d_q, AmgXs0::ready);
+    ConvTest conv;
+    if (skips_converged_cycle(c)) {
+      conv.S = c->d_S;
+      conv.rr_parts = parts2 + kMaxPartials;
+      conv.n_rr = g2;
+      conv.always = c->knobs.skip_arm_always ? 1 : 0;
+    }
+    const int gz = amg_apply(c->amg, c->stream, c->d_r, c->d_z, c->d_r, c->d_zparts, c->d_S, c->d_q, AmgXs0::ready, conv);
     if (amg_comm_failed(c->amg)) {
       c->err = "collective failed inside the multigrid cycle";
       return SGO_ECOMM;
@@ -412,9 +423,10 @@
 }
 
 int ensure_pcg_graph(sgo_ctx* c, int chunk, bool* captured) {
-  const int key = c->ov.active ? 1 : 0;
+  const int key = (c->ov.active ? 1 : 0) | (skips_converged_cycle(c) ? (c->knobs.skip_arm_always ? 6 : 2) : 0);
   if (captured) *captured = false;
-  if (c->pcg_exec && c->pcg_exec_chunk == chunk && c->pcg_exec_key == key) return SGO_OK;
+  const double near = rec_dev(c).arm_near;
+  if (c->pcg_exec && c->pcg_exec_chunk == chunk && c->pcg_exec_key == key && c->pcg_exec_near == near) return SGO_OK;
   if (captured) *captured = true;
   if (c->pcg_exec) {
     HIP_TRY(c, hipStreamSynchronize(c->stream));
@@ -443,6 +455,7 @@
   }
   c->pcg_exec_chunk = chunk;
   c->pcg_exec_key = key;
+  c->pcg_exec_near = near;
   return SGO_OK;
 }
 
@@ -464,6 +477,9 @@
   if (const char* e = std::getenv("SGO_AMG_LAG_TAU")) k.lag_tau = std::atof(e);
   if (const char* e = std::getenv("SGO_AMG_LAG_SLOPE")) k.lag_slope = std::atof(e);
   if (const char* e = std::getenv("SGO_AMG_LAG_FORCE")) k.lag_force_from = std::atoi(e);
+  if (const char* e = std::getenv("SGO_SKIP_CONVERGED_CYCLE")) k.skip_converged_cycle = std::atoi(e) != 0;
+  if (const char* e = std::getenv("SGO_SKIP_ARM_ALWAYS")) k.skip_arm_always = std::atoi(e) != 0;
+  if (const char* e = std::getenv("SGO_SKIP_NEAR")) k.skip_near = std::atof(e);
   c->knobs = k;
 }
 
@@ -1068,6 +1084,7 @@
   c->call = sgo_ctx::CallState();
   c->call.in_optimize = true;
   c->call.lag_on = c->knobs.lag_on && !multi_rank(c);
+  c->call.skip_converged_cycle = c->knobs.skip_converged_cycle;
   c->hier.begin_call(c->n, c->knobs.lag_slope);
   c->lag_note.clear();
   c->tol_cap = c->opts.pcg_tol_cap > 0.0 ? std::max(c->opts.pcg_tol_cap, c->opts.pcg_tol * c->tol_scale) : 0.0;
@@ -1089,6 +1106,9 @@
     if (c->call.lag_on)
       c->call.lag_expect = c->hier.ref_valid && moved_rel(c, 1.0) <= 2.0 * lag_allowed(c) && c->last_dchg[2] <= 4.0 * rules::kLagRowsMoved;
     const PcgScalars S = *c->h_S;
+    ++c->call.solves_run;
+    if (S.armed < 0) ++c->call.cycles_skipped;
+    c->call.armed_iters += S.armed < 0 ? -S.armed : S.armed;
     if (it == 0 && c->tol_cap > 0.0 && S.stop == 1) c->call.bb_ref = S.bb;
     if (c->amg && S.stop != 3 && (rc = record_solve(c, pol, it, interrupted, floor_accept))) return rc;
     if (it == 0 && S.stop == 1) {
@@ -1125,6 +1145,11 @@
                    c->call.skip_update ? " coarse operators kept" : "");
   }
   c->lag_note = pol.note(done);
+  if (c->opts.verbose && skips_converged_cycle(c))
+    std::fprintf(stderr, "[sgo] convergence tested in front of the multigrid cycle in %d PCG iterations of %d solves, %d converged there\n",
+                 c->call.armed_iters, c->call.solves_run, c->call.cycles_skipped);
+  c->lag_note += std::string(c->lag_note.empty() ? "last sgo_optimize_gn; " : "; ") + "converged cycles skipped: " + std::to_string(c->call.cycles_skipped) + " of " +
+                 std::to_string(c->call.solves_run) + " solves";
   if (until) until->stop_reason = failed ? SGO_STOP_FAILED : (stopped ? SGO_STOP_GAIN : SGO_STOP_MAX_ITERS);
   if ((rc = do_chi2(c, c->d_hist + 2 * done, nullptr))) return rc;
   HIP_TRY(c, hipMemcpyAsync(c->h_hist, c->d_hist, sizeof(double) * 2 * (size_t)(done + 1), hipMemcpyDeviceToHost, c->stream));
```

After: 262.4 million. No clear change (-0.3%).
